# calmiLovesAI/ComputerVision.pytorch

Hardware: AMD Instinct MI355X
Metric: images/sec 640x640 YOLOv8-n train step (higher is better)
Workload: dtype f16; 1 GPU; YOLOv8-n train step (fwd + v8 loss + bwd + Adam), batch 32/GPU, 640x640, nc=80, random init; global_batch=32, parallelism=dp1, launch=eager, exchange=none (1 rank), gpu_max_hw_queues=4

## Files before the change

computervision.pytorch_amd/_lib.py:

```python
from __future__ import annotations

import ctypes as C
import os

import numpy as np

_HERE = os.path.dirname(os.path.abspath(__file__))
LIB_PATH = os.environ.get("CVX_LIB") or os.path.join(_HERE, "lib", "libcvx_engine.so")
ABI_VERSION = 6
SEG_OPTS_KEY_OFFSET = 4096


class CvxError(RuntimeError):
    pass


class BufDesc(C.Structure):
    _fields_ = [("h", C.c_int32), ("w", C.c_int32), ("c", C.c_int32), ("kind", C.c_int32)]


class View(C.Structure):
    _fields_ = [("buf", C.c_int32), ("coff", C.c_int32), ("c", C.c_int32), ("pix_off", C.c_int32)]


class OpDesc(C.Structure):
    _fields_ = [
        ("type", C.c_int32),
        ("in_", View), ("out", View), ("res", View),
        ("ih", C.c_int32), ("iw", C.c_int32), ("oh", C.c_int32), ("ow", C.c_int32),
        ("k", C.c_int32), ("stride", C.c_int32), ("pad", C.c_int32), ("dil", C.c_int32),
        ("act", C.c_int32), ("needs_dgrad", C.c_int32), ("w_cin", C.c_int32),
        ("w_off", C.c_int64), ("gamma_off", C.c_int64), ("beta_off", C.c_int64), ("bias_off", C.c_int64),
        ("rmean_off", C.c_int64), ("rvar_off", C.c_int64),
        ("lane", C.c_int32), ("flags", C.c_int32),
    ]


class SegDims(C.Structure):
    _fields_ = [(k, C.c_int32) for k in ("ld", "batch", "nc", "ih", "iw", "oh", "ow")]


class SegCriterion(C.Structure):
    _fields_ = [("base", C.c_int32), ("focal_alpha", C.c_float), ("focal_gamma", C.c_float), ("class_weight", C.c_void_p),
                ("label_smoothing", C.c_float), ("ignore_index", C.c_int64), ("ohem_theta", C.c_float), ("ohem_min_kept", C.c_int64),
                ("region", C.c_int32), ("base_weight", C.c_double), ("weight", C.c_double), ("alpha", C.c_double), ("beta", C.c_double),
                ("gamma", C.c_double), ("smooth", C.c_double), ("per_image", C.c_int32), ("skip_absent", C.c_int32),
                ("region_class_weight", C.c_void_p)]


BUF_ACT_F16, BUF_PRED_F32 = 0, 1
OP_CONV, OP_MAXPOOL5, OP_UPSAMPLE2, OP_MAXPOOL2, OP_DWCONVT, OP_COPY, OP_MAXPOOL3S2, OP_AVGPOOL, OP_RESIZE, OP_MAXPOOL3S1, OP_L2NORM = 1, 2, 3, 4, 5, 6, 7, 8, 9, 10, 11
OP_DROPOUT = 12
ACT_BN_SILU, ACT_BIAS, ACT_BN_RELU, ACT_BN_LINEAR, ACT_BIAS_RELU, ACT_BIAS_LINEAR = 1, 2, 3, 4, 5, 6
OPF_RES_PRE_ACT = 1
OPF_CONV_BIAS = 2
OPF_RAW_F16 = 4

_P, _I32, _I64, _F, _U64 = C.c_void_p, C.c_int32, C.c_int64, C.c_float, C.c_uint64

EXPERIMENTAL_PROTOTYPES = {
    "cvx_chain_pair_unit": (_I32, [_P, _I32, _I32, _I32, _I32, _P, _P, _P, _P, _P, _P, _I32, _P, _I32, _I32, _I32, C.POINTER(_F), _P]),
    "cvx_chain_conv_unit": (_I32, [_P, _I32, _I32, _I32, _I32, _P, _I32, _I32, _I32, _I32, _P, _P, _I32, _P, _I32, _I32, _I32, C.POINTER(_F), _P]),
    "cvx_chain_detect_unit": (_I32, [_P, _I32, _I32, _I32, _I32, _I32, _I32, _I32, _P, _P, _P, _P, _P, _P, _P, _P, _P, _P, _P, _I32, _I32, _I32,
                                     _I32, _I32, C.POINTER(_F), _P]),
    "cvx_wgrad_time_unit": (_I32, [_P, _P, _I32, _I32, _I32, _I32, _I32, _I32, _I32, _I32, _I32, _I32, _P, _I64, C.POINTER(_F), C.POINTER(_I32), _P]),
}

PROTOTYPES = {
    "cvx_last_error": (C.c_char_p, []),
    "cvx_abi_version": (_I32, []),
    "cvx_engine_create": (_I32, [C.POINTER(_P), C.POINTER(BufDesc), _I32, C.POINTER(OpDesc), _I32, _I32, _I32, _I32, _P]),
    "cvx_engine_destroy": (_I32, [_P]),
    "cvx_engine_bind": (_I32, [_P, _P, _P, _I64, _P, _I64]),
    "cvx_engine_set_bn": (_I32, [_P, _F, _F]),
    "cvx_engine_forward": (_I32, [_P, _P, _I32, _I32, _P]),
    "cvx_engine_backward": (_I32, [_P, _P, _F]),
    "cvx_engine_backward_begin": (_I32, [_P, _P, _F]),
    "cvx_engine_backward_range": (_I32, [_P, _I32, _I32]),
    "cvx_engine_grads_ready": (_I32, [_P, _I32, _I32, _P]),
    "cvx_engine_backward_end": (_I32, [_P]),
    "cvx_engine_workspace_bytes": (_I64, [_P]),
    "cvx_engine_plan_generation": (_I64, [_P]),
    "cvx_engine_debug_copy": (_I32, [_P, _I32, _I32, _P, _I64]),
    "cvx_engine_profile": (_I32, [_P, _I32]),
    "cvx_engine_profile_read": (_I32, [_P, _I32, C.POINTER(C.c_double), C.POINTER(C.c_double), C.POINTER(C.c_double),
                                       C.POINTER(_I64)]),
    "cvx_debug_clock_buffer": (_I32, [_P]),
    "cvx_debug_conv_tile_plan": (_I32, [_I32, _I32, _I32, _I32, _I32, _P]),
    "cvx_debug_conv_dma_plan": (_I32, [_I64, _I32, _I32, _I32, _P]),
    "cvx_debug_conv_halo_plan": (_I32, [_I32, _I32, _I32, _I32, _I32, _P]),
    "cvx_debug_conv_pw_plan": (_I32, [_I64, _I32, _I32, _P]),
    "cvx_debug_conv_grid_div": (_I32, [_I32]),
    "cvx_debug_conv_wgrad_plan": (_I32, [_I32] * 14 + [_P]),
    "cvx_debug_conv2d_wgrad_nhwc": (_I32, [_P, _P] + [_I32] * 13 + [_P, _P, _I64, _P]),
    "cvx_engine_profile_dump": (_I32, [_P, C.c_char_p]),
    "cvx_pred_level_to_nchw": (_I32, [_P, _I32, _I32, _I32, _I32, _I32, _I32, _P, _P]),
    "cvx_nchw_grad_to_dpred": (_I32, [_P, _I32, _I32, _I32, _I32, _I32, _I32, _F, _P, _P]),
    "cvx_loss_v8_workspace_bytes": (_I64, [_I32, _I32, _I32, _I32]),
    "cvx_loss_v8": (_I32, [_P, _I32, _I32, _I32, _P, _I32, _I32, C.POINTER(_I32), C.POINTER(_F), _I32, _F, _F, _F, _F, _P, _P, _P,
                           _I64, _P]),
    "cvx_loss_v8_strided": (_I32, [_P, _I32, _I32, _I32, _I32, _P, _I32, _I32, C.POINTER(_I32), C.POINTER(_F), _I32, _F, _F, _F, _F, _P, _P, _P,
                                   _I64, _P]),
    "cvx_loss_v8_assignment": (_I32, [_P, _I32, _I32, _I32, _P, _P, _P]),
    "cvx_pack_targets": (_I32, [_P, _P, _P, _I32, _P, _P]),
    "cvx_decode_strided": (_I32, [_P, _I32, _I32, _I32, _I32, C.POINTER(_I32), C.POINTER(_F), _I32, _P, _P]),
    "cvx_adam_step": (_I32, [_P, _P, _P, _P, _I64, _F, _F, _F, _F, _I32, _P, _I32, _P]),
    "cvx_check_finite": (_I32, [_P, _I64, _P, _P]),
    "cvx_adam_step_dev": (_I32, [_P, _P, _P, _P, _I64, _F, _F, _F, _P, _P, _I32, _F, _P]),
    "cvx_ema_update": (_I32, [_P, _P, _I64, _F, _F, _P]),
    "cvx_adam_ema_step_dev": (_I32, [_P, _P, _P, _P, _I64, _F, _F, _F, _P, _P, _I32, _F, _P, _F, _F, _P]),
    "cvx_optim_step": (_I32, [_I32, _P, _P, _P, _P, _I64, _P, _P, _I32, _P, _F, _F, _F, _P, _I32, _F, _P, _P, _F, _F, _P]),
    "cvx_grad_norm_workspace": (_I64, [_I64]),
    "cvx_grad_norm": (_I32, [_P, _I64, _P, _P, _I32, _F, _F, _P, _P, _P, _I64, _P]),
    "cvx_engine_set_stream": (_I32, [_P, _P]),
    "cvx_engine_exchange_stream": (_P, [_P]),
    "cvx_decode": (_I32, [_P, _I32, _I32, _I32, C.POINTER(_I32), C.POINTER(_F), _I32, _P, _P]),
    "cvx_yolo7_decode": (_I32, [_P, _I32, _I32, _I32, _P, _P, _I32, _I32, _I32, _P, _P, _P]),
    "cvx_ssd_decode": (_I32, [_P, _P, _P, _I32, _I32, _I32, _F, _F, _P, _P, _P]),
    "cvx_ssd_decode_max": (_I32, [_P, _P, _P, _I32, _I32, _I32, _F, _F, _P, _P, _P, _P]),
    "cvx_pred_cols_to_nchw": (_I32, [_P, _I32, _I32, _I32, _I32, _I32, _I32, _I32, _P, _I64, _I64, _P]),
    "cvx_nms_workspace_bytes": (_I64, [_I32, _I32]),
    "cvx_nms": (_I32, [_P, _I32, _I32, _I32, _F, _F, _I32, _P, _P, _P, _P, _I64, _P]),
    "cvx_nms_variant": (_I32, [_P, _I32, _I32, _I32, _F, _F, _I32, _I32, _P, _P, _P, _P, _I64, _P]),
    "cvx_centernet_decode_workspace_bytes": (_I64, [_I32, _I32, _I32, _I32]),
    "cvx_centernet_decode": (_I32, [_P, _I32, _I32, _I32, _I32, _I32, _I32, _I32, _I32, _F, _F, _I32, _P, _P, _P, _P, _P, _P, _P, _I64, _P]),
    "cvx_conv2d_nhwc": (_I32, [_P, _I32, _I32, _I32, _I32, _P, _I32, _I32, _I32, _I32, _I32, _I32, _P, _P, _P, _P]),
    "cvx_conv2d_dgrad_nhwc": (_I32, [_P, _I32, _I32, _I32, _I32, _P, _I32, _I32, _I32, _I32, _I32, _P, _P]),
    "cvx_conv2d_wgrad_workspace_bytes": (_I64, [_I32, _I32, _I32, _I32, _I32, _I32]),
    "cvx_conv2d_wgrad_nhwc": (_I32, [_P, _P, _I32, _I32, _I32, _I32, _I32, _I32, _I32, _I32, _I32, _P, _P, _I64, _P]),
    "cvx_bn_silu_train_nhwc": (_I32, [_P, _I32, _I32, _I32, _P, _P, _F, _F, _P, _P, _P, _P, _P, _P, _P, _P]),
    "cvx_bn_silu_bwd_nhwc": (_I32, [_P, _P, _I32, _I32, _I32, _P, _P, _P, _F, _P, _P, _P, _P, _I32, _P]),
    "cvx_letterbox_geometry": (_I32, [_I32, _I32, _I32, _I32, _P, _P, _P, _P, _P]),
    "cvx_letterbox_u8_to_nchw": (_I32, [_P, _I32, _I32, _I32, _I32, _P, _I32, _I32, _P]),
    "cvx_letterbox_batch_u8_to_nchw": (_I32, [_P, _I32, _I32, _I32, _P, _I32, _I32, _P]),
    "cvx_det_to_image": (_I32, [_P, _P, _I32, _I32, _I32, _P, _P, _P, _P, _P]),
    "cvx_draw_detections": (_I32, [_P, _I32, _I32, _I32, _P, _P, _I32, _P, _I32, _I32, _I32, _P]),
    "cvx_seg_overlay": (_I32, [_P, _I32, _I32, _I32, _P, _I32, _I32, _I32, _I32, _I32, _I32, _P, _I32, _P]),
    "cvx_tiles_u8_to_nchw": (_I32, [_P, _I32, _I32, _P, _I32, _I32, _P]),
    "cvx_det_merge_workspace_bytes": (_I64, [_I32]),
    "cvx_det_merge_tiles": (_I32, [_P, _P, _I32, _I32, _P, _P, _I32, _I32, _F, _I32, _I32, _P, _P, _P, _P, _P, _I64, _P]),
    "cvx_track_state_bytes": (_I64, [_I32]),
    "cvx_track_update": (_I32, [_P, _P, _I32, _I32, _P, _I32, _P, _P, _P, _P, _P]),
    "cvx_draw_tracks": (_I32, [_P, _I32, _I32, _I32, _P, _P, _I32, _P, _P, _I32, _I32, _I32, _P]),
    "cvx_seg_stitch": (_I32, [_P, _I32, _I32, _I32, _I32, _I32, _I32, _I32, _P, _P, _I32, _P, _I32, _I32, _I32, _P, _P, _P, _P, _I32, _I32, _I32, _P]),
    "cvx_seg_tta_inputs": (_I32, [_P, _I32, _I32, _I32, _I32, _I32, _I32, _I32, _P, _P]),
    "cvx_seg_fuse": (_I32, [_P, _I32, _I32, _I32, _I32, _I32, _I32, _I32, _P, _P, _P, _P, _P]),
    "cvx_det_tta_inputs": (_I32, [_P, _I32, _I32, _I32, _P, _I32, _F, _P, _P]),
    "cvx_det_fuse_views": (_I32, [_P, _P, _I32, _P, _P, _I32, _I32, _F, _I32, _I32, _I32, _I32, _P, _P, _P, _P, _P, _P, _I64, _P]),
    "cvx_det_wbf_workspace_bytes": (_I64, [_I32]),
    "cvx_det_fuse_wbf": (_I32, [_P, _P, _I32, _P, _P, _I32, _I32, _P, _F, _F, _I32, _I32, _I32, _I32, _P, _P, _P, _P, _P, _P, _I64, _P]),
    "cvx_aug_images": (_I32, [_P, _P, _P, _I32, _P, _I32, _I32, _P]),
    "cvx_aug_boxes": (_I32, [_P, _P, _I32, _P, _I32, _I32, _I32, _P, _P, _P]),
    "cvx_aug_images_plain": (_I32, [_P, _P, _I32, _P, _I32, _I32, _P]),
    "cvx_aug_boxes_padded": (_I32, [_P, _P, _P, _I32, _P, _I32, _I32, _I32, _I32, _P, _P, _P, _P]),
    "cvx_aug_warp_mix": (_I32, [_P, _P, _I32, _P, _I32, _I32, _P]),
    "cvx_aug_boxes_warp": (_I32, [_P, _P, _I32, _P, _I32, _I32, _I32, _F, _F, _F, _I32, _P, _I32, _P, _P, _P]),
    "cvx_engine_set_seed": (_I32, [_P, _U64]),
    "cvx_engine_keep_shadows": (_I32, [_P]),
    "cvx_engine_set_fusion": (_I32, [_P, _I32]),
    "cvx_engine_fused_groups": (_I32, [_P]),
    "cvx_centernet_loss_workspace_bytes": (_I64, [_I32, _I32]),
    "cvx_centernet_loss": (_I32, [_P, _I32, _I32, _I32, _I32, _I32, _I32, _P, _P, _P, _P, _P, _I32, _F, _F, _F, _F, _P, _P, _P, _P, _P]),
    "cvx_yolo7_loss_workspace_bytes": (_I64, [_I32, _I32, _I32, _I32]),
    "cvx_yolo7_loss": (_I32, [_P, _I32, _I32, _I32, _P, _P, _P, _P, _I32, _F, _F, _F, _F, _F, _F, _P, _P, _P, _P, _P]),
    "cvx_debug_yolo7_loss_layout": (_I32, [_I32, _I32, _I32, _I32, _P]),
    "cvx_centernet_draw_targets": (_I32, [_P, _P, _I32, _I32, _I32, _I32, _I32, _P, _P, _P, _P, _P, _P]),
    "cvx_ssd_encode_targets": (_I32, [_P, _P, _I32, _I32, _P, _I32, _I32, _F, _F, _F, _P, _P, _P]),
    "cvx_multibox_loss_workspace_bytes": (_I64, [_I32, _I32]),
    "cvx_multibox_loss": (_I32, [_P, _P, _P, _I32, _I32, _I32, _F, _F, _F, _P, _P, _P, _P, _P]),
    "cvx_seg_criterion_workspace_bytes": (_I64, [C.POINTER(SegDims), C.POINTER(SegCriterion), _I32]),
    "cvx_seg_criterion_loss": (_I32, [_P, C.POINTER(SegDims), _P, C.POINTER(SegCriterion), _F, _P, _P, _P, _P, _P, _P, _P]),
    "cvx_seg_criterion_eval": (_I32, [_P, C.POINTER(SegDims), _P, C.POINTER(SegCriterion), _P, _P, _P, _P, _P]),
    "cvx_seg_criterion_lovasz_view": (_I32, [C.POINTER(SegDims), C.POINTER(SegCriterion), C.POINTER(_I64)]),
    "cvx_det_match": (_I32, [_P, _P, _I32, _I32, _I32, _P, _P, _P, _I32, _I32, C.c_double, _I32, _P, _P, _P, _I64, _P, _P, _P]),
    "cvx_det_ap": (_I32, [_P, _P, _P, _P, _I32, C.c_double, _I32, _P, _P, _P, _P]),
    "cvx_coco_match": (_I32, [_P, _P, _I32, _I32, _I32, _P, _I32, _I32, _P, _P, _I32, _I32, _P, _P, _P, _P, _P, _P, _I64, _P, _P, _P]),
    "cvx_coco_accumulate": (_I32, [_P, _P, _P, _P, _P, _I32, _P, _P, _P, _P]),
    "cvx_coco_summarize": (_I32, [_P, _P, _I32, _P, _P]),
    "cvx_seg_pipeline": (_I32, [_P, _I32, _P, _I32, _I32, C.POINTER(_F), C.POINTER(_F), _P, _P, _I32, _I32, _P]),
    "cvx_seg_pipeline_aug": (_I32, [_P, _I32, _P, _I32, _I32, _I32, _I32, C.POINTER(_F), C.POINTER(_F), C.POINTER(_F), _P, _P, _I32, _I32, _P]),
    "cvx_resize_bilinear_nchw_grad_to_rows": (_I32, [_P, _I32, _I32, _I32, _I32, _I32, _I32, _F, _P, _I32, _P]),
    "cvx_maxpool3_train_nhwc": (_I32, [_P, _I32, _I32, _I32, _I32, _I32, _P, _P, _P]),
    "cvx_maxpool3_bwd_nhwc": (_I32, [_P, _P, _I32, _I32, _I32, _I32, _I32, _P, _I32, _P]),
    "cvx_l2norm_bwd_nhwc": (_I32, [_P, _P, _P, _I32, _I32, _I32, _F, _P, _P, _I32, _P]),
    "cvx_nchw_cols_grad_to_pred": (_I32, [_P, _I64, _I64, _I32, _I32, _I32, _I32, _I32, _F, _P, _I32, _I32, _P]),
    "cvx_dwconvt_nhwc": (_I32, [_P, _I32, _I32, _I32, _I32, _I32, _P, _P, _P]),
    "cvx_dwconvt_bwd_nhwc": (_I32, [_P, _P, _I32, _I32, _I32, _I32, _I32, _P, _P, _I32, _P, _F, _P]),
    "cvx_maxpool2_bwd_nhwc": (_I32, [_P, _P, _I32, _I32, _I32, _I32, _I32, _P, _I32, _P]),
    "cvx_avgpool_global_bwd_nhwc": (_I32, [_P, _I32, _I32, _I32, _P, _I32, _P]),
    "cvx_resize_bilinear_bwd_nhwc": (_I32, [_P, _I32, _I32, _I32, _I32, _I32, _I32, _P, _I32, _P]),
    "cvx_dropout_nhwc": (_I32, [_P, _I32, _I32, _I32, _F, _U64, _P, _I32, _P]),
    "cvx_bn_act_train_nhwc": (_I32, [_P, _I32, _I32, _I32, _P, _P, _F, _F, _P, _P, _P, _I32, _I32, _P, _P, _P, _P, _P]),
    "cvx_bn_act_bwd_nhwc": (_I32, [_P, _P, _P, _I32, _I32, _I32, _P, _P, _P, _I32, _I32, _F, _P, _P, _P, _P, _I32, _P]),
    "cvx_debug_bn_bwd_plan": (_I32, [_I64, _I32, _P]),
    "cvx_debug_bn_bwd_views": (_I32, [_P, _I32, _I32, _I32, _P, _P, _P, _P, _I32, _I32, _F, _P, _I64, _I32, _P, _I64, _I32, _P, _I64, _I32, _I32,
                                      _P, _P, _P, _P]),
    "cvx_maxpool5_nhwc": (_I32, [_P, _I32, _I32, _I32, _I32, _P, _P, _P]),
    "cvx_maxpool5_bwd_nhwc": (_I32, [_P, _P, _I32, _I32, _I32, _I32, _P, _I32, _P]),
    "cvx_resize_bilinear_rows_to_nchw": (_I32, [_P, _I32, _I32, _I32, _I32, _I32, _I32, _I32, _P, _P]),
    "cvx_maxpool_nhwc": (_I32, [_P, _I32, _I32, _I32, _I32, _I32, _I32, _I32, _P, _P]),
    "cvx_avgpool_global_nhwc": (_I32, [_P, _I32, _I32, _I32, _P, _P]),
    "cvx_resize_bilinear_nhwc": (_I32, [_P, _I32, _I32, _I32, _I32, _I32, _I32, _P, _P]),
    "cvx_l2norm_nhwc": (_I32, [_P, _P, _I32, _I32, _I32, _P, _P]),
    "cvx_upsample2_nhwc": (_I32, [_P, _I32, _I32, _I32, _I32, _P, _P]),
    "cvx_upsample2_bwd_nhwc": (_I32, [_P, _I32, _I32, _I32, _I32, _P, _I32, _P]),
    "cvx_stem_train_nchw": (_I32, [_P, _I32, _I32, _I32, _P, _I32, _P, _P, _F, _F, _P, _P, _P, _P, _P, _P, _P]),
    "cvx_stem_eval_nchw": (_I32, [_P, _I32, _I32, _I32, _P, _I32, _P, _P, _P, _P]),
    "cvx_stem_wgrad_nchw": (_I32, [_P, _I32, _I32, _I32, _P, _I32, _P, _P]),
    "cvx_comm_unique_id": (_I32, [_P]),
    "cvx_comm_create": (_I32, [C.POINTER(_P), _P, _I32, _I32, _I32]),
    "cvx_comm_destroy": (_I32, [_P]),
    "cvx_allreduce_f32": (_I32, [_P, _I64, _P, _P]),
    "cvx_allreduce_grads": (_I32, [_P, _P, _P]),
    "cvx_engine_backward_exchange": (_I32, [_P, _P, _F, _P, _P, _I32, _P]),
    "cvx_stem_backward_nchw": (_I32, [_P, _I32, _I32, _I32, _P, _P, _I32, _P, _P, _P, _F, _P, _P, _P, _P]),
    "cvx_stem_backward_recompute_nchw": (_I32, [_P, _I32, _I32, _I32, _P, _P, _I32, _P, _P, _P, _P, _F, _P, _P, _P, _P]),
}

SEG_VIEW_DTYPE = np.dtype([("rows", "<u8"), ("lh", "<i4"), ("lw", "<i4"), ("flip", "<i4"), ("reserved", "<i4")])
DET_VIEW_DTYPE = np.dtype([("h", "<i4"), ("w", "<i4"), ("top", "<i4"), ("left", "<i4"), ("flip", "<i4"), ("reserved", "<i4")])

_lib = None


def load():
    global _lib
    if _lib is not None:
        return _lib
    if not os.path.exists(LIB_PATH):
        raise CvxError(f"{LIB_PATH} not found: build it with `python -c 'import __graft_entry__ as g; g.build()'` "
                       "(hipcc --offload-arch=gfx950). There is no CPU fallback.")
    lib = C.CDLL(LIB_PATH)
    for name, (res, args) in PROTOTYPES.items():
        fn = getattr(lib, name)
        fn.restype = res
        fn.argtypes = args
    for name, (res, args) in EXPERIMENTAL_PROTOTYPES.items():
        fn = getattr(lib, name, None)
        if fn is not None:
            fn.restype = res
            fn.argtypes = args
    if lib.cvx_abi_version() != ABI_VERSION:
        raise CvxError(f"ABI mismatch: library {lib.cvx_abi_version()} != binding {ABI_VERSION}")
    _lib = lib
    return lib


def has_chain() -> bool:
    return hasattr(load(), "cvx_chain_pair_unit")


def check(rc: int, what: str = ""):
    if rc != 0:
        msg = load().cvx_last_error()
        raise CvxError(f"{what}: {msg.decode() if msg else 'unknown error'}")


def ptr(t):
    return C.c_void_p(0 if t is None else t.data_ptr())


def stream_ptr(device=None):
    import torch
    return C.c_void_p(torch.cuda.current_stream(device).cuda_stream)
```

computervision.pytorch_amd/arena.py:

```python
from __future__ import annotations

from collections import OrderedDict
from typing import Dict, List

import torch
import torch.nn as nn

from . import _lib as L
from .ema import clone_model
from .engine import Engine, check_finite
from .graph import TensorSlot


class ArenaLayout:

    def __init__(self):
        self.slots: "OrderedDict[str, TensorSlot]" = OrderedDict()
        self.nbt_keys: List[str] = []
        self.convs: Dict[str, dict] = {}
        self._p = self._s = 0

    def _take(self, arena, n):
        if arena == "param":
            off, self._p = self._p, (self._p + n + 3) & ~3
# ... 5 lines not shown
        ce = (cout + 7) & ~7
        spec = dict(cout=cout, cout_eng=ce, cin=cin, k=k, **spec_extra, w_off=self._take("param", ce * k * k * cin) if w_off is None else w_off)
        self.slots[key + ".weight"] = TensorSlot("param", spec["w_off"], (cout, cin, k, k), (k * k * cin, 1, k * cin, cin))
        if bias:
            spec["bias_off"] = self._take("param", ce) if b_off is None else b_off
            self.slots[key + ".bias"] = TensorSlot("param", spec["bias_off"], (cout,), (1,))
        self.convs[key] = spec
        return spec

    def bn(self, key, c, spec):
        spec.update(gamma_off=self._take("param", c), beta_off=self._take("param", c), rmean_off=self._take("stat", c),
                    rvar_off=self._take("stat", c))
        self.slots[key + ".weight"] = TensorSlot("param", spec["gamma_off"], (c,), (1,))
        self.slots[key + ".bias"] = TensorSlot("param", spec["beta_off"], (c,), (1,))
        self.slots[key + ".running_mean"] = TensorSlot("stat", spec["rmean_off"], (c,), (1,), False)
        self.slots[key + ".running_var"] = TensorSlot("stat", spec["rvar_off"], (c,), (1,), False)
        self.slots[key + ".num_batches_tracked"] = TensorSlot("nbt", len(self.nbt_keys), (), (), False)
        self.nbt_keys.append(key + ".num_batches_tracked")

    def conv_bn(self, ckey, bkey, cout, cin, k, **spec_extra):
        self.bn(bkey, cout, self.conv(ckey, cout, cin, k, **spec_extra))

    def _finish(self):
        self.n_params = (self._p + 3) & ~3
        self.n_stats = (self._s + 3) & ~3

    def views(self, arena, which="param"):
        return {k: torch.as_strided(arena, sl.shape, sl.strides, sl.offset) for k, sl in self.slots.items() if sl.arena == which}


class _Holder(nn.Module):

    def forward(self, *a, **k):
        raise L.CvxError(f"{type(self).__name__} has no standalone forward: the engine executes the whole graph (call the model that owns it)")


class ArenaModel(nn.Module):

    bn_eps_momentum = (1e-5, 0.1)
    _bind_grads_in_eval = False

    def __init__(self, layout, num_classes: int, loss_scale: float):
        super().__init__()
        self.layout = layout
        self.num_classes = num_classes
        self.loss_scale = float(loss_scale)
        n_bn = sum(1 for key in layout.slots if key.endswith(".running_mean"))
        self._flat = {"param": torch.zeros(layout.n_params), "stat": torch.zeros(layout.n_stats), "nbt": torch.zeros(n_bn, dtype=torch.long),
                      "grad": None}
        self._anchor = torch.zeros(1, requires_grad=True)
        self._grads_attached = False
        self._engines: Dict = {}
        self._build_tree()
        self._attach_views()
        self._init_like_reference()

    __deepcopy__ = clone_model

    def _build_graph(self, h: int, w: int):
        raise NotImplementedError

    def _init_like_reference(self):
        raise NotImplementedError

    def ctor_args(self) -> dict:
        return dict(num_classes=self.num_classes, loss_scale=self.loss_scale)

    def _engine_key(self, h, w, dev):
        return (h, w, dev)

    def _after_bind(self, eng):
        pass

    def _check_input(self, x, training):
        if x.dim() != 4 or x.shape[1] != 3:
            raise ValueError("expected images of shape (B, 3, H, W)")

    def _build_tree(self):
        for key in self.layout.slots:
            mod = self
            for name in key.split(".")[:-1]:
                if name not in mod._modules:
                    mod.add_module(name, _Holder())
                mod = mod._modules[name]

    def _attach_views(self):
        for key, sl in self.layout.slots.items():
            mod = self
            parts = key.split(".")
            for name in parts[:-1]:
                mod = mod._modules[name]
            if sl.arena == "nbt":
                mod._buffers[parts[-1]] = self._flat["nbt"][sl.offset]
                continue
            view = torch.as_strided(self._flat[sl.arena], sl.shape, sl.strides, sl.offset)
            if sl.trainable:
                old = mod._parameters.get(parts[-1])
                mod._parameters[parts[-1]] = nn.Parameter(view, requires_grad=True if old is None else old.requires_grad)
            else:
                mod._buffers[parts[-1]] = view
        self._grads_attached = False

    def _apply(self, fn, recurse=True):
        moved = {k: fn(self._flat[k]) for k in ("param", "stat", "nbt")}
        if moved["param"].dtype != torch.float32 or moved["stat"].dtype != torch.float32:
            raise L.CvxError("the engine keeps fp32 master parameters; half()/bfloat16() are not supported (compute is fp16 inside)")
        for k, t in moved.items():
            self._flat[k] = (t.long() if k == "nbt" else t).contiguous()
        self._flat["grad"] = None
        self._anchor = fn(self._anchor.detach()).requires_grad_(True)
        self._attach_views()
        self._engines.clear()
        return self

    @property
    def flat_params(self) -> torch.Tensor:
        return self._flat["param"]

    @property
    def flat_stats(self) -> torch.Tensor:
        return self._flat["stat"]

    @property
    def flat_grads(self) -> torch.Tensor:
        if self._flat["grad"] is None or self._flat["grad"].device != self._flat["param"].device:
            self._flat["grad"] = torch.zeros_like(self._flat["param"])
            self._grads_attached = False
        return self._flat["grad"]

    def attach_grads(self):
        g = self.flat_grads
        modules = dict(self.named_modules())
        for key, slot in self.layout.slots.items():
            if not slot.trainable:
                continue
            mod_name, attr = key.rsplit(".", 1)
            modules[mod_name]._parameters[attr].grad = torch.as_strided(g, slot.shape, slot.strides, slot.offset)
        self._grads_attached = True

    def engine_for(self, h: int, w: int) -> Engine:
        dev = self._flat["param"].device
        key = self._engine_key(h, w, dev)
        eng = self._engines.get(key)
        if eng is None:
            if dev.type != "cuda":
                raise L.CvxError(f"{type(self).__name__} runs on an MI355X only: move the model with .to('cuda') first (there is no CPU fallback)")
            eng = Engine(self._build_graph(h, w), dev)
            eng.set_bn(*self.bn_eps_momentum)
            self._engines[key] = eng
        eng.bind(self._flat["param"], self.flat_grads if self.training or self._bind_grads_in_eval else self._flat["grad"], self._flat["stat"])
        self._after_bind(eng)
        return eng

    def _run_forward(self, x: torch.Tensor, training: bool, pred=None) -> torch.Tensor:
        self._check_input(x, training)
        eng = self.engine_for(int(x.shape[2]), int(x.shape[3]))
        self._last_engine = eng
        rows = eng.forward(x, training, pred)
        if training:
            self._flat["nbt"] += 1
        return rows

    def _engine_backward(self, dpred: torch.Tensor, loss_scale: float, run_backward=None):
        first = next(p for p in self.parameters() if p.requires_grad)
        if first.grad is None:
            self.flat_grads.zero_()
            self._grads_attached = False
        if run_backward is not None:
            run_backward(self._last_engine, dpred, loss_scale)
        else:
            self._last_engine.backward(dpred, loss_scale)
        if not self._grads_attached or first.grad is None:
            self.attach_grads()


class EngineTrainStep:

    def __init__(self, model, criterion, optimizer, scaler=None, process_group=None, n_buckets: int = 4):
        self.model, self.criterion, self.optimizer, self.scaler = model, criterion, optimizer, scaler
        self.pg, self.n_buckets = process_group, n_buckets
        self.world, self.distributed = 1, False
        if process_group is not None or (torch.distributed.is_available() and torch.distributed.is_initialized()):
            self.world = torch.distributed.get_world_size(process_group)
            self.distributed = True
        self._side = None

    def _begin(self) -> float:
        if not self.model.training:
            raise L.CvxError(f"{type(self).__name__}: call model.train() first")
        self.optimizer.sync_lr()
        return self.scaler.begin_step() if self.scaler is not None else self.model.loss_scale

    def _backward(self, eng, dpred, scale):
        m = self.model
        if self.distributed and m.flat_params.device.type == "cuda":
            if self._side is None:
                from .train import OverlappedExchange
                self._side = OverlappedExchange(self.pg, self.n_buckets)
            self._side.backward(eng, m.flat_grads, dpred, scale)
        else:
            eng.backward(dpred, scale)

    def _update(self):
        if self.scaler is not None:
            if getattr(self.optimizer, "clip_grad_norm", None) is None:
                check_finite(self.model.flat_grads, self.scaler.found_inf)
            self.optimizer.found_inf = self.scaler.found_inf
        self.optimizer.step(zero_grad=True, grad_scale=1.0 / self.world)
        if self.scaler is not None:
            self.scaler.end_step()
```

computervision.pytorch_amd/csrc/loss_v8.hip:

```cpp
#include <cstring>
#include "cvx_common.h"
#include "../../include/cvx_engine.h"

namespace {

constexpr int REG = 16;
constexpr int TOPK = 10;
constexpr int MAXLV = 4;

struct Levels {
  int n;
  int a_off[MAXLV + 1];
  int w[MAXLV];
  float stride[MAXLV];
};

__device__ __forceinline__ void anchor_of(const Levels& L, int a, float* ax, float* ay, float* stride) {
  int lv = 0;
#pragma unroll
  for (int i = 1; i < MAXLV; ++i)
    if (i < L.n && a >= L.a_off[i]) lv = i;
  int r = a - L.a_off[lv];
  int y = r / L.w[lv], x = r - y * L.w[lv];
  *ax = x + 0.5f;
  *ay = y + 0.5f;
  *stride = L.stride[lv];
}

__device__ __forceinline__ float ciou_val(float ax1, float ay1, float ax2, float ay2, float bx1, float by1, float bx2, float by2) {
  const float eps = 1e-7f;
  float w1 = ax2 - ax1, h1 = ay2 - ay1 + eps, w2 = bx2 - bx1, h2 = by2 - by1 + eps;
  float iw = fmaxf(fminf(ax2, bx2) - fmaxf(ax1, bx1), 0.f), ih = fmaxf(fminf(ay2, by2) - fmaxf(ay1, by1), 0.f);
  float inter = iw * ih;
  float uni = w1 * h1 + w2 * h2 - inter + eps;
  float iou = inter / uni;
  float cw = fmaxf(ax2, bx2) - fminf(ax1, bx1), ch = fmaxf(ay2, by2) - fminf(ay1, by1);
  float c2 = cw * cw + ch * ch + eps;
  float sx = bx1 + bx2 - ax1 - ax2, sy = by1 + by2 - ay1 - ay2;
  float rho2 = (sx * sx + sy * sy) * 0.25f;
  float dat = atanf(w2 / h2) - atanf(w1 / h1);
  float v = 0.40528473456935108578f * dat * dat;
  float alpha = v / (v - iou + (1.f + eps));
  return iou - (rho2 / c2 + v * alpha);
}

__device__ __forceinline__ float ciou_grad(float ax1, float ay1, float ax2, float ay2, float bx1, float by1, float bx2, float by2, float g[4]) {
  const float eps = 1e-7f;
  float w1 = ax2 - ax1, h1 = ay2 - ay1 + eps, w2 = bx2 - bx1, h2 = by2 - by1 + eps;
  float iw_raw = fminf(ax2, bx2) - fmaxf(ax1, bx1), ih_raw = fminf(ay2, by2) - fmaxf(ay1, by1);
  float iw = fmaxf(iw_raw, 0.f), ih = fmaxf(ih_raw, 0.f);
  float inter = iw * ih;
  float uni = w1 * h1 + w2 * h2 - inter + eps;
  float iou = inter / uni;
  float cw = fmaxf(ax2, bx2) - fminf(ax1, bx1), ch = fmaxf(ay2, by2) - fminf(ay1, by1);
  float c2 = cw * cw + ch * ch + eps;
  float sx = bx1 + bx2 - ax1 - ax2, sy = by1 + by2 - ay1 - ay2;
  float rho2 = (sx * sx + sy * sy) * 0.25f;
  float dat = atanf(w2 / h2) - atanf(w1 / h1);
  const float k4pi2 = 0.40528473456935108578f;
  float v = k4pi2 * dat * dat;
  float alpha = v / (v - iou + (1.f + eps));
  float diw[4] = {(iw_raw > 0.f && ax1 > bx1) ? -1.f : 0.f, 0.f, (iw_raw > 0.f && ax2 < bx2) ? 1.f : 0.f, 0.f};
  float dih[4] = {0.f, (ih_raw > 0.f && ay1 > by1) ? -1.f : 0.f, 0.f, (ih_raw > 0.f && ay2 < by2) ? 1.f : 0.f};
  float dw1[4] = {-1.f, 0.f, 1.f, 0.f}, dh1[4] = {0.f, -1.f, 0.f, 1.f};
  float dcw[4] = {ax1 < bx1 ? -1.f : 0.f, 0.f, ax2 > bx2 ? 1.f : 0.f, 0.f};
  float dch[4] = {0.f, ay1 < by1 ? -1.f : 0.f, 0.f, ay2 > by2 ? 1.f : 0.f};
  float drho[4] = {-0.5f * sx, -0.5f * sy, -0.5f * sx, -0.5f * sy};
  float inv_u2 = 1.f / (uni * uni), inv_c22 = 1.f / (c2 * c2), inv_hw = 1.f / (h1 * h1 + w1 * w1);
#pragma unroll
  for (int i = 0; i < 4; ++i) {
    float dinter = diw[i] * ih + iw * dih[i];
    float duni = dw1[i] * h1 + w1 * dh1[i] - dinter;
    float diou = (dinter * uni - inter * duni) * inv_u2;
    float dc2 = 2.f * cw * dcw[i] + 2.f * ch * dch[i];
    float dpen = (drho[i] * c2 - rho2 * dc2) * inv_c22;
    float datan1 = (h1 * dw1[i] - w1 * dh1[i]) * inv_hw;
    float dv = 2.f * k4pi2 * dat * (-datan1);
    g[i] = diou - dpen - alpha * dv;
  }
  return iou - (rho2 / c2 + v * alpha);
}

__global__ void tgt_prep_kernel(const float* tg, int N, int B, float img_w, float img_h, float* gtbox, int* gtlabel, int* gtb, int* gtvalid,
                                int* img_start, int* img_end) {
  int n = blockIdx.x * blockDim.x + threadIdx.x;
  if (n >= N) return;
  const float* t = tg + (long long)n * 6;
  int b = (int)t[0];
  float cx = t[2] * img_w, cy = t[3] * img_h, w = t[4] * img_w, h = t[5] * img_h;
  float x1 = cx - w / 2, y1 = cy - h / 2, x2 = cx + w / 2, y2 = cy + h / 2;
  gtbox[n * 4 + 0] = x1;
  gtbox[n * 4 + 1] = y1;
  gtbox[n * 4 + 2] = x2;
  gtbox[n * 4 + 3] = y2;
  gtlabel[n] = (int)t[1];
  gtb[n] = b;
  gtvalid[n] = (x1 + y1 + x2 + y2) > 0.f;
  if (b >= 0 && b < B) {
    if (n == 0 || (int)tg[(long long)(n - 1) * 6] != b) img_start[b] = n;
    if (n == N - 1 || (int)tg[(long long)(n + 1) * 6] != b) img_end[b] = n + 1;
  }
}

__global__ void pred_prep_kernel(const float* pred, int B, int A, int no, Levels L, float* pbox) {
  long long i = (long long)blockIdx.x * blockDim.x + threadIdx.x;
  if (i >= (long long)B * A * 4) return;
  int side = (int)(i & 3);
  long long ba = i >> 2;
  int a = (int)(ba % A);
  const float* l = pred + ba * no + side * REG;
  float v[REG];
  float mx = -INFINITY;
#pragma unroll
  for (int k = 0; k < REG; k += 4) {
    f4 q = *reinterpret_cast<const f4*>(l + k);
    v[k] = q[0];
    v[k + 1] = q[1];
    v[k + 2] = q[2];
    v[k + 3] = q[3];
  }
#pragma unroll
  for (int k = 0; k < REG; ++k) mx = fmaxf(mx, v[k]);
  float s = 0.f, e = 0.f;
#pragma unroll
  for (int k = 0; k < REG; ++k) {
    float p = __expf(v[k] - mx);
    s += p;
    e += p * k;
  }
  float d = e / s;
  float ax, ay, st;
  anchor_of(L, a, &ax, &ay, &st);
  float c = (side & 1) ? ay : ax;
  pbox[i] = side < 2 ? c - d : c + d;
}

constexpr int TAL_TPB = 1024;
__global__ __launch_bounds__(TAL_TPB) void tal_metric_kernel(const float* pred, int A, int no, int nc, Levels L, const float* pbox, const float* gtbox,
                                                         const int* gtlabel, const int* gtb, const int* gtvalid, float* ov, float* metric,
                                                         uint8_t* mask) {
  extern __shared__ float smet[];
  __shared__ float rv[TAL_TPB / 64];
  __shared__ int ri[TAL_TPB / 64];
  const int n = blockIdx.x;
  const int b = gtb[n];
  const bool valid = gtvalid[n] != 0;
  const float gx1 = gtbox[n * 4], gy1 = gtbox[n * 4 + 1], gx2 = gtbox[n * 4 + 2], gy2 = gtbox[n * 4 + 3];
  int label = gtlabel[n];
  label = min(max(label, 0), nc - 1);
  for (int a = threadIdx.x; a < A; a += TAL_TPB) {
    float ax, ay, st;
    anchor_of(L, a, &ax, &ay, &st);
    float px = ax * st, py = ay * st;
    float dmin = fminf(fminf(px - gx1, py - gy1), fminf(gx2 - px, gy2 - py));
    float o = 0.f, m = 0.f;
    if (valid && dmin > 1e-9f) {
      const float* pb = pbox + ((long long)b * A + a) * 4;
      o = fmaxf(ciou_val(gx1, gy1, gx2, gy2, pb[0] * st, pb[1] * st, pb[2] * st, pb[3] * st), 0.f);
      float sc = cvx_sigmoid(pred[((long long)b * A + a) * no + 4 * REG + label]);
      float o2 = o * o;
      m = sqrtf(sc) * (o2 * o2 * o2);
    }
    ov[(long long)n * A + a] = o;
    metric[(long long)n * A + a] = m;
    mask[(long long)n * A + a] = 0;
    smet[a] = m;
  }
  __syncthreads();
  const int lane = threadIdx.x & 63, wave = threadIdx.x >> 6;
  for (int r = 0; r < TOPK; ++r) {
    float best = 0.f;
    int bi = 0x7fffffff;
    for (int a = threadIdx.x; a < A; a += TAL_TPB) {
      float m = smet[a];
      if (m > best) {
        best = m;
        bi = a;
      }
    }
    for (int o = 1; o < 64; o <<= 1) {
      float ob = __shfl_xor(best, o);
      int oi = __shfl_xor(bi, o);
      if (ob > best || (ob == best && oi < bi)) {
        best = ob;
        bi = oi;
      }
    }
    if (lane == 0) {
      rv[wave] = best;
      ri[wave] = bi;
    }
    __syncthreads();
    float fb = rv[0];
    int fi = ri[0];
#pragma unroll
    for (int w = 1; w < TAL_TPB / 64; ++w)
      if (rv[w] > fb || (rv[w] == fb && ri[w] < fi)) {
        fb = rv[w];
        fi = ri[w];
      }
    __syncthreads();
    if (!(fb > 0.f)) break;
    if (threadIdx.x == 0) {
      smet[fi] = -1.f;
      mask[(long long)n * A + fi] = 1;
    }
    __syncthreads();
  }
}

__global__ void tal_resolve_kernel(int B, int A, const int* img_start, const int* img_end, const float* ov, const uint8_t* mask, int* gt_idx) {
  long long i = (long long)blockIdx.x * blockDim.x + threadIdx.x;
  if (i >= (long long)B * A) return;
  int b = (int)(i / A), a = (int)(i - (long long)b * A);
  int s = img_start[b], e = img_end[b];
  int cnt = 0, first = -1, arg = s;
  float best = -1.f;
  for (int n = s; n < e; ++n) {
    if (mask[(long long)n * A + a]) {
      if (cnt == 0) first = n;
      ++cnt;
    }
    float o = ov[(long long)n * A + a];
    if (o > best) {
      best = o;
      arg = n;
    }
  }
  gt_idx[i] = cnt == 0 ? -1 : (cnt == 1 ? first : arg);
}

__global__ __launch_bounds__(TAL_TPB) void tal_posmax_kernel(int A, const int* gtb, const int* gt_idx, const float* ov, const float* metric,
                                                         float* pos_align, float* pos_ov) {
  __shared__ float sa[TAL_TPB / 64], so[TAL_TPB / 64];
  const int n = blockIdx.x;
  const int b = gtb[n];
  float ma = 0.f, mo = 0.f;
  for (int a = threadIdx.x; a < A; a += TAL_TPB) {
    if (gt_idx[(long long)b * A + a] == n) {
      ma = fmaxf(ma, metric[(long long)n * A + a]);
      mo = fmaxf(mo, ov[(long long)n * A + a]);
    }
  }
  ma = cvx_wave_max64(ma);
  mo = cvx_wave_max64(mo);
  if ((threadIdx.x & 63) == 0) {
    sa[threadIdx.x >> 6] = ma;
    so[threadIdx.x >> 6] = mo;
  }
  __syncthreads();
  if (threadIdx.x == 0) {
    float fa = sa[0], fo = so[0];
#pragma unroll
    for (int w = 1; w < TAL_TPB / 64; ++w) {
      fa = fmaxf(fa, sa[w]);
      fo = fmaxf(fo, so[w]);
    }
    pos_align[n] = fa;
    pos_ov[n] = fo;
  }
}

__global__ __launch_bounds__(256) void tal_norm_kernel(long long BA, int A, const int* gt_idx, const float* metric, const float* pos_align,
                                                       const float* pos_ov, float* norm, float* part) {
  __shared__ float sw[4];
  long long i = (long long)blockIdx.x * 256 + threadIdx.x;
  float v = 0.f;
  if (i < BA) {
    int g = gt_idx[i];
    if (g >= 0) {
      int a = (int)(i % A);
      v = metric[(long long)g * A + a] * pos_ov[g] / (pos_align[g] + 1e-9f);
    }
    norm[i] = v;
  }
  v = cvx_wave_sum64(v);
  if ((threadIdx.x & 63) == 0) sw[threadIdx.x >> 6] = v;
  __syncthreads();
  if (threadIdx.x == 0) part[blockIdx.x] = (sw[0] + sw[1]) + (sw[2] + sw[3]);
}

__device__ __forceinline__ float block_sum_partials(const float* part, int np) {
  __shared__ float sw[4];
  float v = 0.f;
  for (int i = threadIdx.x; i < np; i += 256) v += part[i];
  v = cvx_wave_sum64(v);
  if ((threadIdx.x & 63) == 0) sw[threadIdx.x >> 6] = v;
  __syncthreads();
  float t = (sw[0] + sw[1]) + (sw[2] + sw[3]);
  __syncthreads();
  return t;
}

__global__ __launch_bounds__(256) void loss_grad_kernel(const float* pred, int B, int A, int no, int nc, Levels L, const float* pbox,
                                                        const float* gtbox, const int* gtlabel, const int* gt_idx, const float* norm,
                                                        const float* tss_part, int n_tss_part, float gain_box, float gain_cls, float gain_dfl,
                                                        float loss_scale, half_t* dpred, float* loss_part) {
  __shared__ float sl[4][3];
  const float tss = fmaxf(block_sum_partials(tss_part, n_tss_part), 1.f);
  const int lane = threadIdx.x & 63, s = lane & 15;
  const long long BA = (long long)B * A;
  const long long i = (long long)blockIdx.x * 16 + (threadIdx.x >> 4);
  const bool live = i < BA;
  const long long ii = live ? i : 0;
  const int a = (int)(ii % A);
  const float* p = pred + ii * no;
  half_t* dp = dpred + ii * no;
  const int g = live ? gt_idx[ii] : -1;
  const bool fg = g >= 0;
  const float w = fg ? norm[ii] : 0.f;
  const float kscale = (float)B / tss * loss_scale;
  float l_cls = 0.f, l_box = 0.f, l_dfl = 0.f;

  int label = fg ? min(max(gtlabel[g], 0), nc - 1) : -1;
  const float kc = gain_cls * kscale;
  if ((nc & 3) == 0) {
    for (int c4 = s * 4; c4 < nc; c4 += 64) {
      if (live) {
        const f4 x4 = *reinterpret_cast<const f4*>(p + 4 * REG + c4);
        h4 o;
#pragma unroll
        for (int k = 0; k < 4; ++k) {
          const float x = x4[k];
          const float t = (c4 + k == label) ? w : 0.f;
          const float e = __expf(-fabsf(x));
          const float l1p = e < 1e-3f ? e * (1.f - e * (0.5f - e * (1.f / 3.f))) : __logf(1.f + e);
          l_cls += fmaxf(x, 0.f) - x * t + l1p;
          const float sg = (x >= 0.f ? 1.f : e) * __builtin_amdgcn_rcpf(1.f + e);
          o[k] = (half_t)((sg - t) * kc);
        }
        *reinterpret_cast<h4*>(dp + 4 * REG + c4) = o;
      }
    }
  } else {
    for (int c = s; c < nc; c += 16) {
      if (live) {
        float x = p[4 * REG + c];
        float t = (c == label) ? w : 0.f;
        l_cls += fmaxf(x, 0.f) - x * t + log1pf(__expf(-fabsf(x)));
        dp[4 * REG + c] = (half_t)((cvx_sigmoid(x) - t) * kc);
      }
    }
  }

  const int side = s >> 2, q = s & 3;
  f4 lg = live ? *reinterpret_cast<const f4*>(p + side * REG + q * 4) : f4{0.f, 0.f, 0.f, 0.f};
  float mx = fmaxf(fmaxf(lg[0], lg[1]), fmaxf(lg[2], lg[3]));
  mx = fmaxf(mx, __shfl_xor(mx, 1));
  mx = fmaxf(mx, __shfl_xor(mx, 2));
  float ex[4], se = 0.f, sb = 0.f;
#pragma unroll
  for (int k = 0; k < 4; ++k) {
    ex[k] = __expf(lg[k] - mx);
    se += ex[k];
    sb += ex[k] * (float)(q * 4 + k);
  }
  se += __shfl_xor(se, 1);
  se += __shfl_xor(se, 2);
  sb += __shfl_xor(sb, 1);
  sb += __shfl_xor(sb, 2);
  const float inv_se = 1.f / se;
  const float E = sb * inv_se;
  const int base = lane & ~15;
  const float dl = __shfl(E, base + 0), dt = __shfl(E, base + 4), dr = __shfl(E, base + 8), db = __shfl(E, base + 12);
  float gout[4] = {0.f, 0.f, 0.f, 0.f};
  if (fg) {
    float ax, ay, st;
    anchor_of(L, a, &ax, &ay, &st);
    const float inv_st = 1.f / st;
    const float tx1 = gtbox[g * 4] * inv_st, ty1 = gtbox[g * 4 + 1] * inv_st, tx2 = gtbox[g * 4 + 2] * inv_st, ty2 = gtbox[g * 4 + 3] * inv_st;
    float gb[4];
    float ci = ciou_grad(ax - dl, ay - dt, ax + dr, ay + db, tx1, ty1, tx2, ty2, gb);
    if (s == 0) l_box = (1.f - ci) * w;
    const float dE = side == 0 ? gb[0] : side == 1 ? gb[1] : side == 2 ? -gb[2] : -gb[3];
    const float kb = gain_box * kscale * w;
    float tdist = side == 0 ? ax - tx1 : side == 1 ? ay - ty1 : side == 2 ? tx2 - ax : ty2 - ay;
    tdist = fminf(fmaxf(tdist, 0.f), (float)(REG - 1) - 0.01f);
    const int tl = (int)tdist;
    const float wl = (float)(tl + 1) - tdist, wr = 1.f - wl;
    const float kd = gain_dfl * kscale * w * 0.25f;
    const float lse = mx + __logf(se);
    float ce = 0.f;
#pragma unroll
    for (int k = 0; k < 4; ++k) {
      const int bin = q * 4 + k;
      const float pk = ex[k] * inv_se;
      const float ind = (bin == tl ? wl : 0.f) + (bin == tl + 1 ? wr : 0.f);
      ce += ind * (lse - lg[k]);
      gout[k] = kb * dE * pk * ((float)bin - E) + kd * (pk - ind);
    }
    ce += __shfl_xor(ce, 1);
    ce += __shfl_xor(ce, 2);
    if (q == 0) l_dfl = ce * 0.25f * w;
  }
  if (live) {
    h4 o = {(half_t)gout[0], (half_t)gout[1], (half_t)gout[2], (half_t)gout[3]};
    *reinterpret_cast<h4*>(dp + side * REG + q * 4) = o;
  }

  l_box = cvx_wave_sum64(l_box);
  l_cls = cvx_wave_sum64(l_cls);
  l_dfl = cvx_wave_sum64(l_dfl);
  if (lane == 0) {
    sl[threadIdx.x >> 6][0] = l_box;
    sl[threadIdx.x >> 6][1] = l_cls;
    sl[threadIdx.x >> 6][2] = l_dfl;
  }
  __syncthreads();
  if (threadIdx.x < 3) loss_part[(long long)blockIdx.x * 3 + threadIdx.x] = (sl[0][threadIdx.x] + sl[1][threadIdx.x]) + (sl[2][threadIdx.x] + sl[3][threadIdx.x]);
}

__global__ __launch_bounds__(1024) void loss_finalize_kernel(const float* loss_part, int nblocks, const float* tss_part, int n_tss_part,
                                                             float gain_box, float gain_cls, float gain_dfl, float* items, float* aux) {
  __shared__ double sw[16][3];
  __shared__ float st[4];
  {
    float v = 0.f;
    if (threadIdx.x < 256) {
      for (int i = threadIdx.x; i < n_tss_part; i += 256) v += tss_part[i];
      v = cvx_wave_sum64(v);
      if ((threadIdx.x & 63) == 0) st[threadIdx.x >> 6] = v;
    }
  }
  double acc[3] = {0, 0, 0};
  for (int i = threadIdx.x; i < nblocks; i += 1024)
    for (int k = 0; k < 3; ++k) acc[k] += (double)loss_part[(long long)i * 3 + k];
  for (int k = 0; k < 3; ++k) {
    for (int o = 1; o < 64; o <<= 1) acc[k] += __shfl_xor(acc[k], o);
    if ((threadIdx.x & 63) == 0) sw[threadIdx.x >> 6][k] = acc[k];
  }
  __syncthreads();
  if (threadIdx.x == 0) {
    const float tss_raw = (st[0] + st[1]) + (st[2] + st[3]);
    const float tss = fmaxf(tss_raw, 1.f);
    const float gains[3] = {gain_box, gain_cls, gain_dfl};
    for (int k = 0; k < 3; ++k) {
      double t = 0;
      for (int w = 0; w < 16; ++w) t += sw[w][k];
      items[k] = (float)(t / (double)tss) * gains[k];
    }
    if (aux) aux[0] = tss_raw;
  }
}

struct Ws {
  float *gtbox, *pbox, *ov, *metric, *norm, *pos_align, *pos_ov, *tss_part, *loss_part, *aux;
  int *gtlabel, *gtb, *gtvalid, *img_start, *img_end, *gt_idx;
  uint8_t* mask;
};

long long align_up(long long x) { return (x + 255) & ~255LL; }

long long carve(char* base, int B, int A, int N, Ws* w) {
  long long off = 0;
  auto take = [&](long long bytes) {
    char* p = base ? base + off : nullptr;
    off += align_up(bytes);
    return p;
  };
  const long long BA = (long long)B * A;
  const int Nn = N > 0 ? N : 1;
  Ws t;
  t.gtbox = (float*)take(Nn * 16LL);
  t.gtlabel = (int*)take(Nn * 4LL);
  t.gtb = (int*)take(Nn * 4LL);
  t.gtvalid = (int*)take(Nn * 4LL);
  t.img_start = (int*)take(B * 4LL);
  t.img_end = (int*)take(B * 4LL);
  t.pbox = (float*)take(BA * 16);
  t.ov = (float*)take((long long)Nn * A * 4);
  t.metric = (float*)take((long long)Nn * A * 4);
  t.mask = (uint8_t*)take((long long)Nn * A);
  t.gt_idx = (int*)take(BA * 4);
  t.norm = (float*)take(BA * 4);
  t.pos_align = (float*)take(Nn * 4LL);
  t.pos_ov = (float*)take(Nn * 4LL);
  t.tss_part = (float*)take(((BA + 255) / 256) * 4);
  t.loss_part = (float*)take(((BA + 15) / 16) * 12);
  t.aux = (float*)take(64);
  if (w) *w = t;
  return off;
}

}

extern "C" int64_t cvx_loss_v8_workspace_bytes(int32_t batch, int32_t anchors, int32_t nc, int32_t max_targets) {
  (void)nc;
  return carve(nullptr, batch, anchors, max_targets, nullptr) + 256;
}

extern "C" int cvx_loss_v8(const float* pred, int32_t B, int32_t A, int32_t nc, const float* targets, int32_t N, int32_t max_targets,
                           const int32_t* level_hw, const float* strides, int32_t n_levels, float gain_box, float gain_cls, float gain_dfl,
                           float loss_scale, float* loss_items, void* dpred_f16, void* workspace, int64_t workspace_bytes, void* hip_stream) {
  return cvx_loss_v8_strided(pred, nc + 4 * REG, B, A, nc, targets, N, max_targets, level_hw, strides, n_levels, gain_box, gain_cls, gain_dfl,
                             loss_scale, loss_items, dpred_f16, workspace, workspace_bytes, hip_stream);
}

extern "C" int cvx_loss_v8_strided(const float* pred, int32_t pred_ld, int32_t B, int32_t A, int32_t nc, const float* targets, int32_t N,
                                   int32_t max_targets, const int32_t* level_hw, const float* strides, int32_t n_levels, float gain_box,
                                   float gain_cls, float gain_dfl, float loss_scale, float* loss_items, void* dpred_f16, void* workspace,
                                   int64_t workspace_bytes, void* hip_stream) {
  CVX_CHECK(pred && loss_items && dpred_f16 && workspace && level_hw && strides, "null arguments");
  CVX_CHECK(pred_ld >= nc + 4 * REG && pred_ld % 4 == 0, "pred_ld must cover 64 + nc values and be a multiple of 4");
  CVX_CHECK(n_levels >= 1 && n_levels <= MAXLV, "1..4 levels");
  CVX_CHECK(N >= 0 && N <= max_targets && (N == 0 || targets), "targets");
  CVX_CHECK(workspace_bytes >= cvx_loss_v8_workspace_bytes(B, A, nc, max_targets), "workspace too small");
  CVX_CHECK(((uintptr_t)pred % 16) == 0 && ((uintptr_t)dpred_f16 % 8) == 0, "alignment");
  hipStream_t st = (hipStream_t)hip_stream;
  const int no = pred_ld;
  Levels L;
  memset(&L, 0, sizeof(L));
  L.n = n_levels;
  int off = 0;
  for (int i = 0; i < n_levels; ++i) {
    L.a_off[i] = off;
    L.w[i] = level_hw[2 * i + 1];
    L.stride[i] = strides[i];
    off += level_hw[2 * i] * level_hw[2 * i + 1];
  }
  L.a_off[n_levels] = off;
  CVX_CHECK(off == A, "level sizes do not add up to the anchor count");
  const float img_h = level_hw[0] * strides[0], img_w = level_hw[1] * strides[0];
  char* base = (char*)(((uintptr_t)workspace + 255) & ~(uintptr_t)255);
  Ws w;
  carve(base, B, A, max_targets, &w);
  const long long BA = (long long)B * A;
  const int n_tss = (int)((BA + 255) / 256);
  const int n_lb = (int)((BA + 15) / 16);
  half_t* dpred = (half_t*)dpred_f16;

  {
    char *a = (char*)w.img_start, *b = (char*)w.img_end;
    if (b > a && b - a <= 4096) {
      CVX_HIP(hipMemsetAsync(a, 0, (size_t)(b - a) + (size_t)B * 4, st));
    } else {
      CVX_HIP(hipMemsetAsync(w.img_start, 0, B * 4, st));
      CVX_HIP(hipMemsetAsync(w.img_end, 0, B * 4, st));
    }
  }
  if (N > 0) {
    hipLaunchKernelGGL(tgt_prep_kernel, dim3(cvx_cdiv(N, 128)), dim3(128), 0, st, targets, N, B, img_w, img_h, w.gtbox, w.gtlabel, w.gtb,
                       w.gtvalid, w.img_start, w.img_end);
    hipLaunchKernelGGL(pred_prep_kernel, dim3(cvx_cdiv(BA * 4, 256)), dim3(256), 0, st, pred, B, A, no, L, w.pbox);
    hipLaunchKernelGGL(tal_metric_kernel, dim3(N), dim3(TAL_TPB), (size_t)A * 4, st, pred, A, no, nc, L, w.pbox, w.gtbox, w.gtlabel, w.gtb,
                       w.gtvalid, w.ov, w.metric, w.mask);
  }
  hipLaunchKernelGGL(tal_resolve_kernel, dim3(cvx_cdiv(BA, 256)), dim3(256), 0, st, B, A, w.img_start, w.img_end, w.ov, w.mask, w.gt_idx);
  if (N > 0)
    hipLaunchKernelGGL(tal_posmax_kernel, dim3(N), dim3(TAL_TPB), 0, st, A, w.gtb, w.gt_idx, w.ov, w.metric, w.pos_align, w.pos_ov);
  hipLaunchKernelGGL(tal_norm_kernel, dim3(n_tss), dim3(256), 0, st, BA, A, w.gt_idx, w.metric, w.pos_align, w.pos_ov, w.norm, w.tss_part);
  hipLaunchKernelGGL(loss_grad_kernel, dim3(n_lb), dim3(256), 0, st, pred, B, A, no, nc, L, w.pbox, w.gtbox, w.gtlabel, w.gt_idx, w.norm,
                     w.tss_part, n_tss, gain_box, gain_cls, gain_dfl, loss_scale, dpred, w.loss_part);
  hipLaunchKernelGGL(loss_finalize_kernel, dim3(1), dim3(1024), 0, st, w.loss_part, n_lb, w.tss_part, n_tss, gain_box, gain_cls, gain_dfl,
                     loss_items, w.aux);
  CVX_HIP(hipGetLastError());
  return 0;
}

extern "C" int cvx_loss_v8_assignment(const void* workspace, int32_t B, int32_t A, int32_t max_targets, int32_t* gt_index, float* norm_score,
                                      void* hip_stream) {
  CVX_CHECK(workspace && gt_index && norm_score && B > 0 && A > 0, "bad arguments");
  char* base = (char*)(((uintptr_t)workspace + 255) & ~(uintptr_t)255);
  Ws w;
  carve(base, B, A, max_targets, &w);
  hipStream_t st = (hipStream_t)hip_stream;
  CVX_HIP(hipMemcpyAsync(gt_index, w.gt_idx, (size_t)B * A * 4, hipMemcpyDeviceToDevice, st));
  CVX_HIP(hipMemcpyAsync(norm_score, w.norm, (size_t)B * A * 4, hipMemcpyDeviceToDevice, st));
  return 0;
}

namespace {
__global__ __launch_bounds__(256) void pack_targets_kernel(const float* bi, const float* cls, const float* box, int N, float* out) {
  const int i = blockIdx.x * 256 + threadIdx.x;
  if (i >= N) return;
  const float b = bi[i];
  int rank = 0;
  for (int j = 0; j < N; ++j) {
    const float bj = bi[j];
    rank += (bj < b || (bj == b && j < i)) ? 1 : 0;
  }
  float* o = out + (long long)rank * 6;
  o[0] = b;
  o[1] = cls[i];
  o[2] = box[i * 4 + 0];
  o[3] = box[i * 4 + 1];
  o[4] = box[i * 4 + 2];
  o[5] = box[i * 4 + 3];
}
}

extern "C" int cvx_pack_targets(const float* batch_idx, const float* cls, const float* bboxes, int32_t n, float* rows, void* hip_stream) {
  if (n <= 0) return 0;
  CVX_CHECK(batch_idx && cls && bboxes && rows, "null arguments");
  hipLaunchKernelGGL(pack_targets_kernel, dim3(cvx_cdiv(n, 256)), dim3(256), 0, (hipStream_t)hip_stream, batch_idx, cls, bboxes, n, rows);
  CVX_HIP(hipGetLastError());
  return 0;
}
```

computervision.pytorch_amd/csrc/misc_ops.hip:

```cpp
#include <algorithm>
#include "misc_ops.h"
#include "bilinear.h"
#include "bn_common.h"

namespace {

__device__ __forceinline__ long long voff(const ViewDesc& v, int b, long long pix) { return (long long)b * v.bstride + pix * v.ld; }

__global__ void image_to_nhwc8_kernel(const float* img, int B, int HW, half_t* out) {
  long long i = (long long)blockIdx.x * blockDim.x + threadIdx.x;
  long long n = (long long)B * HW;
  if (i >= n) return;
  long long b = i / HW, pix = i - b * HW;
  const float* src = img + b * 3 * HW + pix;
  h8 o = {(half_t)src[0], (half_t)src[HW], (half_t)src[2LL * HW], (half_t)0, (half_t)0, (half_t)0, (half_t)0, (half_t)0};
  *reinterpret_cast<h8*>(out + i * 8) = o;
}

__global__ void maxpool2_kernel(ViewDesc in, ViewDesc out, int B, int IH, int IW, int OH, int OW, int CG) {
  long long i = (long long)blockIdx.x * blockDim.x + threadIdx.x;
  long long n = (long long)B * OH * OW * CG;
  if (i >= n) return;
  int cg = (int)(i % CG);
  long long t = i / CG;
// ... 713 lines not shown
      h8 g = *reinterpret_cast<const h8*>(gout.p + voff(gout, (int)b, pix) + cg * 8);
      if (relu) {
        const h8 fo = *reinterpret_cast<const h8*>(fout.p + voff(fout, (int)b, pix) + cg * 8);
#pragma unroll
        for (int i = 0; i < 8; ++i)
          if (!((float)fo[i] > 0.f)) g[i] = (half_t)0.f;
      }
      *reinterpret_cast<h8*>(dy + m * C + cg * 8) = g;
#pragma unroll
      for (int i = 0; i < 8; ++i) acc[0][i] += (float)g[i];
    }
  }
  cvx_bn::block_channel_sums<1>(acc, C, CG, cg, active, sacc, part, blockIdx.x);
}

__global__ void copy_slice_kernel(ViewDesc in, ViewDesc out, int B, int HW, int CG) {
  long long i = (long long)blockIdx.x * blockDim.x + threadIdx.x;
  long long n = (long long)B * HW * CG;
  if (i >= n) return;
  int cg = (int)(i % CG);
  long long t = i / CG;
  int pix = (int)(t % HW);
  int b = (int)(t / HW);
  *reinterpret_cast<h8*>(out.p + voff(out, b, pix) + cg * 8) = *reinterpret_cast<const h8*>(in.p + voff(in, b, pix) + cg * 8);
}
__global__ void add_slice_kernel(ViewDesc in, ViewDesc out, int B, int HW, int CG) {
  long long i = (long long)blockIdx.x * blockDim.x + threadIdx.x;
  long long n = (long long)B * HW * CG;
  if (i >= n) return;
  int cg = (int)(i % CG);
  long long t = i / CG;
  int pix = (int)(t % HW);
  int b = (int)(t / HW);
  half_t* q = out.p + voff(out, b, pix) + cg * 8;
  const h8 a = *reinterpret_cast<const h8*>(in.p + voff(in, b, pix) + cg * 8), o = *reinterpret_cast<const h8*>(q);
  h8 r;
#pragma unroll
  for (int k = 0; k < 8; ++k) r[k] = (half_t)((float)a[k] + (float)o[k]);
  *reinterpret_cast<h8*>(q) = r;
}

__global__ void maxpool5_fwd_kernel(ViewDesc in, ViewDesc out, int B, int H, int W, int CG, uint8_t* idx) {
  long long i = (long long)blockIdx.x * blockDim.x + threadIdx.x;
  long long n = (long long)B * H * W * CG;
  if (i >= n) return;
  int cg = (int)(i % CG);
  long long t = i / CG;
  int w = (int)(t % W);
  t /= W;
  int h = (int)(t % H);
  int b = (int)(t / H);
  float best[8];
  int bi[8];
#pragma unroll
  for (int k = 0; k < 8; ++k) {
    best[k] = -INFINITY;
    bi[k] = 0;
  }
  bool first = true;
#pragma unroll
  for (int dy = 0; dy < 5; ++dy) {
    const int hh = h + dy - 2;
    const bool rok = hh >= 0 && hh < H;
    const int hc = min(max(hh, 0), H - 1);
    h8 v[5];
    bool ok[5];
#pragma unroll
    for (int dx = 0; dx < 5; ++dx) {
      const int ww = w + dx - 2;
      ok[dx] = rok && ww >= 0 && ww < W;
      const int wc = min(max(ww, 0), W - 1);
      v[dx] = *reinterpret_cast<const h8*>(in.p + voff(in, b, (long long)hc * W + wc) + cg * 8);
    }
#pragma unroll
    for (int dx = 0; dx < 5; ++dx) {
      if (!ok[dx]) continue;
#pragma unroll
      for (int k = 0; k < 8; ++k) {
        float f = (float)v[dx][k];
        if (first || f > best[k]) {
          best[k] = f;
          bi[k] = dy * 5 + dx;
        }
      }
      first = false;
    }
  }
  h8 o;
#pragma unroll
  for (int k = 0; k < 8; ++k) o[k] = (half_t)best[k];
  long long pix = (long long)h * W + w;
  *reinterpret_cast<h8*>(out.p + voff(out, b, pix) + cg * 8) = o;
  if (idx) {
    unsigned long long pk = 0;
#pragma unroll
    for (int k = 0; k < 8; ++k) pk |= (unsigned long long)(bi[k] & 0xff) << (8 * k);
    *reinterpret_cast<unsigned long long*>(idx + (((long long)b * H * W + pix) * CG + cg) * 8) = pk;
  }
}

__global__ void maxpool5_bwd_kernel(ViewDesc gout, ViewDesc gin, int B, int H, int W, int CG, const uint8_t* idx, int accumulate) {
  long long i = (long long)blockIdx.x * blockDim.x + threadIdx.x;
  long long n = (long long)B * H * W * CG;
  if (i >= n) return;
  int cg = (int)(i % CG);
  long long t = i / CG;
  int w = (int)(t % W);
  t /= W;
  int h = (int)(t % H);
  int b = (int)(t / H);
  float acc[8];
#pragma unroll
  for (int k = 0; k < 8; ++k) acc[k] = 0.f;
#pragma unroll
  for (int dy = 0; dy < 5; ++dy) {
    const int oh = h + dy - 2;
    const bool rok = oh >= 0 && oh < H;
    const int ohc = min(max(oh, 0), H - 1);
    unsigned long long pk[5];
    h8 g[5];
    bool ok[5];
#pragma unroll
    for (int dx = 0; dx < 5; ++dx) {
      const int ow = w + dx - 2;
      ok[dx] = rok && ow >= 0 && ow < W;
      const long long pix = (long long)ohc * W + min(max(ow, 0), W - 1);
      pk[dx] = *reinterpret_cast<const unsigned long long*>(idx + (((long long)b * H * W + pix) * CG + cg) * 8);
      g[dx] = *reinterpret_cast<const h8*>(gout.p + voff(gout, b, pix) + cg * 8);
    }
#pragma unroll
    for (int dx = 0; dx < 5; ++dx) {
      if (!ok[dx]) continue;
      const int tapcode = (4 - dy) * 5 + (4 - dx);
#pragma unroll
      for (int k = 0; k < 8; ++k)
        if ((int)((pk[dx] >> (8 * k)) & 0xff) == tapcode) acc[k] += (float)g[dx][k];
    }
  }
  half_t* q = gin.p + voff(gin, b, (long long)h * W + w) + cg * 8;
  if (accumulate) {
    h8 old = *reinterpret_cast<const h8*>(q);
#pragma unroll
    for (int k = 0; k < 8; ++k) acc[k] += (float)old[k];
  }
  h8 o;
#pragma unroll
  for (int k = 0; k < 8; ++k) o[k] = (half_t)acc[k];
  *reinterpret_cast<h8*>(q) = o;
}

__device__ __forceinline__ void pool5_row(const h8* src, int h, int w, int W, h8* rm, unsigned* ri) {
  float best[8];
  int bi[8];
  bool first = true;
#pragma unroll
  for (int dx = 0; dx < 5; ++dx) {
    const int ww = w + dx - 2;
    const bool ok = ww >= 0 && ww < W;
    const h8 v = src[h * W + min(max(ww, 0), W - 1)];
#pragma unroll
    for (int k = 0; k < 8; ++k) {
      const float f = (float)v[k];
      const bool take = ok && (first || f > best[k]);
      best[k] = take ? f : (first ? -INFINITY : best[k]);
      bi[k] = take ? dx : (first ? 0 : bi[k]);
    }
    first = first && !ok;
  }
  h8 o;
  unsigned pk = 0;
#pragma unroll
  for (int k = 0; k < 8; ++k) {
    o[k] = (half_t)best[k];
    pk |= (unsigned)bi[k] << (4 * k);
  }
  rm[h * W + w] = o;
  ri[h * W + w] = pk;
}
__device__ __forceinline__ h8 pool5_col(const h8* rm, const unsigned* ri, int h, int w, int H, int W, unsigned long long* pk_out) {
  float best[8];
  int bi[8];
  bool first = true;
#pragma unroll
  for (int dy = 0; dy < 5; ++dy) {
    const int hh = h + dy - 2;
    const bool ok = hh >= 0 && hh < H;
    const int q = min(max(hh, 0), H - 1) * W + w;
    const h8 v = rm[q];
    const unsigned di = ri[q];
#pragma unroll
    for (int k = 0; k < 8; ++k) {
      const float f = (float)v[k];
      const bool take = ok && (first || f > best[k]);
      best[k] = take ? f : (first ? -INFINITY : best[k]);
      bi[k] = take ? dy * 5 + (int)((di >> (4 * k)) & 7u) : (first ? 0 : bi[k]);
    }
    first = first && !ok;
  }
  h8 o;
  unsigned long long pk = 0;
#pragma unroll
  for (int k = 0; k < 8; ++k) {
    o[k] = (half_t)best[k];
    pk |= (unsigned long long)(bi[k] & 0xff) << (8 * k);
  }
  *pk_out = pk;
  return o;
}

constexpr int SPPF_FWD_BYTES_PER_PIXEL = 16 + 16 + 4;
constexpr int SPPF_BWD_BYTES_PER_PIXEL = 16 + 32;

__global__ __launch_bounds__(256) void sppf_pool3_fwd_kernel(ViewDesc in, ViewDesc o1, ViewDesc o2, ViewDesc o3, int H, int W, int CG, uint8_t* i1,
                                                             uint8_t* i2, uint8_t* i3) {
  extern __shared__ __attribute__((aligned(16))) unsigned char sppf_lds[];
  const int HW = H * W;
  h8* cur = reinterpret_cast<h8*>(sppf_lds);
  h8* rm = cur + HW;
  unsigned* ri = reinterpret_cast<unsigned*>(rm + HW);
  const int b = blockIdx.x / CG, cg = blockIdx.x - b * CG;
  for (int p = threadIdx.x; p < HW; p += 256) cur[p] = *reinterpret_cast<const h8*>(in.p + voff(in, b, p) + cg * 8);
  __syncthreads();
#pragma unroll
  for (int s = 0; s < 3; ++s) {
    const ViewDesc& out = s == 0 ? o1 : s == 1 ? o2 : o3;
    uint8_t* idx = s == 0 ? i1 : s == 1 ? i2 : i3;
    for (int p = threadIdx.x; p < HW; p += 256) {
      const int h = p / W;
      pool5_row(cur, h, p - h * W, W, rm, ri);
    }
    __syncthreads();
    for (int p = threadIdx.x; p < HW; p += 256) {
      const int h = p / W;
      unsigned long long pk;
      const h8 o = pool5_col(rm, ri, h, p - h * W, H, W, &pk);
      cur[p] = o;
      *reinterpret_cast<h8*>(out.p + voff(out, b, p) + cg * 8) = o;
      if (idx) *reinterpret_cast<unsigned long long*>(idx + (((long long)b * HW + p) * CG + cg) * 8) = pk;
    }
    __syncthreads();
  }
}

__global__ __launch_bounds__(256) void sppf_pool3_bwd_kernel(ViewDesc g3, ViewDesc g2, ViewDesc g1, ViewDesc g0, int H, int W, int CG, const uint8_t* i1,
                                                             const uint8_t* i2, const uint8_t* i3, int acc_mask) {
  extern __shared__ __attribute__((aligned(16))) unsigned char sppf_lds[];
  const int HW = H * W;
  h8* gcur = reinterpret_cast<h8*>(sppf_lds);
  h8* gnext = gcur + HW;
  unsigned long long* pks = reinterpret_cast<unsigned long long*>(gnext + HW);
  const int b = blockIdx.x / CG, cg = blockIdx.x - b * CG;
  for (int p = threadIdx.x; p < HW; p += 256) gcur[p] = *reinterpret_cast<const h8*>(g3.p + voff(g3, b, p) + cg * 8);
#pragma unroll
  for (int s = 2; s >= 0; --s) {
    const uint8_t* idx = s == 2 ? i3 : s == 1 ? i2 : i1;
    const ViewDesc& gin = s == 2 ? g2 : s == 1 ? g1 : g0;
    const bool accumulate = ((acc_mask >> s) & 1) != 0;
    for (int p = threadIdx.x; p < HW; p += 256) pks[p] = *reinterpret_cast<const unsigned long long*>(idx + (((long long)b * HW + p) * CG + cg) * 8);
    __syncthreads();
    for (int q = threadIdx.x; q < HW; q += 256) {
      const int hq = q / W, wq = q - hq * W;
      float a[8];
#pragma unroll
      for (int k = 0; k < 8; ++k) a[k] = 0.f;
      for (int dy = 0; dy < 5; ++dy) {
        const int h = hq - dy + 2;
        if (h < 0 || h >= H) continue;
        for (int dx = 0; dx < 5; ++dx) {
          const int w = wq - dx + 2;
          if (w < 0 || w >= W) continue;
          const int p = h * W + w;
          const unsigned long long pk = pks[p];
          const h8 g = gcur[p];
          const unsigned tap = (unsigned)(dy * 5 + dx);
#pragma unroll
          for (int k = 0; k < 8; ++k)
            if (((pk >> (8 * k)) & 0xff) == tap) a[k] += (float)g[k];
        }
      }
      half_t* dst = gin.p + voff(gin, b, q) + cg * 8;
      if (accumulate) {
        const h8 old = *reinterpret_cast<const h8*>(dst);
#pragma unroll
        for (int k = 0; k < 8; ++k) a[k] += (float)old[k];
      }
      h8 o;
#pragma unroll
      for (int k = 0; k < 8; ++k) o[k] = (half_t)a[k];
      gnext[q] = o;
      *reinterpret_cast<h8*>(dst) = o;
    }
    __syncthreads();
    h8* t = gcur;
    gcur = gnext;
    gnext = t;
  }
}

__global__ void upsample2_fwd_kernel(ViewDesc in, ViewDesc out, int B, int H, int W, int CG) {
  long long i = (long long)blockIdx.x * blockDim.x + threadIdx.x;
  int OH = 2 * H, OW = 2 * W;
  long long n = (long long)B * OH * OW * CG;
  if (i >= n) return;
  int cg = (int)(i % CG);
  long long t = i / CG;
  int ow = (int)(t % OW);
  t /= OW;
  int oh = (int)(t % OH);
  int b = (int)(t / OH);
  h8 v = *reinterpret_cast<const h8*>(in.p + voff(in, b, (long long)(oh >> 1) * W + (ow >> 1)) + cg * 8);
  *reinterpret_cast<h8*>(out.p + voff(out, b, (long long)oh * OW + ow) + cg * 8) = v;
}

__global__ void upsample2_bwd_kernel(ViewDesc gout, ViewDesc gin, int B, int H, int W, int CG, int accumulate) {
  long long i = (long long)blockIdx.x * blockDim.x + threadIdx.x;
  long long n = (long long)B * H * W * CG;
  if (i >= n) return;
  int cg = (int)(i % CG);
  long long t = i / CG;
  int w = (int)(t % W);
  t /= W;
  int h = (int)(t % H);
  int b = (int)(t / H);
  int OW = 2 * W;
  float acc[8];
#pragma unroll
  for (int k = 0; k < 8; ++k) acc[k] = 0.f;
#pragma unroll
  for (int dy = 0; dy < 2; ++dy)
#pragma unroll
    for (int dx = 0; dx < 2; ++dx) {
      h8 g = *reinterpret_cast<const h8*>(gout.p + voff(gout, b, (long long)(2 * h + dy) * OW + 2 * w + dx) + cg * 8);
#pragma unroll
      for (int k = 0; k < 8; ++k) acc[k] += (float)g[k];
    }
  half_t* q = gin.p + voff(gin, b, (long long)h * W + w) + cg * 8;
  if (accumulate) {
    h8 old = *reinterpret_cast<const h8*>(q);
#pragma unroll
    for (int k = 0; k < 8; ++k) acc[k] += (float)old[k];
  }
  h8 o;
#pragma unroll
  for (int k = 0; k < 8; ++k) o[k] = (half_t)acc[k];
  *reinterpret_cast<h8*>(q) = o;
}

__global__ void pred_to_nchw_kernel(const float* pred, int B, int A, int no, int a_off, int HW, float* out) {
  long long i = (long long)blockIdx.x * blockDim.x + threadIdx.x;
  long long n = (long long)B * no * HW;
  if (i >= n) return;
  int pix = (int)(i % HW);
  long long t = i / HW;
  int c = (int)(t % no);
  int b = (int)(t / no);
  out[i] = pred[((long long)b * A + a_off + pix) * no + c];
}
__global__ void nchw_to_pred_f16_kernel(const float* g, int B, int A, int no, int a_off, int HW, float scale, half_t* dpred) {
  long long i = (long long)blockIdx.x * blockDim.x + threadIdx.x;
  long long n = (long long)B * HW * no;
  if (i >= n) return;
  int c = (int)(i % no);
  long long t = i / no;
  int pix = (int)(t % HW);
  int b = (int)(t / HW);
  dpred[((long long)b * A + a_off + pix) * no + c] = (half_t)(g[((long long)b * no + c) * HW + pix] * scale);
}

__global__ __launch_bounds__(256) void pack_weights_kernel(const float* master, half_t* shadow, const PackDesc* descs, const BlockRef* blocks) {
  __shared__ float tile[32][33];
  const BlockRef br = blocks[blockIdx.x];
  const PackDesc d = descs[br.desc];
  if (br.start < 0) {
    const int lin = -(br.start + 1);
    const int tci = (d.Cin + 31) / 32, tco = (d.Cout + 31) / 32;
    const int t = lin / (tco * tci), rem = lin - t * (tco * tci);
    const int co0 = (rem / tci) * 32, ci0 = (rem % tci) * 32;
    const int c = threadIdx.x & 31, r0 = threadIdx.x >> 5;
#pragma unroll
    for (int k = 0; k < 4; ++k) {
      const int r = r0 + 8 * k;
      const int co = co0 + r, ci = ci0 + c;
      tile[r][c] = (co < d.Cout && ci < d.Cin) ? master[d.src_off + ((long long)co * d.T + t) * d.Cin + ci] : 0.f;
    }
    __syncthreads();
#pragma unroll
    for (int k = 0; k < 4; ++k) {
      const int r = r0 + 8 * k;
      const int ci = ci0 + r, co = co0 + c;
      if (ci < d.Cin && co < d.Cout) shadow[d.dg_off + ((long long)ci * d.T + t) * d.Cout + co] = (half_t)tile[c][r];
    }
    return;
  }
  const int total = d.Cout * d.T * d.Cin_pad;
  for (int k = 0; k < 4; ++k) {
    int e = br.start + k * 256 + threadIdx.x;
    if (e >= total) return;
    int ci = e % d.Cin_pad;
    int row = e / d.Cin_pad;
    float v = ci < d.Cin ? master[d.src_off + (long long)row * d.Cin + ci] : 0.f;
    shadow[d.fwd_off + e] = (half_t)v;
  }
}

__global__ __launch_bounds__(256) void ps_pack_kernel(const half_t* dg_base, half_t* ps_base, const PsPackDesc d) {
  const int k8 = (4 * d.C) / 8;
  const long long total = 4LL * d.cin_pad * k8;
  const long long idx = (long long)blockIdx.x * 256 + threadIdx.x;
  if (idx >= total) return;
  const int n = (int)(idx / k8), kk = (int)(idx - (long long)n * k8) * 8;
  const int phase = n / d.cin_pad, ci = n - phase * d.cin_pad;
  const int tau = kk / d.C, co = kk - tau * d.C;
  const int wt = d.wtap[phase * 4 + tau];
  h8 v = {0, 0, 0, 0, 0, 0, 0, 0};
  if (wt >= 0) v = *reinterpret_cast<const h8*>(dg_base + d.dg_off + ((long long)ci * d.T + wt) * d.C + co);
  *reinterpret_cast<h8*>(ps_base + d.ps_off + (long long)n * 4 * d.C + kk) = v;
}

__global__ __launch_bounds__(256) void reduce_slabs_kernel(const float* slabs, float* grads, float inv_scale, const SlabDesc* descs,
                                                           const BlockRef* blocks) {
  __shared__ float sred[256];
  const BlockRef br = blocks[blockIdx.x];
  const SlabDesc d = descs[br.desc];
  if (d.nsplit == 0) return;
  const long long total = (long long)d.rows * d.Cin;
  const long long slab_elems = (long long)d.rows * d.Cin_pad;
  const int LR = d.lanes, COLS = 256 / LR;
  const int col = threadIdx.x % COLS, rl = threadIdx.x / COLS;
  const long long e = (long long)br.start + col;
  float acc = 0.f;
// ... 242 lines not shown
```

computervision.pytorch_amd/csrc/unit_ops.hip:

```cpp
#include <vector>

#include "../../include/cvx_engine.h"
#include "misc_ops.h"
#include "stem.h"

namespace {

struct Scratch {
  void* p = nullptr;
  int alloc(size_t bytes) {
    CVX_HIP(hipMalloc(&p, bytes));
    CVX_HIP(hipMemset(p, 0, bytes));
    return 0;
  }
  ~Scratch() {
    if (p) (void)hipFree(p);
  }
};
size_t slab_bytes(int C) { return (size_t)cvx_stat_replicas(C) * C * CVX_STAT_WORDS * 8; }
ViewDesc dense(const void* p, int hw, int C) { return ViewDesc{(half_t*)p, (long long)hw * C, C}; }

}

extern "C" int cvx_bn_silu_train_nhwc(const float* y_f32, int32_t batch, int32_t hw, int32_t c, const float* gamma, const float* beta, float eps,
                                      float momentum, float* running_mean, float* running_var, const void* res_f16, void* out_f16,
                                      void* xhat_f16, float* mean, float* invstd, void* hip_stream) {
  return cvx_bn_act_train_nhwc(y_f32, batch, hw, c, gamma, beta, eps, momentum, running_mean, running_var, res_f16, 0, 0, out_f16, xhat_f16, mean,
                               invstd, hip_stream);
}
extern "C" int cvx_bn_act_train_nhwc(const float* y_f32, int32_t batch, int32_t hw, int32_t c, const float* gamma, const float* beta, float eps,
                                     float momentum, float* running_mean, float* running_var, const void* res_f16, int32_t act, int32_t res_pre,
                                     void* out_f16, void* xhat_f16, float* mean, float* invstd, void* hip_stream) {
  CVX_CHECK(y_f32 && gamma && beta && running_mean && running_var && out_f16 && xhat_f16 && mean && invstd && batch > 0 && hw > 0, "bad arguments");
  hipStream_t st = (hipStream_t)hip_stream;
  const long long M = (long long)batch * hw;
  Scratch slab;
  CVX_TRY(slab.alloc(slab_bytes(c)));
  CVX_TRY(cvx_bn_stats_f32(y_f32, M, c, (long long*)slab.p, st));
  BnTrainArgs ta{(const long long*)slab.p, gamma, beta, mean, invstd, running_mean, running_var, eps, momentum};
  CVX_TRY(cvx_bn_act_apply(y_f32, M, c, hw, ta, dense(out_f16, hw, c), res_f16 ? dense(res_f16, hw, c) : ViewDesc{nullptr, 0, 0}, act, res_pre,
                           (half_t*)xhat_f16, st));
  CVX_HIP(hipStreamSynchronize(st));
  return 0;
}

extern "C" int cvx_bn_silu_bwd_nhwc(const void* xhat_f16, const void* gout_f16, int32_t batch, int32_t hw, int32_t c, const float* gamma,
                                    const float* beta, const float* invstd, float inv_scale, float* dgamma, float* dbeta, void* dy_f16,
                                    void* gres_f16, int32_t res_accumulate, void* hip_stream) {
  return cvx_bn_act_bwd_nhwc(xhat_f16, gout_f16, nullptr, batch, hw, c, gamma, beta, invstd, 0, 0, inv_scale, dgamma, dbeta, dy_f16, gres_f16,
                             res_accumulate, hip_stream);
}
extern "C" int cvx_bn_act_bwd_nhwc(const void* xhat_f16, const void* gout_f16, const void* out_f16, int32_t batch, int32_t hw, int32_t c,
                                   const float* gamma, const float* beta, const float* invstd, int32_t act, int32_t res_pre, float inv_scale,
                                   float* dgamma, float* dbeta, void* dy_f16, void* gres_f16, int32_t res_accumulate, void* hip_stream) {
  CVX_CHECK(xhat_f16 && gout_f16 && gamma && beta && invstd && dgamma && dbeta && dy_f16 && batch > 0 && hw > 0, "bad arguments");
  CVX_CHECK(!(act == 0 && res_pre) || out_f16, "SiLU with a pre-activation residual: the residual's forward value is needed (pass it as out_f16)");
  const BnActKind ak{act, res_pre, out_f16 ? dense(out_f16, hw, c) : ViewDesc{nullptr, 0, 0}};
  hipStream_t st = (hipStream_t)hip_stream;
  const long long M = (long long)batch * hw;
  Scratch slab;
  CVX_TRY(slab.alloc(slab_bytes(c) + CVX_STAT_GATE_WORDS * 8));
  BnCoef k{invstd, gamma, beta};
  const ViewDesc g = dense(gout_f16, hw, c);
  const int one = cvx_bn_bwd_fused((const half_t*)xhat_f16, M, c, hw, k, (long long*)slab.p, (unsigned long long*)((char*)slab.p + slab_bytes(c)), inv_scale,
                                   dgamma, dbeta, g, ak, (half_t*)dy_f16, gres_f16 ? dense(gres_f16, hw, c) : ViewDesc{nullptr, 0, 0}, res_accumulate, st);
  if (one < 0) return one;
  if (one == 0) {
    CVX_HIP(hipStreamSynchronize(st));
    return 0;
  }
  CVX_TRY(cvx_bn_bwd_reduce((const half_t*)xhat_f16, M, c, hw, k, g, ak, (long long*)slab.p, st));
  CVX_TRY(cvx_bn_bwd_apply((const half_t*)xhat_f16, M, c, hw, k, (const long long*)slab.p, inv_scale, dgamma, dbeta, g, ak, (half_t*)dy_f16,
                           gres_f16 ? dense(gres_f16, hw, c) : ViewDesc{nullptr, 0, 0}, res_accumulate, st));
  CVX_HIP(hipStreamSynchronize(st));
  return 0;
}

extern "C" int cvx_debug_bn_bwd_plan(int64_t rows, int32_t c, int32_t* out4) {
  int o[4] = {0, 0, 0, 0};
  CVX_CHECK(out4, "bad arguments");
  CVX_TRY(cvx_bn_bwd_plan(rows, c, o));
  for (int i = 0; i < 4; ++i) out4[i] = o[i];
  return 0;
}
extern "C" int cvx_debug_bn_bwd_views(const void* kept_f16, int32_t batch, int32_t hw, int32_t c, const float* gamma, const float* beta,
                                      const float* invstd, const float* mean, int32_t act, int32_t res_pre, float inv_scale, const void* gout_f16,
                                      int64_t gout_bstride, int32_t gout_ld, const void* fwd_f16, int64_t fwd_bstride, int32_t fwd_ld,
                                      void* gres_f16, int64_t gres_bstride, int32_t gres_ld, int32_t res_accumulate, float* dgamma, float* dbeta,
                                      void* dy_f16, void* hip_stream) {
  CVX_CHECK(kept_f16 && gout_f16 && gamma && beta && invstd && dgamma && dbeta && dy_f16 && batch > 0 && hw > 0, "bad arguments");
  CVX_CHECK(gout_ld >= c && gout_bstride >= (int64_t)hw * gout_ld && (!fwd_f16 || (fwd_ld >= c && fwd_bstride >= (int64_t)hw * fwd_ld)) &&
                (!gres_f16 || (gres_ld >= c && gres_bstride >= (int64_t)hw * gres_ld)),
            "a view's pixel pitch is below its channels, or its image pitch below its pixels");
  CVX_CHECK(gout_ld % 8 == 0 && gout_bstride % 8 == 0 && (!fwd_f16 || (fwd_ld % 8 == 0 && fwd_bstride % 8 == 0)) &&
                (!gres_f16 || (gres_ld % 8 == 0 && gres_bstride % 8 == 0)),
            "view pitches in multiples of 8 elements (16-byte rows)");
  hipStream_t st = (hipStream_t)hip_stream;
  const long long M = (long long)batch * hw;
  const ViewDesc none{nullptr, 0, 0};
  const BnActKind ak{act, res_pre, fwd_f16 ? ViewDesc{(half_t*)fwd_f16, fwd_bstride, fwd_ld} : none};
  const ViewDesc g{(half_t*)gout_f16, gout_bstride, gout_ld};
  const ViewDesc gres = gres_f16 ? ViewDesc{(half_t*)gres_f16, gres_bstride, gres_ld} : none;
  Scratch slab;
  CVX_TRY(slab.alloc(slab_bytes(c)));
  BnCoef k{invstd, gamma, beta, mean};
  CVX_TRY(cvx_bn_bwd_reduce((const half_t*)kept_f16, M, c, hw, k, g, ak, (long long*)slab.p, st));
  CVX_TRY(cvx_bn_bwd_apply((const half_t*)kept_f16, M, c, hw, k, (const long long*)slab.p, inv_scale, dgamma, dbeta, g, ak, (half_t*)dy_f16, gres,
                           res_accumulate, st));
  CVX_HIP(hipStreamSynchronize(st));
  return 0;
}

extern "C" int cvx_maxpool5_nhwc(const void* x_f16, int32_t batch, int32_t h, int32_t w, int32_t c, void* out_f16, uint8_t* argmax,
                                 void* hip_stream) {
  CVX_CHECK(x_f16 && out_f16 && batch > 0 && c % 8 == 0, "bad arguments (channels in multiples of 8)");
  CVX_TRY(cvx_maxpool5_fwd(dense(x_f16, h * w, c), dense(out_f16, h * w, c), batch, h, w, c, argmax, (hipStream_t)hip_stream));
  CVX_HIP(hipStreamSynchronize((hipStream_t)hip_stream));
  return 0;
}
extern "C" int cvx_maxpool5_bwd_nhwc(const void* gout_f16, const uint8_t* argmax, int32_t batch, int32_t h, int32_t w, int32_t c,
                                     void* gin_f16, int32_t accumulate, void* hip_stream) {
  CVX_CHECK(gout_f16 && argmax && gin_f16 && batch > 0 && c % 8 == 0, "bad arguments (channels in multiples of 8)");
  CVX_TRY(cvx_maxpool5_bwd(dense(gout_f16, h * w, c), dense(gin_f16, h * w, c), batch, h, w, c, argmax, accumulate, (hipStream_t)hip_stream));
  CVX_HIP(hipStreamSynchronize((hipStream_t)hip_stream));
  return 0;
}
extern "C" int cvx_resize_bilinear_rows_to_nchw(const float* rows_f32, int32_t ld, int32_t batch, int32_t c, int32_t ih, int32_t iw, int32_t oh,
                                                int32_t ow, float* out_nchw, void* hip_stream) {
  CVX_CHECK(rows_f32 && out_nchw && batch > 0, "bad arguments");
  CVX_TRY(cvx_resize_bilinear_f32_nchw(rows_f32, ld, batch, c, ih, iw, oh, ow, out_nchw, (hipStream_t)hip_stream));
  return 0;
}
extern "C" int cvx_pred_cols_to_nchw(const float* rows, int32_t ld, int32_t col0, int32_t c, int32_t batch, int32_t anchors, int32_t a_off,
                                     int32_t hw, float* out, int64_t out_bstride, int64_t out_off, void* hip_stream) {
  CVX_CHECK(rows && out && batch > 0 && c > 0 && col0 >= 0 && col0 + c <= ld && a_off >= 0 && a_off + hw <= anchors, "bad arguments");
  return cvx_pred_cols_to_nchw_launch(rows, ld, col0, c, batch, anchors, a_off, hw, out, out_bstride, out_off, (hipStream_t)hip_stream);
}
extern "C" int cvx_nchw_cols_grad_to_pred(const float* grad, int64_t grad_bstride, int64_t grad_off, int32_t c, int32_t batch, int32_t anchors,
                                          int32_t a_off, int32_t hw, float scale, void* dpred_f16, int32_t ld, int32_t col0, void* hip_stream) {
  CVX_CHECK(grad && dpred_f16 && batch > 0 && c > 0 && col0 >= 0 && col0 + c <= ld && a_off >= 0 && a_off + hw <= anchors, "bad arguments");
  return cvx_nchw_cols_grad_to_pred_launch(grad, grad_bstride, grad_off, c, batch, anchors, a_off, hw, scale, (half_t*)dpred_f16, ld, col0,
                                           (hipStream_t)hip_stream);
}
extern "C" int cvx_l2norm_bwd_nhwc(const void* x_f16, const void* gout_f16, const float* weight, int32_t batch, int32_t hw, int32_t c, float inv_scale,
                                   void* gin_f16, float* dweight, int32_t accumulate, void* hip_stream) {
  CVX_CHECK(x_f16 && gout_f16 && weight && gin_f16 && dweight && batch > 0, "bad arguments");
  Scratch part;
  CVX_TRY(part.alloc((size_t)cvx_l2norm_bwd_blocks((long long)batch * hw) * c * 4));
  CVX_TRY(cvx_l2norm_bwd(dense(x_f16, hw, c), dense(gout_f16, hw, c), dense(gin_f16, hw, c), weight, dweight, inv_scale, batch, hw, c, accumulate,
                         (float*)part.p, (hipStream_t)hip_stream));
  CVX_HIP(hipStreamSynchronize((hipStream_t)hip_stream));
  return 0;
}
extern "C" int cvx_maxpool_nhwc(const void* x_f16, int32_t batch, int32_t h, int32_t w, int32_t c, int32_t kernel, int32_t stride,
                                int32_t ceil_mode, void* out_f16, void* hip_stream) {
  CVX_CHECK(x_f16 && out_f16 && batch > 0 && c % 8 == 0, "bad arguments (channels in multiples of 8)");
  hipStream_t st = (hipStream_t)hip_stream;
  if (kernel == 2 && stride == 2) {
    const int oh = ceil_mode ? (h + 1) / 2 : h / 2, ow = ceil_mode ? (w + 1) / 2 : w / 2;
    CVX_TRY(cvx_maxpool2(dense(x_f16, h * w, c), dense(out_f16, oh * ow, c), batch, h, w, oh, ow, c, st));
  } else if (kernel == 3 && (stride == 1 || stride == 2) && !ceil_mode) {
    const int oh = (h - 1) / stride + 1, ow = (w - 1) / stride + 1;
    CVX_TRY(cvx_maxpool3(dense(x_f16, h * w, c), dense(out_f16, oh * ow, c), batch, h, w, c, stride, nullptr, st));
  } else {
    CVX_CHECK(false, "max pools built: 2x2 / stride 2 (floor or ceil mode), 3x3 / pad 1 / stride 1 or 2");
  }
  CVX_HIP(hipStreamSynchronize(st));
  return 0;
}
extern "C" int cvx_avgpool_global_nhwc(const void* x_f16, int32_t batch, int32_t hw, int32_t c, void* out_f16, void* hip_stream) {
  CVX_CHECK(x_f16 && out_f16 && batch > 0 && c % 8 == 0, "bad arguments (channels in multiples of 8)");
  CVX_TRY(cvx_avgpool_global(dense(x_f16, hw, c), dense(out_f16, 1, c), batch, hw, c, (hipStream_t)hip_stream));
  CVX_HIP(hipStreamSynchronize((hipStream_t)hip_stream));
  return 0;
}
extern "C" int cvx_resize_bilinear_nhwc(const void* x_f16, int32_t batch, int32_t ih, int32_t iw, int32_t c, int32_t oh, int32_t ow,
                                        void* out_f16, void* hip_stream) {
  CVX_CHECK(x_f16 && out_f16 && batch > 0 && c % 8 == 0, "bad arguments (channels in multiples of 8)");
  CVX_TRY(cvx_resize_bilinear(dense(x_f16, ih * iw, c), dense(out_f16, oh * ow, c), batch, ih, iw, oh, ow, c, (hipStream_t)hip_stream));
  CVX_HIP(hipStreamSynchronize((hipStream_t)hip_stream));
  return 0;
}
extern "C" int cvx_l2norm_nhwc(const void* x_f16, const float* weight, int32_t batch, int32_t hw, int32_t c, void* out_f16, void* hip_stream) {
  CVX_CHECK(x_f16 && weight && out_f16 && batch > 0 && c % 8 == 0, "bad arguments (channels in multiples of 8)");
  CVX_TRY(cvx_l2norm(dense(x_f16, hw, c), dense(out_f16, hw, c), weight, batch, hw, c, (hipStream_t)hip_stream));
  CVX_HIP(hipStreamSynchronize((hipStream_t)hip_stream));
  return 0;
}
extern "C" int cvx_maxpool3_train_nhwc(const void* x_f16, int32_t batch, int32_t h, int32_t w, int32_t c, int32_t stride, void* out_f16,
                                       uint8_t* argmax, void* hip_stream) {
  CVX_CHECK(x_f16 && out_f16 && argmax && batch > 0 && c % 8 == 0, "bad arguments (channels in multiples of 8)");
  const int oh = (h - 1) / stride + 1, ow = (w - 1) / stride + 1;
  CVX_TRY(cvx_maxpool3(dense(x_f16, h * w, c), dense(out_f16, oh * ow, c), batch, h, w, c, stride, argmax, (hipStream_t)hip_stream));
  CVX_HIP(hipStreamSynchronize((hipStream_t)hip_stream));
  return 0;
}
extern "C" int cvx_maxpool3_bwd_nhwc(const void* gout_f16, const uint8_t* argmax, int32_t batch, int32_t h, int32_t w, int32_t c, int32_t stride,
                                     void* gin_f16, int32_t accumulate, void* hip_stream) {
  CVX_CHECK(gout_f16 && argmax && gin_f16 && batch > 0 && c % 8 == 0, "bad arguments (channels in multiples of 8)");
  const int oh = (h - 1) / stride + 1, ow = (w - 1) / stride + 1;
  CVX_TRY(cvx_maxpool3_bwd(dense(gout_f16, oh * ow, c), dense(gin_f16, h * w, c), batch, h, w, c, stride, argmax, accumulate, (hipStream_t)hip_stream));
  CVX_HIP(hipStreamSynchronize((hipStream_t)hip_stream));
  return 0;
}
extern "C" int cvx_maxpool2_bwd_nhwc(const void* x_f16, const void* gout_f16, int32_t batch, int32_t h, int32_t w, int32_t c, int32_t ceil_mode,
                                     void* gin_f16, int32_t accumulate, void* hip_stream) {
  CVX_CHECK(x_f16 && gout_f16 && gin_f16 && batch > 0 && c % 8 == 0, "bad arguments (channels in multiples of 8)");
  const int oh = ceil_mode ? (h + 1) / 2 : h / 2, ow = ceil_mode ? (w + 1) / 2 : w / 2;
  CVX_TRY(cvx_maxpool2_bwd(dense(x_f16, h * w, c), dense(gout_f16, oh * ow, c), dense(gin_f16, h * w, c), batch, h, w, oh, ow, c, accumulate,
                           (hipStream_t)hip_stream));
  CVX_HIP(hipStreamSynchronize((hipStream_t)hip_stream));
  return 0;
}
extern "C" int cvx_dwconvt_nhwc(const void* x_f16, int32_t batch, int32_t ih, int32_t iw, int32_t c, int32_t f, const float* weight, void* out_f16,
                                void* hip_stream) {
  CVX_CHECK(x_f16 && weight && out_f16 && batch > 0 && c % 8 == 0 && f >= 2 && f % 2 == 0, "bad arguments (channels in multiples of 8, even stride)");
  CVX_TRY(cvx_dwconvt(dense(x_f16, ih * iw, c), dense(out_f16, ih * f * iw * f, c), weight, batch, ih, iw, c, f, (hipStream_t)hip_stream));
  CVX_HIP(hipStreamSynchronize((hipStream_t)hip_stream));
  return 0;
}
extern "C" int cvx_dwconvt_bwd_nhwc(const void* x_f16, const void* gout_f16, int32_t batch, int32_t ih, int32_t iw, int32_t c, int32_t f,
                                    const float* weight, void* gin_f16, int32_t accumulate, float* dweight, float inv_scale, void* hip_stream) {
  CVX_CHECK(x_f16 && gout_f16 && weight && gin_f16 && dweight && batch > 0 && c % 8 == 0 && f >= 2 && f % 2 == 0,
            "bad arguments (channels in multiples of 8, even stride)");
  float* part = nullptr;
  CVX_HIP(hipMalloc((void**)&part, (size_t)cvx_dwconvt_bwd_scratch_floats((long long)batch * ih * iw, c, f) * 4));
  int rc = cvx_dwconvt_bwd(dense(x_f16, ih * iw, c), dense(gout_f16, ih * f * iw * f, c), dense(gin_f16, ih * iw, c), weight, dweight, inv_scale, batch,
                           ih, iw, c, f, accumulate, part, (hipStream_t)hip_stream);
  (void)hipStreamSynchronize((hipStream_t)hip_stream);
  (void)hipFree(part);
  return rc;
}
extern "C" int cvx_avgpool_global_bwd_nhwc(const void* gout_f16, int32_t batch, int32_t hw, int32_t c, void* gin_f16, int32_t accumulate,
                                           void* hip_stream) {
  CVX_CHECK(gout_f16 && gin_f16 && batch > 0 && c % 8 == 0, "bad arguments (channels in multiples of 8)");
  CVX_TRY(cvx_avgpool_global_bwd(dense(gout_f16, 1, c), dense(gin_f16, hw, c), batch, hw, c, accumulate, (hipStream_t)hip_stream));
  CVX_HIP(hipStreamSynchronize((hipStream_t)hip_stream));
  return 0;
}
extern "C" int cvx_resize_bilinear_bwd_nhwc(const void* gout_f16, int32_t batch, int32_t ih, int32_t iw, int32_t c, int32_t oh, int32_t ow,
                                            void* gin_f16, int32_t accumulate, void* hip_stream) {
  CVX_CHECK(gout_f16 && gin_f16 && batch > 0 && c % 8 == 0, "bad arguments (channels in multiples of 8)");
  CVX_TRY(cvx_resize_bilinear_bwd(dense(gout_f16, oh * ow, c), dense(gin_f16, ih * iw, c), batch, ih, iw, oh, ow, c, accumulate,
                                  (hipStream_t)hip_stream));
  CVX_HIP(hipStreamSynchronize((hipStream_t)hip_stream));
  return 0;
}
extern "C" int cvx_dropout_nhwc(const void* x_f16, int32_t batch, int32_t hw, int32_t c, float p, uint64_t seed, void* out_f16, int32_t accumulate,
                                void* hip_stream) {
  CVX_CHECK(x_f16 && out_f16 && batch > 0 && c % 8 == 0, "bad arguments (channels in multiples of 8)");
  CVX_TRY(cvx_dropout(dense(x_f16, hw, c), dense(out_f16, hw, c), batch, hw, c, p, seed, accumulate, (hipStream_t)hip_stream));
  CVX_HIP(hipStreamSynchronize((hipStream_t)hip_stream));
  return 0;
}
extern "C" int cvx_upsample2_nhwc(const void* x_f16, int32_t batch, int32_t h, int32_t w, int32_t c, void* out_f16, void* hip_stream) {
  CVX_CHECK(x_f16 && out_f16 && batch > 0 && c % 8 == 0, "bad arguments (channels in multiples of 8)");
  CVX_TRY(cvx_upsample2_fwd(dense(x_f16, h * w, c), dense(out_f16, 4 * h * w, c), batch, h, w, c, (hipStream_t)hip_stream));
  CVX_HIP(hipStreamSynchronize((hipStream_t)hip_stream));
  return 0;
}
extern "C" int cvx_upsample2_bwd_nhwc(const void* gout_f16, int32_t batch, int32_t h, int32_t w, int32_t c, void* gin_f16, int32_t accumulate,
                                      void* hip_stream) {
  CVX_CHECK(gout_f16 && gin_f16 && batch > 0 && c % 8 == 0, "bad arguments (channels in multiples of 8)");
  CVX_TRY(cvx_upsample2_bwd(dense(gout_f16, 4 * h * w, c), dense(gin_f16, h * w, c), batch, h, w, c, accumulate, (hipStream_t)hip_stream));
  CVX_HIP(hipStreamSynchronize((hipStream_t)hip_stream));
  return 0;
}

extern "C" int cvx_stem_train_nchw(const float* images, int32_t batch, int32_t h, int32_t w, const float* weight, int32_t cout,
                                   const float* gamma, const float* beta, float eps, float momentum, float* running_mean,
                                   float* running_var, void* out_f16, void* xhat_f16, float* mean, float* invstd, void* hip_stream) {
  CVX_CHECK(images && weight && gamma && beta && running_mean && running_var && out_f16 && xhat_f16 && mean && invstd, "null arguments");
  hipStream_t st = (hipStream_t)hip_stream;
  const StemParams sp{images, batch, h, w, h / 2, w / 2, weight, cout};
  Scratch slab;
  CVX_TRY(slab.alloc(slab_bytes(cout)));
// ... 80 lines not shown
```

computervision.pytorch_amd/engine.py:

```python
from __future__ import annotations

import ctypes as C
from typing import Optional, Sequence

import warnings

import torch

from . import _lib as L
from .graph import Graph, ParamLayout, build_yolov8_graph, grad_buckets


def _need_gpu(t: torch.Tensor, what: str):
    if not t.is_cuda:
        raise L.CvxError(f"{what} must live on an MI355X device (got {t.device}); the engine has no CPU path")


class Engine:
    _warned_stream = False
    keep_weight_images = True

    def __init__(self, graph: Graph, device: torch.device):
        self.lib = L.load()
        self.graph = graph
        self.device = torch.device(device)
        if self.device.type != "cuda":
            raise L.CvxError("the engine needs a HIP device (torch device type 'cuda'); there is no CPU path")
        bufs, ops = graph.c_arrays()
        h = C.c_void_p()
        with torch.cuda.device(self.device):
            L.check(self.lib.cvx_engine_create(C.byref(h), bufs, len(graph.bufs), ops, len(graph.ops), graph.image_buf, graph.pred_buf,
                                               self.device.index or 0, L.stream_ptr(self.device)), "cvx_engine_create")
        self.handle = h
        self._bound = None

    def bind(self, params: torch.Tensor, grads: Optional[torch.Tensor], stats: torch.Tensor):
        for t, n in ((params, "params"), (stats, "stats")):
            _need_gpu(t, n)
            assert t.dtype == torch.float32 and t.is_contiguous()
        key = (params.data_ptr(), 0 if grads is None else grads.data_ptr(), stats.data_ptr())
        if key == self._bound:
            return
        L.check(self.lib.cvx_engine_bind(self.handle, L.ptr(params), L.ptr(grads), params.numel(), L.ptr(stats), stats.numel()),
                "cvx_engine_bind")
        self._bound = key
        self._keep = (params, grads, stats)

    def set_bn(self, eps: float, momentum: float):
        L.check(self.lib.cvx_engine_set_bn(self.handle, eps, momentum), "cvx_engine_set_bn")

    def set_fusion(self, enable: bool):
        L.check(self.lib.cvx_engine_set_fusion(self.handle, int(bool(enable))), "cvx_engine_set_fusion")

    def fused_groups(self) -> int:
        return int(self.lib.cvx_engine_fused_groups(self.handle))

    def set_seed(self, seed: int):
        if seed != getattr(self, "_seed", None):
            L.check(self.lib.cvx_engine_set_seed(self.handle, int(seed) & (2 ** 64 - 1)), "cvx_engine_set_seed")
            self._seed = seed

    def forward(self, images: torch.Tensor, training: bool, pred: Optional[torch.Tensor] = None) -> torch.Tensor:
        _need_gpu(images, "images")
        images = images.contiguous().float()
        b = images.shape[0]
        no = self.graph.bufs[self.graph.pred_buf][2]
        if pred is None:
            pred = torch.empty(b, self.graph.anchors, no, device=images.device, dtype=torch.float32)
        self._use_current_stream()
        params = self._keep[0] if getattr(self, "_keep", None) else None
        wkey = None if params is None else (params.data_ptr(), params._version, PARAM_WRITES.get(params.data_ptr(), 0))
        if Engine.keep_weight_images and wkey is not None and wkey == getattr(self, "_weights_key", None) and not torch.cuda.is_current_stream_capturing():
            L.check(self.lib.cvx_engine_keep_shadows(self.handle), "cvx_engine_keep_shadows")
        self._weights_key = wkey
        L.check(self.lib.cvx_engine_forward(self.handle, L.ptr(images), b, 1 if training else 0, L.ptr(pred)), "cvx_engine_forward")
        self._images = images if training else None
        return pred

    def exchange_stream(self) -> torch.cuda.Stream:
        if getattr(self, "_xstream", None) is None:
            ptr = self.lib.cvx_engine_exchange_stream(self.handle)
            if not ptr:
                raise L.CvxError("cvx_engine_exchange_stream failed")
            self._xstream = torch.cuda.ExternalStream(int(ptr), device=self.device)
        return self._xstream

    def plan_generation(self) -> int:
        return int(self.lib.cvx_engine_plan_generation(self.handle))

    def _use_current_stream(self):
        s = torch.cuda.current_stream(self.device).cuda_stream
        if s != 0 and not Engine._warned_stream and not torch.cuda.is_current_stream_capturing():
            Engine._warned_stream = True
            warnings.warn("the engine is being launched on a non-default HIP stream: fine by itself (the engine leaves one hardware queue "
                          "to the caller), but a process that works more than four queues -- this stream, the default stream, the engine's two, "
                          "a data-parallel exchange stream, further torch streams -- pays 2.2-2.5x per train step on the ROCm 7 runtime "
                          "(tools/stream_probe.py, DESIGN.md section 6)", RuntimeWarning, stacklevel=3)
        if s != getattr(self, "_stream", None):
            L.check(self.lib.cvx_engine_set_stream(self.handle, C.c_void_p(s)), "cvx_engine_set_stream")
            self._stream = s

    def backward(self, dpred_f16: torch.Tensor, loss_scale: float):
        assert dpred_f16.dtype == torch.float16 and dpred_f16.is_contiguous()
        self._use_current_stream()
        L.check(self.lib.cvx_engine_backward(self.handle, L.ptr(dpred_f16), float(loss_scale)), "cvx_engine_backward")

    def backward_begin(self, dpred_f16: torch.Tensor, loss_scale: float):
        assert dpred_f16.dtype == torch.float16 and dpred_f16.is_contiguous()
        self._use_current_stream()
        L.check(self.lib.cvx_engine_backward_begin(self.handle, L.ptr(dpred_f16), float(loss_scale)), "cvx_engine_backward_begin")

    def backward_range(self, op_hi: int, op_lo: int):
        L.check(self.lib.cvx_engine_backward_range(self.handle, op_hi, op_lo), "cvx_engine_backward_range")

    def grads_ready(self, op_hi: int, op_lo: int, stream: torch.cuda.Stream):
        if stream is None:
            stream = torch.cuda.current_stream(self.device)
        L.check(self.lib.cvx_engine_grads_ready(self.handle, op_hi, op_lo, C.c_void_p(stream.cuda_stream)), "cvx_engine_grads_ready")

    def backward_end(self):
        L.check(self.lib.cvx_engine_backward_end(self.handle), "cvx_engine_backward_end")

    def grad_buckets(self, layout: ParamLayout, n_buckets: int):
        return grad_buckets(self.graph, layout, n_buckets)

    def read_buffer(self, buf: int, batch: int, grad: bool = False) -> torch.Tensor:
        h, w, c, _ = self.graph.bufs[buf]
        out = torch.empty(batch, h, w, c, dtype=torch.float16, device=self.device)
        L.check(self.lib.cvx_engine_debug_copy(self.handle, buf, 1 if grad else 0, L.ptr(out), out.numel() * 2), "cvx_engine_debug_copy")
        return out

    def read_layer(self, op: int, batch: int, what: str = "xhat") -> torch.Tensor:
        o = self.graph.ops[op]
        wide = what == "xhat32"
        out = torch.empty(batch, o["oh"], o["ow"], o["out"][2], dtype=torch.float32 if wide else torch.float16, device=self.device)
        which = {"xhat": 2, "dy": 3, "xhat32": 4}[what]
        L.check(self.lib.cvx_engine_debug_copy(self.handle, op, which, L.ptr(out), out.numel() * (4 if wide else 2)), "cvx_engine_debug_copy")
        return out

    PROFILE_CLASSES = ("conv_fwd", "conv_dgrad", "conv_wgrad", "bn_silu_fwd", "bn_silu_bwd", "misc", "slab_reduce")

    def profile(self, enable: bool):
        L.check(self.lib.cvx_engine_profile(self.handle, 1 if enable else 0), "cvx_engine_profile")

    def profile_read(self):
        n = len(self.PROFILE_CLASSES)
        ms, fl, by, la = (C.c_double * n)(), (C.c_double * n)(), (C.c_double * n)(), (C.c_int64 * n)()
        L.check(self.lib.cvx_engine_profile_read(self.handle, n, ms, fl, by, la), "cvx_engine_profile_read")
        return {name: dict(ms=ms[i], flops=fl[i], bytes=by[i], launches=int(la[i])) for i, name in enumerate(self.PROFILE_CLASSES)}

    def profile_dump(self, path: str):
        L.check(self.lib.cvx_engine_profile_dump(self.handle, str(path).encode()), "cvx_engine_profile_dump")

    def workspace_bytes(self) -> int:
        return int(self.lib.cvx_engine_workspace_bytes(self.handle))

    def __del__(self):
        try:
            if getattr(self, "handle", None):
                self.lib.cvx_engine_destroy(self.handle)
                self.handle = None
        except Exception:
            pass


def _levels(level_hw: Sequence[Sequence[int]], strides: Sequence[float]):
    flat = [int(v) for hw in level_hw for v in hw]
    return (C.c_int32 * len(flat))(*flat), (C.c_float * len(strides))(*[float(s) for s in strides]), len(strides)


class V8LossOp:

    def __init__(self, nc: int, gains=(7.5, 0.5, 1.5)):
        self.lib = L.load()
        self.nc = nc
        self.gains = tuple(float(g) for g in gains)
        self._ws = None

    def __call__(self, pred: torch.Tensor, targets: torch.Tensor, level_hw, strides, loss_scale: float,
                 dpred: Optional[torch.Tensor] = None):
        _need_gpu(pred, "pred")
        B, A, no = pred.shape
        assert pred.dtype == torch.float32 and no == self.nc + 64
        if not (pred.stride(2) == 1 and pred.stride(0) == A * pred.stride(1) and pred.stride(1) % 4 == 0):
            padded = torch.zeros(B, A, (no + 3) & ~3, dtype=torch.float32, device=pred.device)
            padded[..., :no] = pred
            pred = padded[..., :no]
        ld = pred.stride(1)
        n = int(targets.shape[0])
        if n:
            _need_gpu(targets, "targets")
            targets = targets.contiguous().float()
        cap = max(n, 1)
        need = int(self.lib.cvx_loss_v8_workspace_bytes(B, A, self.nc, cap))
        if self._ws is None or self._ws.numel() < need or self._ws.device != pred.device:
            self._ws = torch.empty(need, dtype=torch.uint8, device=pred.device)
        if dpred is None:
            dpred = torch.zeros(B, A, ld, dtype=torch.float16, device=pred.device)
        assert dpred.is_contiguous() and dpred.shape[2] == ld
        items = torch.empty(3, dtype=torch.float32, device=pred.device)
        lv, st, nl = _levels(level_hw, strides)
        L.check(self.lib.cvx_loss_v8_strided(L.ptr(pred), ld, B, A, self.nc, L.ptr(targets) if n else C.c_void_p(0), n, cap, lv, st, nl,
                                             self.gains[0], self.gains[1], self.gains[2], float(loss_scale), L.ptr(items), L.ptr(dpred),
                                             L.ptr(self._ws), self._ws.numel(), L.stream_ptr(pred.device)), "cvx_loss_v8")
        self._last_shape = (B, A, cap)
        return items, dpred

    def assignment(self, B: int, A: int, n_targets: int):
        assert self._ws is not None and self._last_shape == (B, A, max(n_targets, 1)), "call the loss first (same shapes)"
        dev = self._ws.device
        idx = torch.empty(B, A, dtype=torch.int32, device=dev)
        norm = torch.empty(B, A, dtype=torch.float32, device=dev)
        L.check(self.lib.cvx_loss_v8_assignment(L.ptr(self._ws), B, A, max(n_targets, 1), L.ptr(idx), L.ptr(norm), L.stream_ptr(dev)),
                "cvx_loss_v8_assignment")
        return idx.long(), norm


PARAM_WRITES: dict = {}


def _note_param_write(params: torch.Tensor):
    PARAM_WRITES[params.data_ptr()] = PARAM_WRITES.get(params.data_ptr(), 0) + 1


def adam_step(params, grads, exp_avg, exp_avg_sq, lr, betas, eps, step, found_inf=None, zero_grad=True):
    lib = L.load()
    _need_gpu(params, "params")
    _note_param_write(params)
    L.check(lib.cvx_adam_step(L.ptr(params), L.ptr(grads), L.ptr(exp_avg), L.ptr(exp_avg_sq), params.numel(), lr, betas[0], betas[1], eps,
                              step, L.ptr(found_inf), 1 if zero_grad else 0, L.stream_ptr(params.device)), "cvx_adam_step")


def adam_step_dev(params, grads, exp_avg, exp_avg_sq, betas, eps, state, found_inf=None, zero_grad=True, grad_scale=1.0):
    lib = L.load()
    _need_gpu(params, "params")
    _note_param_write(params)
    L.check(lib.cvx_adam_step_dev(L.ptr(params), L.ptr(grads), L.ptr(exp_avg), L.ptr(exp_avg_sq), params.numel(), betas[0], betas[1], eps,
                                  L.ptr(state), L.ptr(found_inf), 1 if zero_grad else 0, float(grad_scale), L.stream_ptr(params.device)),
            "cvx_adam_step_dev")


def ema_update(ema_arena: torch.Tensor, src: torch.Tensor, d: float, one_minus_d: float):
    lib = L.load()
    _need_gpu(ema_arena, "ema")
    _need_gpu(src, "src")
    if ema_arena.numel() != src.numel():
        raise L.CvxError(f"the average holds {ema_arena.numel()} values, the arena it follows {src.numel()}")
    if ema_arena.numel() == 0:
        return
    _note_param_write(ema_arena)
    L.check(lib.cvx_ema_update(L.ptr(ema_arena), L.ptr(src), ema_arena.numel(), float(d), float(one_minus_d), L.stream_ptr(src.device)),
            "cvx_ema_update")


def adam_ema_step_dev(params, grads, exp_avg, exp_avg_sq, betas, eps, state, ema_arena, d, one_minus_d, found_inf=None, zero_grad=True,
                      grad_scale=1.0):
    lib = L.load()
    _need_gpu(params, "params")
    _need_gpu(ema_arena, "ema")
    if ema_arena.numel() != params.numel():
        raise L.CvxError(f"the average holds {ema_arena.numel()} values, the parameter arena {params.numel()}")
    _note_param_write(params)
    _note_param_write(ema_arena)
    L.check(lib.cvx_adam_ema_step_dev(L.ptr(params), L.ptr(grads), L.ptr(exp_avg), L.ptr(exp_avg_sq), params.numel(), betas[0], betas[1], eps,
                                      L.ptr(state), L.ptr(found_inf), 1 if zero_grad else 0, float(grad_scale), L.ptr(ema_arena), float(d),
                                      float(one_minus_d), L.stream_ptr(params.device)), "cvx_adam_ema_step_dev")


def check_finite(grads: torch.Tensor, found_inf: torch.Tensor):
    lib = L.load()
    L.check(lib.cvx_check_finite(L.ptr(grads), grads.numel(), L.ptr(found_inf), L.stream_ptr(grads.device)), "cvx_check_finite")


OPTIM_SGD, OPTIM_ADAM = 0, 1
OPTIM_MAX_GROUPS, OPTIM_GROUP_FLOATS, OPTIM_UNMAPPED = 16, 8, 255


def _check_group_tables(n, group_map, group_state):
    if group_map.dtype != torch.uint8 or group_map.numel() != (n + 3) // 4:
        raise L.CvxError(f"the group map is one uint8 per 16-byte chunk: {(n + 3) // 4} bytes for {n} values, got {group_map.numel()} of {group_map.dtype}")
    if group_state.dtype != torch.float32 or group_state.dim() != 2 or group_state.shape[1] != OPTIM_GROUP_FLOATS or not group_state.is_contiguous():
        raise L.CvxError(f"the group table is a contiguous float32 (n_groups, {OPTIM_GROUP_FLOATS}) tensor")
    return int(group_state.shape[0])


def optim_step(kind, params, grads, buf1, buf2, group_map, group_state, state, betas=(0.9, 0.999), eps=1e-8, found_inf=None, zero_grad=True,
               grad_scale=1.0, clip_state=None, ema_arena=None, d=0.0, one_minus_d=1.0):
    lib = L.load()
    _need_gpu(params, "params")
    n = params.numel()
    G = _check_group_tables(n, group_map, group_state)
    if ema_arena is not None:
        _need_gpu(ema_arena, "ema")
        if ema_arena.numel() != n:
            raise L.CvxError(f"the average holds {ema_arena.numel()} values, the parameter arena {n}")
        _note_param_write(ema_arena)
    _note_param_write(params)
    L.check(lib.cvx_optim_step(int(kind), L.ptr(params), L.ptr(grads), L.ptr(buf1), L.ptr(buf2), n, L.ptr(group_map), L.ptr(group_state), G,
                               L.ptr(state), betas[0], betas[1], eps, L.ptr(found_inf), 1 if zero_grad else 0, float(grad_scale), L.ptr(clip_state),
                               L.ptr(ema_arena), float(d), float(one_minus_d), L.stream_ptr(params.device)), "cvx_optim_step")


def grad_norm_workspace(n: int) -> int:
    return int(L.load().cvx_grad_norm_workspace(int(n)))


def grad_norm(grads, group_map, group_state, max_norm, clip_state, workspace, grad_scale=1.0, found_inf=None):
    lib = L.load()
    _need_gpu(grads, "grads")
    G = _check_group_tables(grads.numel(), group_map, group_state)
    L.check(lib.cvx_grad_norm(L.ptr(grads), grads.numel(), L.ptr(group_map), L.ptr(group_state), G, float(grad_scale), float(max_norm),
                              L.ptr(clip_state), L.ptr(found_inf), L.ptr(workspace), workspace.numel(), L.stream_ptr(grads.device)), "cvx_grad_norm")


def decode(pred: torch.Tensor, nc: int, level_hw, strides) -> torch.Tensor:
    lib = L.load()
    _need_gpu(pred, "pred")
    B, A, no = pred.shape
    if not (pred.stride(2) == 1 and pred.stride(0) == A * pred.stride(1)):
        pred = pred.contiguous()
    y = torch.empty(B, 4 + nc, A, dtype=torch.float32, device=pred.device)
    lv, st, nl = _levels(level_hw, strides)
    L.check(lib.cvx_decode_strided(L.ptr(pred), pred.stride(1), B, A, nc, lv, st, nl, L.ptr(y), L.stream_ptr(pred.device)), "cvx_decode")
    return y


_nms_ws = {}


NMS_VARIANTS = {"tv0141_cuda": 0, "tv0141_cpu": 1, "offset": 2, "vanilla": 3}


def nms(y: torch.Tensor, conf_thres: float, iou_thres: float, max_det: int = 300, variant: str = "tv0141_cuda", boxes_xyxy: bool = False):
    lib = L.load()
    _need_gpu(y, "y")
    if not (0 <= conf_thres <= 1 and 0 <= iou_thres <= 1):
        raise AssertionError("thresholds must lie in [0, 1]")
    y = y.contiguous().float()
    B, ch, A = y.shape
    nc = ch - 4
    need = int(lib.cvx_nms_workspace_bytes(B, A))
    ws = _nms_ws.get(y.device)
    if ws is None or ws.numel() < need:
        ws = _nms_ws[y.device] = torch.empty(need, dtype=torch.uint8, device=y.device)
    rows = torch.zeros(B, max_det, 6, dtype=torch.float32, device=y.device)
    index = torch.zeros(B, max_det, dtype=torch.int32, device=y.device)
    counts = torch.zeros(B, dtype=torch.int32, device=y.device)
    L.check(lib.cvx_nms_variant(L.ptr(y), B, A, nc, conf_thres, iou_thres, max_det, NMS_VARIANTS[variant] | (0x100 if boxes_xyxy else 0), L.ptr(rows), L.ptr(index),
                                L.ptr(counts), L.ptr(ws), ws.numel(), L.stream_ptr(y.device)), "cvx_nms")
    return rows, index, counts


def yolo7_decode(rows: torch.Tensor, nc: int, level_hw, anchors_wh, input_hw, want_nms_input: bool = True):
    lib = L.load()
    _need_gpu(rows, "rows")
    rows = rows.contiguous().float()
    B, R, ld = rows.shape
    assert R == sum(h * w for h, w in level_hw)
# ... 102 lines not shown
```

computervision.pytorch_amd/model.py:

```python
from __future__ import annotations

import math
from typing import Optional

import torch
import torch.nn as nn

from .arena import ArenaModel, _Holder
from .engine import decode
from .graph import REG_MAX, STRIDES, ParamLayout, build_yolov8_graph

BN_EPS, BN_MOMENTUM = 1e-3, 0.03


class Conv2dParams(_Holder):
    def __init__(self, c1, c2, k, bias):
        super().__init__()
        self.in_channels, self.out_channels, self.kernel_size = c1, c2, (k, k)
        self.weight = nn.Parameter(torch.empty(0))
        if bias:
            self.bias = nn.Parameter(torch.empty(0))
        else:
            self.register_parameter("bias", None)

# ... 16 lines not shown
        self.bn = BatchNormParams(c2)
        self.stride = s


class Bottleneck(_Holder):
    def __init__(self, c, shortcut):
        super().__init__()
        self.cv1 = Conv(c, c, 3)
        self.cv2 = Conv(c, c, 3)
        self.add = shortcut


class C2f(_Holder):
    def __init__(self, c1, c2, n, shortcut):
        super().__init__()
        self.c = c2 // 2
        self.cv1 = Conv(c1, 2 * self.c, 1)
        self.cv2 = Conv((2 + n) * self.c, c2, 1)
        self.m = nn.ModuleList(Bottleneck(self.c, shortcut) for _ in range(n))


class SPPF(_Holder):
    def __init__(self, c1, c2):
        super().__init__()
        self.cv1 = Conv(c1, c1 // 2, 1)
        self.cv2 = Conv((c1 // 2) * 4, c2, 1)


class Upsample(_Holder):
    pass


class Concat(_Holder):
    pass


class DFL(_Holder):
    def __init__(self, c1=REG_MAX):
        super().__init__()
        self.conv = Conv2dParams(c1, 1, 1, bias=False)
        self.conv.weight.requires_grad_(False)
        self.c1 = c1


class Detect(_Holder):
    def __init__(self, nc, ch, c_box, c_cls):
        super().__init__()
        self.nc, self.nl, self.reg_max = nc, len(ch), REG_MAX
        self.no = nc + 4 * REG_MAX
        self.stride = torch.tensor([float(s) for s in STRIDES])
        self.cv2 = nn.ModuleList(nn.Sequential(Conv(x, c_box, 3), Conv(c_box, c_box, 3), Conv2dParams(c_box, 4 * REG_MAX, 1, True)) for x in ch)
        self.cv3 = nn.ModuleList(nn.Sequential(Conv(x, c_cls, 3), Conv(c_cls, c_cls, 3), Conv2dParams(c_cls, nc, 1, True)) for x in ch)
        self.dfl = DFL(REG_MAX)


class PredList(list):
    pred: Optional[torch.Tensor] = None
    level_hw = None


class _EngineFn(torch.autograd.Function):
    @staticmethod
    def forward(ctx, images, anchor, model):
        ctx.model = model
        pred = model._run_forward(images, training=True)
        return pred

    @staticmethod
    def backward(ctx, gpred):
        model = ctx.model
        model._run_backward(gpred)
        return None, None, None


class Yolo8(ArenaModel):
    bn_eps_momentum = (BN_EPS, BN_MOMENTUM)
    _bind_grads_in_eval = True

    def __init__(self, scale_name: str = "n", num_classes: int = 80, ch: int = 3, loss_scale: float = 1024.0):
        if ch != 3:
            raise ValueError("the MI355X engine is built for 3-channel images")
        super().__init__(ParamLayout(scale_name, num_classes), num_classes, loss_scale)
        self.scale_name = scale_name

    def ctor_args(self):
        return dict(super().ctor_args(), scale_name=self.scale_name)

    def _build_graph(self, h, w):
        return build_yolov8_graph(self.layout, h, w)

    def _build_tree(self):
        lay = self.layout
        c64, c128, c256, c512, c1024 = lay.c64, lay.c128, lay.c256, lay.c512, lay.c1024
        layers = [
            Conv(3, c64, 3, 2), Conv(c64, c128, 3, 2), C2f(c128, c128, lay.n3, True), Conv(c128, c256, 3, 2),
            C2f(c256, c256, lay.n6, True), Conv(c256, c512, 3, 2), C2f(c512, c512, lay.n6, True), Conv(c512, c1024, 3, 2),
            C2f(c1024, c1024, lay.n3, True), SPPF(c1024, c1024),
            Upsample(), Concat(), C2f(c1024 + c512, c512, lay.n3, False),
            Upsample(), Concat(), C2f(c512 + c256, c256, lay.n3, False),
            Conv(c256, c256, 3, 2), Concat(), C2f(c256 + c512, c512, lay.n3, False),
            Conv(c512, c512, 3, 2), Concat(), C2f(c512 + c1024, c1024, lay.n3, False),
            Detect(self.num_classes, lay.head_in, lay.c_box, lay.c_cls),
        ]
        self.model = nn.Sequential(*layers)
        self.stride = self.model[-1].stride

    def _attach_views(self):
        super()._attach_views()
        i_bn = 0
        for mod in self.modules():
            if isinstance(mod, BatchNormParams):
                mod._buffers["num_batches_tracked"] = self._flat["nbt"][i_bn]
                i_bn += 1
        dfl = self.model[-1].dfl.conv
        if dfl.weight.numel() == 0:
            dfl._parameters["weight"] = nn.Parameter(torch.arange(REG_MAX, dtype=torch.float32).view(1, REG_MAX, 1, 1), requires_grad=False)

    def _apply(self, fn, recurse=True):
        grad = self._flat["grad"]
        super()._apply(fn)
        if grad is not None:
            self._flat["grad"] = fn(grad).contiguous()
        dfl = self.model[-1].dfl.conv
        dfl._parameters["weight"] = nn.Parameter(fn(dfl.weight.data), requires_grad=False)
        self.model[-1].stride = fn(self.model[-1].stride)
        self.stride = self.model[-1].stride
        return self

    def _init_like_reference(self):
        det = self.model[-1]
        with torch.no_grad():
            for mod in self.modules():
                if isinstance(mod, Conv2dParams):
                    k = mod.kernel_size[0]
                    w = torch.empty(mod.out_channels, mod.in_channels, k, k)
                    nn.init.kaiming_uniform_(w, a=math.sqrt(5))
                    if mod.weight.requires_grad:
                        mod.weight.copy_(w)
                    if mod.bias is not None:
                        bound = 1.0 / math.sqrt(mod.in_channels * k * k)
                        b = torch.empty(mod.out_channels)
                        nn.init.uniform_(b, -bound, bound)
                        mod.bias.copy_(b)
                elif isinstance(mod, BatchNormParams):
                    mod.weight.fill_(1.0)
                    mod.bias.zero_()
                    mod.running_mean.zero_()
                    mod.running_var.fill_(0.9)
            self._flat["nbt"].fill_(1)
            for a, b, s in zip(det.cv2, det.cv3, STRIDES):
                a[-1].bias.fill_(1.0)
                b[-1].bias[:det.nc] = math.log(5 / det.nc / (640 / s) ** 2)

    def _run_forward(self, images: torch.Tensor, training: bool, pred: Optional[torch.Tensor] = None) -> torch.Tensor:
        out = super()._run_forward(images, training, pred)
        no = self.layout.no
        return out if out.shape[2] == no else out[..., :no]

    def _run_backward(self, gpred: torch.Tensor):
        dpred = (gpred * self.loss_scale).to(torch.float16)
        if self.layout.no_pad != self.layout.no:
            padded = torch.zeros(*dpred.shape[:2], self.layout.no_pad, dtype=torch.float16, device=dpred.device)
            padded[..., :self.layout.no] = dpred
            dpred = padded
        self._engine_backward(dpred.contiguous(), self.loss_scale)

    def level_shapes(self, h: int, w: int):
        return [(h // s, w // s) for s in STRIDES]

    def forward(self, x: torch.Tensor):
        B, _, H, W = x.shape
        det = self.model[-1]
        if self.training and torch.is_grad_enabled():
            pred = _EngineFn.apply(x, self._anchor, self)
        else:
            pred = self._run_forward(x, training=self.training)
        outs = PredList()
        off = 0
        for (h, w) in self.level_shapes(H, W):
            outs.append(pred[:, off:off + h * w, :].permute(0, 2, 1).reshape(B, det.no, h, w))
            off += h * w
        outs.pred = pred
        outs.level_hw = self.level_shapes(H, W)
        if self.training:
            return outs
        y = decode(pred.detach(), det.nc, outs.level_hw, STRIDES)
        return y, outs


def get_yolo8(model_type: str, nc: int = 80, **kw) -> Yolo8:
    return Yolo8(model_type, nc, **kw)
```

computervision.pytorch_amd/train.py:

```python
from __future__ import annotations

from typing import Dict, List, Optional

import torch

import ctypes as C
import os

from . import _lib as L
from .arena import EngineTrainStep
from .engine import V8LossOp, _note_param_write, adam_ema_step_dev, adam_step, adam_step_dev
from .graph import STRIDES
from .model import PredList, Yolo8
from .optim import FlatStep


def flatten_targets(batch: Dict[str, torch.Tensor], device) -> torch.Tensor:
    n = int(batch["batch_idx"].numel())
    device = torch.device(device)
    if n == 0:
        return torch.zeros(0, 6, device=device)
    bi, cls, box = batch["batch_idx"].reshape(-1), batch["cls"].reshape(-1), batch["bboxes"].reshape(-1, 4)
    if bi.is_cuda and device.type == "cuda":
        bi, cls, box = (t if t.dtype == torch.float32 and t.is_contiguous() else t.float().contiguous() for t in (bi, cls, box))
# ... 112 lines not shown
        self._ensure_state()
        if "state" in sd:
            params = self._all_params()
            self._m.zero_()
            self._v.zero_()
            step = 0
            skipped = []
            for i, st in sd["state"].items():
                i = int(i)
                if i >= len(params):
                    raise L.CvxError(f"optimizer checkpoint has state for parameter {i}, the model has {len(params)} parameters")
                mv = self._moment_views(params[i])
                if mv is None:
                    skipped.append(i)
                    continue
                for key in ("exp_avg", "exp_avg_sq"):
                    if tuple(st[key].shape) != tuple(params[i].shape):
                        raise L.CvxError(f"optimizer checkpoint: {key} of parameter {i} has shape {tuple(st[key].shape)}, the model's is {tuple(params[i].shape)}")
                mv[0].copy_(st["exp_avg"])
                mv[1].copy_(st["exp_avg_sq"])
                step = max(step, int(float(st["step"])))
            self._step = step
            if skipped:
                import warnings
                warnings.warn(f"FlatAdam.load_state_dict: state of {len(skipped)} parameter(s) (indices {skipped[:8]}...) was NOT restored: they are "
                              "not views of the flat parameter arena (their moments start from zero)", stacklevel=2)
        else:
            self._step = int(sd["step"])
            if sd.get("exp_avg") is not None:
                self._m.copy_(sd["exp_avg"])
                self._v.copy_(sd["exp_avg_sq"])
            else:
                self._m.zero_()
                self._v.zero_()
        self._state.copy_(torch.tensor([self.param_groups[0]["lr"], float(self._step), 0.0, 0.0]))
        self._lr_on_device = self.param_groups[0]["lr"]


class DynamicLossScale:

    def __init__(self, device, init_scale=65536.0, growth_factor=2.0, backoff_factor=0.5, growth_interval=2000,
                 min_scale=1.0, max_scale=2.0 ** 24):
        self.scale = float(init_scale)
        self.growth_factor, self.backoff_factor, self.growth_interval = growth_factor, backoff_factor, int(growth_interval)
        self.min_scale, self.max_scale = float(min_scale), float(max_scale)
        self.device = torch.device(device)
        self.found_inf = torch.zeros(1, dtype=torch.int32, device=device)
        self._host = torch.zeros(1, dtype=torch.int32).pin_memory() if torch.device(device).type == "cuda" else torch.zeros(1, dtype=torch.int32)
        self._event = None
        self._good = 0
        self.skipped = 0

    def poll(self):
        if self._event is None or not self._event.query():
            return
        self._event = None
        if int(self._host[0]) != 0:
            self.scale = max(self.scale * self.backoff_factor, self.min_scale)
            self._good = 0
            self.skipped += 1
        else:
            self._good += 1
            if self._good >= self.growth_interval:
                self.scale = min(self.scale * self.growth_factor, self.max_scale)
                self._good = 0

    def begin_step(self) -> float:
        self.poll()
        self.found_inf.zero_()
        return self.scale

    def end_step(self):
        if self._event is None:
            with torch.cuda.device(self.device):
                self._host.copy_(self.found_inf, non_blocking=True)
                self._event = torch.cuda.Event()
                self._event.record(torch.cuda.current_stream(self.device))

    def state_dict(self):
        return {"scale": self.scale, "good_steps": self._good}

    def load_state_dict(self, sd):
        self.scale, self._good = float(sd["scale"]), int(sd.get("good_steps", 0))


class CvxComm:

    def __init__(self, device: torch.device, process_group=None, rank: Optional[int] = None, world: Optional[int] = None, unique_id: Optional[bytes] = None):
        import torch.distributed as dist
        lib = L.load()
        have_pg = dist.is_available() and dist.is_initialized()
        self.rank = rank if rank is not None else (dist.get_rank(process_group) if have_pg else 0)
        self.world = world if world is not None else (dist.get_world_size(process_group) if have_pg else 1)
        if unique_id is None:
            buf = C.create_string_buffer(128)
            if self.rank == 0:
                L.check(lib.cvx_comm_unique_id(buf), "cvx_comm_unique_id")
            box = [bytes(buf.raw)]
            if self.world > 1:
                dist.broadcast_object_list(box, src=0, group=process_group)
            unique_id = box[0]
        self.handle = C.c_void_p()
        dev_index = device.index if device.index is not None else torch.cuda.current_device()
        L.check(lib.cvx_comm_create(C.byref(self.handle), C.c_char_p(unique_id), self.rank, self.world, dev_index), "cvx_comm_create")
        self.stream = None
        self._lib = lib

    def all_reduce_(self, t: torch.Tensor, stream: Optional[torch.cuda.Stream] = None):
        st = stream or torch.cuda.current_stream(t.device)
        L.check(self._lib.cvx_allreduce_f32(L.ptr(t), t.numel(), self.handle, C.c_void_p(st.cuda_stream)), "cvx_allreduce_f32")
        _note_param_write(t)
        return t

    def backward_exchange(self, eng, buckets, dpred: torch.Tensor, loss_scale: float):
        flat = (C.c_int64 * (4 * len(buckets)))(*[int(v) for b in buckets for v in b])
        eng._use_current_stream()
        self.stream = eng.exchange_stream()
        L.check(self._lib.cvx_engine_backward_exchange(eng.handle, L.ptr(dpred), float(loss_scale), self.handle, flat, len(buckets),
                                                       C.c_void_p(self.stream.cuda_stream)), "cvx_engine_backward_exchange")

    def __del__(self):
        try:
            if getattr(self, "handle", None):
                self._lib.cvx_comm_destroy(self.handle)
        except Exception:
            pass


class FusedTrainStep(EngineTrainStep):

    def __init__(self, model: Yolo8, criterion: V8DetectionLoss, optimizer: FlatAdam, process_group=None, n_buckets: int = 4,
                 scaler: Optional[DynamicLossScale] = None, comm: Optional["CvxComm"] = None):
        super().__init__(model, criterion, optimizer, scaler, process_group, n_buckets)
        self.comm = comm
        if comm is not None:
            self.world, self.distributed = comm.world, True
        self._pred = None
        self._dpred = None
        self._buckets, self._buckets_key = None, None

    def __call__(self, images: torch.Tensor, batch: Dict[str, torch.Tensor]) -> torch.Tensor:
        self.optimizer.sync_lr()
        return self._eager(images, batch)

    def _eager(self, images: torch.Tensor, batch: Dict[str, torch.Tensor]) -> torch.Tensor:
        m, crit = self.model, self.criterion
        dev = m.flat_params.device
        B, _, H, W = images.shape
        eng = m.engine_for(H, W)
        A, no = eng.graph.anchors, m.layout.no_pad
        if self._pred is None or self._pred.shape[0] != B or self._pred.shape[1] != A:
            self._pred = torch.empty(B, A, no, device=dev)
            self._dpred = torch.zeros(B, A, no, device=dev, dtype=torch.float16)
        targets = flatten_targets(batch, dev)
        scale = self.scaler.begin_step() if self.scaler is not None else crit.loss_scale
        pred = m._run_forward(images, training=True, pred=self._pred)
        items, dpred = crit.op(pred, targets, m.level_shapes(H, W), STRIDES, scale, self._dpred)
        if self.distributed and dev.type == "cuda":
            self._backward_overlapped(eng, dpred, scale)
        else:
            eng.backward(dpred, scale)
        self._update()
        return items

    def _backward_overlapped(self, eng, dpred, loss_scale):
        m = self.model
        g = m.flat_grads
        self._side = eng.exchange_stream()
        key = id(eng)
        if self._buckets_key != key:
            self._buckets = eng.grad_buckets(m.layout, self.n_buckets)
            self._buckets_key = key
        if self.comm is not None:
            self.comm.backward_exchange(eng, self._buckets, dpred, loss_scale)
            return
        cur = torch.cuda.current_stream(g.device)
        backward_with_overlapped_exchange(eng, self._buckets, g, dpred, loss_scale, self.pg, self._side)
        cur.wait_stream(self._side)


def backward_with_overlapped_exchange(eng, buckets, g: torch.Tensor, dpred, loss_scale: float, group=None, side_stream=None):
    import torch.distributed as dist
    eng.backward_begin(dpred, loss_scale)
    for op_hi, op_lo, p0, p1 in buckets:
        eng.backward_range(op_hi, op_lo)
        eng.grads_ready(op_hi, op_lo, side_stream)
        if side_stream is not None:
            with torch.cuda.stream(side_stream):
                dist.all_reduce(g[p0:p1], group=group)
        else:
            dist.all_reduce(g[p0:p1], group=group)
    eng.backward_end()


class OverlappedExchange:

    def __init__(self, process_group=None, n_buckets: int = 4):
        self.pg, self.n_buckets = process_group, n_buckets
        self._side = None
        self._buckets, self._key = None, None

    def backward(self, eng, flat_grads: torch.Tensor, dpred: torch.Tensor, loss_scale: float):
        from .graph import generic_grad_buckets
        self._side = eng.exchange_stream()
        if self._key != id(eng):
            self._buckets, self._key = generic_grad_buckets(eng.graph, self.n_buckets), id(eng)
        cur = torch.cuda.current_stream(flat_grads.device)
        backward_with_overlapped_exchange(eng, self._buckets, flat_grads, dpred, loss_scale, self.pg, self._side)
        cur.wait_stream(self._side)


def broadcast_bn_statistics(model: Yolo8, group=None, src: int = 0):
    import torch.distributed as dist
    if dist.is_available() and dist.is_initialized() and dist.get_world_size(group) > 1:
        dist.broadcast(model.flat_stats, src=src, group=group)
        dist.broadcast(model._flat["nbt"], src=src, group=group)


def bucket_bounds(n: int, n_buckets: int):
    per = (n + n_buckets - 1) // max(n_buckets, 1)
    per = max((per + 3) & ~3, 4)
    return [(s, min(n, s + per)) for s in range(0, n, per)]


def allreduce_mean_flat(g: torch.Tensor, world: int, group=None, n_buckets: int = 4, side_stream=None, average: bool = True):
    import torch.distributed as dist
    if not (dist.is_available() and dist.is_initialized()):
        return
    bounds = bucket_bounds(g.numel(), n_buckets)
    if not g.is_cuda or side_stream is None:
        for s, e in bounds:
            dist.all_reduce(g[s:e], group=group)
            if average:
                g[s:e].div_(world)
        return
    cur = torch.cuda.current_stream(g.device)
    side_stream.wait_stream(cur)
    with torch.cuda.stream(side_stream):
        for s, e in bounds:
            chunk = g[s:e]
            dist.all_reduce(chunk, group=group)
            if average:
                chunk.div_(world)
    cur.wait_stream(side_stream)
```

include/cvx_engine.h:

```cpp
#ifndef CVX_ENGINE_H
#define CVX_ENGINE_H
#include <stdint.h>
#ifdef __cplusplus
extern "C" {
#endif

#define CVX_ABI_VERSION 6

const char* cvx_last_error(void);
int cvx_abi_version(void);

enum { CVX_BUF_ACT_F16 = 0, CVX_BUF_PRED_F32 = 1 };
typedef struct {
  int32_t h, w, c;
  int32_t kind;
} cvx_buf_desc;

typedef struct {
  int32_t buf;
  int32_t coff;
  int32_t c;
  int32_t pix_off;
} cvx_view;

enum { CVX_OP_CONV = 1, CVX_OP_MAXPOOL5 = 2, CVX_OP_UPSAMPLE2 = 3,
       CVX_OP_MAXPOOL2 = 4,
       CVX_OP_DWCONVT = 5,
       CVX_OP_COPY = 6,
       CVX_OP_MAXPOOL3S2 = 7,
       CVX_OP_AVGPOOL = 8,
       CVX_OP_RESIZE = 9,
       CVX_OP_MAXPOOL3S1 = 10,
       CVX_OP_L2NORM = 11,
       CVX_OP_DROPOUT = 12 };
enum { CVX_ACT_BN_SILU = 1, CVX_ACT_BIAS = 2,
       CVX_ACT_BN_RELU = 3,
       CVX_ACT_BN_LINEAR = 4,
       CVX_ACT_BIAS_RELU = 5,
       CVX_ACT_BIAS_LINEAR = 6 };
#define CVX_OPF_RES_PRE_ACT 1
#define CVX_OPF_CONV_BIAS 2
#define CVX_OPF_RAW_F16 4

typedef struct {
  int32_t type;
  cvx_view in, out, res;
  int32_t ih, iw, oh, ow;
  int32_t k, stride, pad, dil;
  int32_t act;
  int32_t needs_dgrad;
  int32_t w_cin;
  int64_t w_off;
  int64_t gamma_off, beta_off;
  int64_t bias_off;
  int64_t rmean_off, rvar_off;
  int32_t lane;
  int32_t flags;
} cvx_op_desc;

typedef struct cvx_engine cvx_engine;

int cvx_engine_create(cvx_engine** out, const cvx_buf_desc* bufs, int32_t nbufs, const cvx_op_desc* ops, int32_t nops,
                      int32_t image_buf, int32_t pred_buf, int32_t device, void* hip_stream);
int cvx_engine_destroy(cvx_engine* e);

int cvx_engine_bind(cvx_engine* e, float* params, float* grads, int64_t n_params, float* stats, int64_t n_stats);

int cvx_engine_set_stream(cvx_engine* e, void* hip_stream);
void* cvx_engine_exchange_stream(cvx_engine* e);

int cvx_engine_set_bn(cvx_engine* e, float eps, float momentum);
int cvx_engine_keep_shadows(cvx_engine* e);
int cvx_engine_set_fusion(cvx_engine* e, int32_t enable);
int32_t cvx_engine_fused_groups(const cvx_engine* e);

int cvx_engine_set_seed(cvx_engine* e, uint64_t seed);

int cvx_engine_forward(cvx_engine* e, const float* images, int32_t batch, int32_t training, float* pred);

int cvx_engine_backward(cvx_engine* e, const void* dpred_f16, float loss_scale);

int cvx_engine_debug_copy(cvx_engine* e, int32_t buf, int32_t which, void* dst, int64_t bytes);

int cvx_engine_backward_begin(cvx_engine* e, const void* dpred_f16, float loss_scale);
int cvx_engine_backward_range(cvx_engine* e, int32_t op_hi, int32_t op_lo);
int cvx_engine_grads_ready(cvx_engine* e, int32_t op_hi, int32_t op_lo, void* hip_stream);
int cvx_engine_backward_end(cvx_engine* e);

int cvx_engine_profile(cvx_engine* e, int32_t enable);
int cvx_engine_profile_read(cvx_engine* e, int32_t n_classes, double* ms, double* flops, double* bytes, int64_t* launches);
int cvx_engine_profile_dump(cvx_engine* e, const char* path);

int cvx_debug_clock_buffer(void* buf);

int cvx_debug_conv_tile_plan(int32_t batch, int32_t h, int32_t w, int32_t cin, int32_t cout, int32_t* out8);
int cvx_debug_conv_dma_plan(int64_t pixels, int32_t cin, int32_t cout, int32_t ntaps, int32_t* out4);
int cvx_debug_conv_halo_plan(int32_t batch, int32_t h, int32_t w, int32_t cin, int32_t cout, int32_t* out4);
int cvx_debug_conv_pw_plan(int64_t pixels, int32_t cin, int32_t cout, int32_t* out4);
int cvx_debug_conv_grid_div(int32_t div);
int cvx_debug_conv_wgrad_plan(int32_t batch, int32_t ih, int32_t iw, int32_t cin, int32_t cout, int32_t k, int32_t stride, int32_t pad, int32_t dil,
                              int32_t x_ld, int32_t dy_ld, int32_t kernel, int32_t nsplit, int32_t wide, int32_t* out16);
int cvx_debug_conv2d_wgrad_nhwc(const void* x_f16, const void* dy_f16, int32_t batch, int32_t ih, int32_t iw, int32_t cin, int32_t cout, int32_t k,
                                int32_t stride, int32_t pad, int32_t dil, int32_t x_ld, int32_t dy_ld, int32_t kernel, int32_t nsplit, float* dw,
                                void* workspace, int64_t workspace_bytes, void* hip_stream);

int64_t cvx_engine_workspace_bytes(const cvx_engine* e);
int64_t cvx_engine_plan_generation(const cvx_engine* e);

int cvx_pred_level_to_nchw(const float* pred, int32_t batch, int32_t anchors, int32_t no, int32_t a_off, int32_t h, int32_t w,
                           float* out_nchw, void* hip_stream);
int cvx_nchw_grad_to_dpred(const float* grad_nchw, int32_t batch, int32_t anchors, int32_t no, int32_t a_off, int32_t h, int32_t w,
                           float scale, void* dpred_f16, void* hip_stream);

int64_t cvx_loss_v8_workspace_bytes(int32_t batch, int32_t anchors, int32_t nc, int32_t max_targets_per_image);
int cvx_loss_v8(const float* pred, int32_t batch, int32_t anchors, int32_t nc, const float* targets, int32_t n_targets,
                int32_t max_targets_per_image, const int32_t* level_hw, const float* strides, int32_t n_levels, float gain_box,
                float gain_cls, float gain_dfl, float loss_scale, float* loss_items, void* dpred_f16, void* workspace,
                int64_t workspace_bytes, void* hip_stream);
int cvx_loss_v8_strided(const float* pred, int32_t pred_ld, int32_t batch, int32_t anchors, int32_t nc, const float* targets,
                        int32_t n_targets, int32_t max_targets_per_image, const int32_t* level_hw, const float* strides, int32_t n_levels,
                        float gain_box, float gain_cls, float gain_dfl, float loss_scale, float* loss_items, void* dpred_f16,
                        void* workspace, int64_t workspace_bytes, void* hip_stream);

int cvx_loss_v8_assignment(const void* workspace, int32_t batch, int32_t anchors, int32_t max_targets_per_image, int32_t* gt_index,
                           float* norm_score, void* hip_stream);
int cvx_pack_targets(const float* batch_idx, const float* cls, const float* bboxes, int32_t n, float* rows, void* hip_stream);

int cvx_letterbox_geometry(int32_t h, int32_t w, int32_t H, int32_t W, int32_t* new_h, int32_t* new_w, int32_t* top, int32_t* left, double* scale);
int cvx_letterbox_u8_to_nchw(const uint8_t* image_hwc, int32_t h, int32_t w, int32_t letterbox, int32_t swap_rb, float* out_chw, int32_t H,
                             int32_t W, void* hip_stream);
typedef struct cvx_letterbox_job {
  const uint8_t* src;
  int32_t h, w, out, reserved;
} cvx_letterbox_job;
int cvx_letterbox_batch_u8_to_nchw(const cvx_letterbox_job* jobs, int32_t n_jobs, int32_t letterbox, int32_t swap_rb, float* out_nchw, int32_t H,
                                   int32_t W, void* hip_stream);

int cvx_adam_step(float* params, float* grads, float* exp_avg, float* exp_avg_sq, int64_t n, float lr, float beta1, float beta2,
                  float eps, int32_t step, const int32_t* found_inf, int32_t zero_grad, void* hip_stream);
int cvx_check_finite(const float* grads, int64_t n, int32_t* found_inf, void* hip_stream);
int cvx_adam_step_dev(float* params, float* grads, float* exp_avg, float* exp_avg_sq, int64_t n, float beta1, float beta2, float eps,
                      float* state, const int32_t* found_inf, int32_t zero_grad, float grad_scale, void* hip_stream);

int cvx_ema_update(float* ema, const float* src, int64_t n, float d, float one_minus_d, void* hip_stream);
int cvx_adam_ema_step_dev(float* params, float* grads, float* exp_avg, float* exp_avg_sq, int64_t n, float beta1, float beta2, float eps,
                          float* state, const int32_t* found_inf, int32_t zero_grad, float grad_scale, float* ema, float d, float one_minus_d,
                          void* hip_stream);

enum { CVX_OPTIM_SGD = 0, CVX_OPTIM_ADAM = 1 };
#define CVX_OPTIM_MAX_GROUPS 16
#define CVX_OPTIM_GROUP_FLOATS 8
#define CVX_OPTIM_UNMAPPED 255
int cvx_optim_step(int32_t kind, float* params, float* grads, float* buf1, float* buf2, int64_t n, const uint8_t* group_map, float* group_state,
                   int32_t n_groups, float* state, float beta1, float beta2, float eps, const int32_t* found_inf, int32_t zero_grad,
                   float grad_scale, const float* clip_state, float* ema, float d, float one_minus_d, void* hip_stream);
int64_t cvx_grad_norm_workspace(int64_t n);
int cvx_grad_norm(const float* grads, int64_t n, const uint8_t* group_map, const float* group_state, int32_t n_groups, float grad_scale,
                  float max_norm, float* clip_state, int32_t* found_inf, float* workspace, int64_t workspace_floats, void* hip_stream);

int cvx_decode(const float* pred, int32_t batch, int32_t anchors, int32_t nc, const int32_t* level_hw, const float* strides,
               int32_t n_levels, float* y, void* hip_stream);
int cvx_decode_strided(const float* pred, int32_t pred_ld, int32_t batch, int32_t anchors, int32_t nc, const int32_t* level_hw,
                       const float* strides, int32_t n_levels, float* y, void* hip_stream);
int cvx_ssd_decode(const float* loc, const float* conf, const float* priors, int32_t batch, int32_t anchors, int32_t num_classes_plus_bg,
                   float variance_xy, float variance_wh, float* boxes, float* prob, void* hip_stream);
int cvx_ssd_decode_max(const float* loc, const float* conf, const float* priors, int32_t B, int32_t A, int32_t num_classes_plus_bg,
                       float variance_xy, float variance_wh, float* boxes, float* prob, float* class_max, void* hip_stream);
int cvx_pred_cols_to_nchw(const float* rows, int32_t ld, int32_t col0, int32_t c, int32_t batch, int32_t anchors, int32_t a_off, int32_t hw,
                          float* out, int64_t out_bstride, int64_t out_off, void* hip_stream);
int cvx_yolo7_decode(const float* pred, int32_t pred_ld, int32_t batch, int32_t nc, const int32_t* level_hw, const float* anchors_wh,
                     int32_t n_levels, int32_t input_h, int32_t input_w, float* dec, float* y, void* hip_stream);
enum { CVX_NMS_TV0141_CUDA = 0,
       CVX_NMS_TV0141_CPU = 1,
       CVX_NMS_OFFSET = 2,
       CVX_NMS_VANILLA = 3 };
#define CVX_NMS_BOXES_XYXY 0x100
int64_t cvx_nms_workspace_bytes(int32_t batch, int32_t anchors);
int cvx_nms(const float* y, int32_t batch, int32_t anchors, int32_t nc, float conf_thres, float iou_thres, int32_t max_det,
            float* out_rows, int32_t* out_index, int32_t* counts, void* workspace, int64_t workspace_bytes, void* hip_stream);
int cvx_nms_variant(const float* y, int32_t batch, int32_t anchors, int32_t nc, float conf_thres, float iou_thres, int32_t max_det,
                    int32_t variant, float* out_rows, int32_t* out_index, int32_t* counts, void* workspace, int64_t workspace_bytes,
                    void* hip_stream);

int64_t cvx_centernet_decode_workspace_bytes(int32_t batch, int32_t h, int32_t w, int32_t nc);
int cvx_centernet_decode(const float* pred, int32_t pred_ld, int32_t batch, int32_t h, int32_t w, int32_t nc, int32_t reg_col, int32_t wh_col,
                         int32_t k, float conf, float nms_thr, int32_t use_nms, float* boxes, float* scores, int32_t* classes,
                         int32_t* topk_index, int32_t* keep, int32_t* counts, void* workspace, int64_t workspace_bytes, void* hip_stream);

int cvx_conv2d_nhwc(const void* x_f16, int32_t batch, int32_t ih, int32_t iw, int32_t cin, const void* w_f16, int32_t cout, int32_t k,
                    int32_t stride, int32_t pad, int32_t dil, int32_t mode, const float* scale_or_bias, const float* shift, void* out,
                    void* hip_stream);
int cvx_conv2d_dgrad_nhwc(const void* dy_f16, int32_t batch, int32_t ih, int32_t iw, int32_t cin, const void* wt_f16, int32_t cout,
                          int32_t k, int32_t stride, int32_t pad, int32_t dil, void* dx_f16, void* hip_stream);
int64_t cvx_conv2d_wgrad_workspace_bytes(int32_t batch, int32_t oh, int32_t ow, int32_t cin, int32_t cout, int32_t k);
int cvx_conv2d_wgrad_nhwc(const void* x_f16, const void* dy_f16, int32_t batch, int32_t ih, int32_t iw, int32_t cin, int32_t cout,
                          int32_t k, int32_t stride, int32_t pad, int32_t dil, float* dw, void* workspace, int64_t workspace_bytes,
                          void* hip_stream);


int cvx_bn_silu_train_nhwc(const float* y_f32, int32_t batch, int32_t hw, int32_t c, const float* gamma, const float* beta, float eps,
                           float momentum, float* running_mean, float* running_var, const void* res_f16, void* out_f16, void* xhat_f16,
                           float* mean, float* invstd, void* hip_stream);
int cvx_bn_silu_bwd_nhwc(const void* xhat_f16, const void* gout_f16, int32_t batch, int32_t hw, int32_t c, const float* gamma,
                         const float* beta, const float* invstd, float inv_scale, float* dgamma, float* dbeta, void* dy_f16, void* gres_f16,
                         int32_t res_accumulate, void* hip_stream);
int cvx_bn_act_train_nhwc(const float* y_f32, int32_t batch, int32_t hw, int32_t c, const float* gamma, const float* beta, float eps,
                          float momentum, float* running_mean, float* running_var, const void* res_f16, int32_t act, int32_t res_pre,
                          void* out_f16, void* xhat_f16, float* mean, float* invstd, void* hip_stream);
int cvx_bn_act_bwd_nhwc(const void* xhat_f16, const void* gout_f16, const void* out_f16, int32_t batch, int32_t hw, int32_t c,
                        const float* gamma, const float* beta, const float* invstd, int32_t act, int32_t res_pre, float inv_scale,
                        float* dgamma, float* dbeta, void* dy_f16, void* gres_f16, int32_t res_accumulate, void* hip_stream);
int cvx_debug_bn_bwd_plan(int64_t rows, int32_t c, int32_t* out4);
int cvx_debug_bn_bwd_views(const void* kept_f16, int32_t batch, int32_t hw, int32_t c, const float* gamma, const float* beta,
                           const float* invstd, const float* mean, int32_t act, int32_t res_pre, float inv_scale, const void* gout_f16,
                           int64_t gout_bstride, int32_t gout_ld, const void* fwd_f16, int64_t fwd_bstride, int32_t fwd_ld, void* gres_f16,
                           int64_t gres_bstride, int32_t gres_ld, int32_t res_accumulate, float* dgamma, float* dbeta, void* dy_f16,
                           void* hip_stream);
int cvx_maxpool5_nhwc(const void* x_f16, int32_t batch, int32_t h, int32_t w, int32_t c, void* out_f16, uint8_t* argmax, void* hip_stream);
int cvx_maxpool5_bwd_nhwc(const void* gout_f16, const uint8_t* argmax, int32_t batch, int32_t h, int32_t w, int32_t c, void* gin_f16,
                          int32_t accumulate, void* hip_stream);
int cvx_maxpool_nhwc(const void* x_f16, int32_t batch, int32_t h, int32_t w, int32_t c, int32_t kernel, int32_t stride, int32_t ceil_mode,
                     void* out_f16, void* hip_stream);
int cvx_avgpool_global_nhwc(const void* x_f16, int32_t batch, int32_t hw, int32_t c, void* out_f16, void* hip_stream);
int cvx_resize_bilinear_nhwc(const void* x_f16, int32_t batch, int32_t ih, int32_t iw, int32_t c, int32_t oh, int32_t ow, void* out_f16,
                             void* hip_stream);
int cvx_l2norm_nhwc(const void* x_f16, const float* weight, int32_t batch, int32_t hw, int32_t c, void* out_f16, void* hip_stream);
int cvx_resize_bilinear_rows_to_nchw(const float* rows_f32, int32_t ld, int32_t batch, int32_t c, int32_t ih, int32_t iw, int32_t oh, int32_t ow,
                                     float* out_nchw, void* hip_stream);
#define CVX_SEG_OPTS_KEY_OFFSET 4096
#define CVX_SEG_DIMS_BYTES 28
#define CVX_SEG_CRITERION_BYTES 128
typedef struct cvx_seg_dims {
  int32_t ld, batch, nc, ih, iw, oh, ow;
} cvx_seg_dims;
typedef struct cvx_seg_criterion {
  int32_t base;
  float focal_alpha, focal_gamma;
  const float* class_weight;
  float label_smoothing;
  int64_t ignore_index;
  float ohem_theta;
  int64_t ohem_min_kept;
  int32_t region;
  double base_weight, weight, alpha, beta, gamma, smooth;
  int32_t per_image, skip_absent;
  const float* region_class_weight;
} cvx_seg_criterion;
int64_t cvx_seg_criterion_workspace_bytes(const cvx_seg_dims* dims, const cvx_seg_criterion* crit, int32_t for_eval);
int cvx_seg_criterion_loss(const float* rows_f32, const cvx_seg_dims* dims, const int64_t* target, const cvx_seg_criterion* crit, float loss_scale,
                           float* loss_out, void* dpred_f16, int32_t* bad_target, double* stats_out, double* region_stats_out, void* workspace,
                           void* hip_stream);
int cvx_seg_criterion_eval(const float* rows_f32, const cvx_seg_dims* dims, const int64_t* target, const cvx_seg_criterion* crit, int64_t* confusion,
                           float* loss_out, double* region_stats_out, void* workspace, void* hip_stream);
int cvx_seg_criterion_lovasz_view(const cvx_seg_dims* dims, const cvx_seg_criterion* crit, int64_t offsets_out[3]);
int cvx_det_match(const float* rows, const int32_t* counts, int32_t batch, int32_t max_det, int32_t box_mode, const float* box_map,
                  const int32_t* gt, const int32_t* gt_counts, int32_t max_gt, int32_t nc, double min_overlap, int32_t quantize,
                  float* rec_score, int32_t* rec_class, int32_t* rec_flag, int64_t capacity, int64_t* state, int64_t* gt_per_class,
                  void* hip_stream);
int cvx_det_ap(const float* score, const int32_t* flag, const int64_t* seg_off, const int64_t* gt_per_class, int32_t nc,
               double score_threshold, int32_t quantize, double* prec, double* rec, double* stats, void* hip_stream);
int cvx_coco_match(const float* rows, const int32_t* counts, int32_t batch, int32_t max_det, int32_t box_mode, const float* box_map,
                   int32_t truncate, int32_t quantize, const double* gt, const int32_t* gt_counts, int32_t max_gt, int32_t nc,
                   const double* iou_thrs, float* rec_score, int32_t* rec_class, int32_t* rec_rank, int64_t* rec_matched, int64_t* rec_ignored,
                   int64_t capacity, int64_t* state, int64_t* npig, void* hip_stream);
int cvx_coco_accumulate(const int32_t* rank, const int64_t* matched, const int64_t* ignored, const int64_t* seg_off, const int64_t* npig,
                        int32_t nc, const double* rec_thrs, double* precision, double* recall, void* hip_stream);
int cvx_coco_summarize(const double* precision, const double* recall, int32_t nc, double* stats, void* hip_stream);
int64_t cvx_centernet_loss_workspace_bytes(int32_t batch, int32_t anchors);
int cvx_centernet_loss(const float* rows_f32, int32_t ld, int32_t batch, int32_t anchors, int32_t nc, int32_t col_a, int32_t col_b,
                       const float* heat_true, const float* true_a, const float* true_b, const float* mask, const int64_t* indices,
                       int32_t max_objects, float hm_weight, float a_weight, float b_weight, float loss_scale, float* loss_items, void* dpred_f16,
                       int32_t* bad_index, void* workspace, void* hip_stream);
int64_t cvx_multibox_loss_workspace_bytes(int32_t batch, int32_t anchors);
int cvx_multibox_loss(const float* loc, const float* conf, const float* y_true, int32_t batch, int32_t anchors, int32_t nc1, float neg_pos_ratio,
                      float alpha, float grad_scale, float* loss_items, float* dloc, float* dconf, void* workspace, void* hip_stream);
int64_t cvx_yolo7_loss_workspace_bytes(int32_t batch, int32_t anchors, int32_t ld, int32_t n_targets);
int cvx_yolo7_loss(const float* rows_f32, int32_t ld, int32_t batch, int32_t nc, const int32_t* level_hw, const float* anchors_px, const float* strides,
                   const float* targets, int32_t n_targets, float img_size, float box_ratio, float obj_ratio, float cls_ratio, float label_smoothing,
                   float loss_scale, float* loss_items, void* dpred_f16, int32_t* bad, void* workspace, void* hip_stream);
int cvx_debug_yolo7_loss_layout(int32_t batch, int32_t anchors, int32_t ld, int32_t n_targets, int64_t* offsets);
int cvx_centernet_draw_targets(const float* labels, const int32_t* counts, int32_t batch, int32_t max_boxes, int32_t fh, int32_t fw, int32_t nc,
                               float* heatmap, float* reg, float* wh, float* reg_mask, float* indices, void* hip_stream);
int cvx_ssd_encode_targets(const float* labels, const int32_t* counts, int32_t batch, int32_t max_boxes, const float* priors, int32_t anchors, int32_t nc1,
                           float overlap_threshold, float variance_xy, float variance_wh, float* y_true, int32_t* workspace, void* hip_stream);
int cvx_resize_bilinear_nchw_grad_to_rows(const float* grad_nchw, int32_t batch, int32_t nc, int32_t ih, int32_t iw, int32_t oh, int32_t ow,
                                          float scale, void* dpred_f16, int32_t ld, void* hip_stream);
int cvx_maxpool3_train_nhwc(const void* x_f16, int32_t batch, int32_t h, int32_t w, int32_t c, int32_t stride, void* out_f16, uint8_t* argmax,
                            void* hip_stream);
int cvx_maxpool3_bwd_nhwc(const void* gout_f16, const uint8_t* argmax, int32_t batch, int32_t h, int32_t w, int32_t c, int32_t stride,
                          void* gin_f16, int32_t accumulate, void* hip_stream);
int cvx_avgpool_global_bwd_nhwc(const void* gout_f16, int32_t batch, int32_t hw, int32_t c, void* gin_f16, int32_t accumulate, void* hip_stream);
int cvx_l2norm_bwd_nhwc(const void* x_f16, const void* gout_f16, const float* weight, int32_t batch, int32_t hw, int32_t c, float inv_scale,
                        void* gin_f16, float* dweight, int32_t accumulate, void* hip_stream);
int cvx_nchw_cols_grad_to_pred(const float* grad, int64_t grad_bstride, int64_t grad_off, int32_t c, int32_t batch, int32_t anchors, int32_t a_off,
                               int32_t hw, float scale, void* dpred_f16, int32_t ld, int32_t col0, void* hip_stream);
int cvx_maxpool2_bwd_nhwc(const void* x_f16, const void* gout_f16, int32_t batch, int32_t h, int32_t w, int32_t c, int32_t ceil_mode,
                          void* gin_f16, int32_t accumulate, void* hip_stream);
int cvx_dwconvt_nhwc(const void* x_f16, int32_t batch, int32_t ih, int32_t iw, int32_t c, int32_t f, const float* weight, void* out_f16,
                     void* hip_stream);
int cvx_dwconvt_bwd_nhwc(const void* x_f16, const void* gout_f16, int32_t batch, int32_t ih, int32_t iw, int32_t c, int32_t f, const float* weight,
                         void* gin_f16, int32_t accumulate, float* dweight, float inv_scale, void* hip_stream);
int cvx_resize_bilinear_bwd_nhwc(const void* gout_f16, int32_t batch, int32_t ih, int32_t iw, int32_t c, int32_t oh, int32_t ow, void* gin_f16,
                                 int32_t accumulate, void* hip_stream);
int cvx_dropout_nhwc(const void* x_f16, int32_t batch, int32_t hw, int32_t c, float p, uint64_t seed, void* out_f16, int32_t accumulate,
                     void* hip_stream);

int cvx_upsample2_nhwc(const void* x_f16, int32_t batch, int32_t h, int32_t w, int32_t c, void* out_f16, void* hip_stream);
int cvx_upsample2_bwd_nhwc(const void* gout_f16, int32_t batch, int32_t h, int32_t w, int32_t c, void* gin_f16, int32_t accumulate,
                           void* hip_stream);
int cvx_stem_train_nchw(const float* images, int32_t batch, int32_t h, int32_t w, const float* weight, int32_t cout, const float* gamma,
                        const float* beta, float eps, float momentum, float* running_mean, float* running_var, void* out_f16,
                        void* xhat_f16, float* mean, float* invstd, void* hip_stream);
int cvx_stem_eval_nchw(const float* images, int32_t batch, int32_t h, int32_t w, const float* weight, int32_t cout, const float* scale,
                       const float* shift, void* out_f16, void* hip_stream);
int cvx_stem_wgrad_nchw(const float* images, int32_t batch, int32_t h, int32_t w, const void* dy_f16, int32_t cout, float* dw,
                        void* hip_stream);
int cvx_stem_backward_nchw(const float* images, int32_t batch, int32_t h, int32_t w, const void* xhat_f16, const void* gout_f16, int32_t cout,
                           const float* gamma, const float* beta, const float* invstd, float inv_scale, float* dgamma, float* dbeta, float* dw,
                           void* hip_stream);
int cvx_stem_backward_recompute_nchw(const float* images, int32_t batch, int32_t h, int32_t w, const float* weight, const void* gout_f16, int32_t cout,
                                     const float* gamma, const float* beta, const float* mean, const float* invstd, float inv_scale,
                                     float* dgamma, float* dbeta, float* dw, void* hip_stream);

typedef struct cvx_aug_job {
  const uint8_t* src;
  int32_t ih, iw, nh, nw, dx, dy, flip, out, x0, y0, x1, y1, quad, reserved;
} cvx_aug_job;
int cvx_aug_images(const cvx_aug_job* jobs, const int32_t* job_start, const uint8_t* luts, int32_t batch, float* out_nchw, int32_t H, int32_t W,
                   void* hip_stream);
int cvx_aug_boxes(const cvx_aug_job* jobs, const int32_t* job_box_start, int32_t n_jobs, const float* boxes, int32_t n_boxes, int32_t H, int32_t W,
                  float* targets, int32_t* count, void* hip_stream);
int cvx_aug_images_plain(const cvx_aug_job* jobs, const int32_t* job_start, int32_t batch, float* out_nchw, int32_t H, int32_t W, void* hip_stream);
int cvx_aug_boxes_padded(const cvx_aug_job* jobs, const int32_t* job_start, const int32_t* job_box_start, int32_t batch, const float* boxes,
                         int32_t n_boxes, int32_t H, int32_t W, int32_t max_boxes, float* labels, int32_t* counts, int32_t* overflow, void* hip_stream);
typedef struct cvx_aug_view {
  float m[9], inv[9], s;
  int32_t partner;
  float r, r1;
  int32_t reserved[2];
} cvx_aug_view;
int cvx_aug_warp_mix(const float* canvases, const cvx_aug_view* views, int32_t batch, float* out_nchw, int32_t H, int32_t W, void* hip_stream);
int cvx_aug_boxes_warp(const float* labels_in, const int32_t* counts_in, int32_t cap_in, const cvx_aug_view* views, int32_t batch, int32_t H,
                       int32_t W, float min_wh, float min_area_ratio, float max_aspect, int32_t compact, float* out, int32_t cap_out,
                       int32_t* counts, int32_t* overflow, void* hip_stream);

typedef struct cvx_seg_job {
  const uint8_t* image;
  const uint8_t* mask;
  int32_t ih, iw, rh, rw, i, j, flip, mask_channels, reserved[4];
} cvx_seg_job;
int cvx_seg_pipeline(const cvx_seg_job* jobs, int32_t batch, const uint8_t* colours, int32_t n_colours, int32_t label_mode, const float* mean3,
                     const float* std3, float* out_nchw, int64_t* targets, int32_t H, int32_t W, void* hip_stream);

#define CVX_SEG_AUG_BRIGHTNESS 1
#define CVX_SEG_AUG_CONTRAST 2
#define CVX_SEG_AUG_CONTRAST_LAST 4
#define CVX_SEG_AUG_SATURATION 8
#define CVX_SEG_AUG_HUE 16
#define CVX_SEG_AUG_BLUR 32
typedef struct cvx_seg_aug_job {
  const uint8_t* image;
  const uint8_t* mask;
  int32_t ih, iw, rh, rw, i, j, flip, mask_channels;
  float cos, sin;
  int32_t flags;
  float beta, alpha, sat, hue;
  int32_t blur_k;
  float taps[9];
  int32_t reserved[3];
} cvx_seg_aug_job;
int cvx_seg_pipeline_aug(const cvx_seg_aug_job* jobs, int32_t batch, const uint8_t* colours, int32_t n_colours, int32_t label_mode,
                         int32_t unlisted_mode, int32_t ignore_index, const float* fill3, const float* mean3, const float* std3,
                         float* out_nchw, int64_t* targets, int32_t H, int32_t W, void* hip_stream);
// ... 93 lines not shown
```

Baseline: 5785 images/sec.

## Split v8 loss into prepare/prepared/finalize and parallelize TAL top-k across anchor chunks

Target packing and preparation move into one early kernel that runs before the forward pass. That kernel also clears the per-target tickets and bumps the batch counter, which removes the host-side flatten and several memsets. The TAL metric kernel is split across anchor chunks with per-chunk top-k candidates, merged by the last block through an atomic ticket. This replaces the per-anchor byte mask with a compact per-target selection list. Loss-item finalization runs on a separate exchange stream so it can overlap backward. The cost is more code complexity and an O(N^2) rank pack in a single block.

```diff
diff --git a/computervision.pytorch_amd/_lib.py b/computervision.pytorch_amd/_lib.py
--- a/computervision.pytorch_amd/_lib.py
+++ b/computervision.pytorch_amd/_lib.py
@@ -101,6 +101,10 @@
                            _I64, _P]),
     "cvx_loss_v8_strided": (_I32, [_P, _I32, _I32, _I32, _I32, _P, _I32, _I32, C.POINTER(_I32), C.POINTER(_F), _I32, _F, _F, _F, _F, _P, _P, _P,
                                    _I64, _P]),
+    "cvx_loss_v8_prepare_targets": (_I32, [_P, _P, _P, _I32, _I32, _I32, _I32, _I32, C.POINTER(_I32), C.POINTER(_F), _I32, _P, _I32, _P, _I64, _P]),
+    "cvx_loss_v8_prepared": (_I32, [_P, _I32, _I32, _I32, _I32, _I32, _I32, C.POINTER(_I32), C.POINTER(_F), _I32, _F, _F, _F, _F, _P, _P, _I64,
+                                    _P]),
+    "cvx_loss_v8_finalize": (_I32, [_P, _I64, _I32, _I32, _I32, _I32, _F, _F, _F, _P, _P]),
     "cvx_loss_v8_assignment": (_I32, [_P, _I32, _I32, _I32, _P, _P, _P]),
     "cvx_pack_targets": (_I32, [_P, _P, _P, _I32, _P, _P]),
     "cvx_decode_strided": (_I32, [_P, _I32, _I32, _I32, _I32, C.POINTER(_I32), C.POINTER(_F), _I32, _P, _P]),
@@ -197,6 +201,8 @@
                                       _P, _P, _P, _P]),
     "cvx_maxpool5_nhwc": (_I32, [_P, _I32, _I32, _I32, _I32, _P, _P, _P]),
     "cvx_maxpool5_bwd_nhwc": (_I32, [_P, _P, _I32, _I32, _I32, _I32, _P, _I32, _P]),
+    "cvx_sppf_pool3_nhwc": (_I32, [_P, _I32, _I32, _I32, _I32, _I32, _P, _P]),
+    "cvx_sppf_pool3_bwd_nhwc": (_I32, [_P, _P, _I32, _I32, _I32, _I32, _I32, _I32, _P]),
     "cvx_resize_bilinear_rows_to_nchw": (_I32, [_P, _I32, _I32, _I32, _I32, _I32, _I32, _I32, _P, _P]),
     "cvx_maxpool_nhwc": (_I32, [_P, _I32, _I32, _I32, _I32, _I32, _I32, _I32, _P, _P]),
     "cvx_avgpool_global_nhwc": (_I32, [_P, _I32, _I32, _I32, _P, _P]),
diff --git a/computervision.pytorch_amd/arena.py b/computervision.pytorch_amd/arena.py
--- a/computervision.pytorch_amd/arena.py
+++ b/computervision.pytorch_amd/arena.py
@@ -181,12 +181,12 @@
         self._after_bind(eng)
         return eng
 
-    def _run_forward(self, x: torch.Tensor, training: bool, pred=None) -> torch.Tensor:
+    def _run_forward(self, x: torch.Tensor, training: bool, pred=None, count_batch: bool = True) -> torch.Tensor:
         self._check_input(x, training)
         eng = self.engine_for(int(x.shape[2]), int(x.shape[3]))
         self._last_engine = eng
         rows = eng.forward(x, training, pred)
-        if training:
+        if training and count_batch:
             self._flat["nbt"] += 1
         return rows
 
diff --git a/computervision.pytorch_amd/csrc/loss_v8.hip b/computervision.pytorch_amd/csrc/loss_v8.hip
--- a/computervision.pytorch_amd/csrc/loss_v8.hip
+++ b/computervision.pytorch_amd/csrc/loss_v8.hip
@@ -81,10 +81,8 @@
   return iou - (rho2 / c2 + v * alpha);
 }
 
-__global__ void tgt_prep_kernel(const float* tg, int N, int B, float img_w, float img_h, float* gtbox, int* gtlabel, int* gtb, int* gtvalid,
-                                int* img_start, int* img_end) {
-  int n = blockIdx.x * blockDim.x + threadIdx.x;
-  if (n >= N) return;
+__device__ __forceinline__ void tgt_prep_row(const float* tg, int n, int N, int B, float img_w, float img_h, float* gtbox, int* gtlabel, int* gtb,
+                                             int* gtvalid, int* img_start, int* img_end) {
   const float* t = tg + (long long)n * 6;
   int b = (int)t[0];
   float cx = t[2] * img_w, cy = t[3] * img_h, w = t[4] * img_w, h = t[5] * img_h;
@@ -102,6 +100,45 @@
   }
 }
 
+__global__ void tgt_prep_kernel(const float* tg, int N, int B, float img_w, float img_h, float* gtbox, int* gtlabel, int* gtb, int* gtvalid,
+                                int* img_start, int* img_end) {
+  int n = blockIdx.x * blockDim.x + threadIdx.x;
+  if (n >= N) return;
+  tgt_prep_row(tg, n, N, B, img_w, img_h, gtbox, gtlabel, gtb, gtvalid, img_start, img_end);
+}
+
+__device__ __forceinline__ void pack_row(const float* bi, const float* cls, const float* box, int N, int i, float* out) {
+  const float b = bi[i];
+  int rank = 0;
+  for (int j = 0; j < N; ++j) {
+    const float bj = bi[j];
+    rank += (bj < b || (bj == b && j < i)) ? 1 : 0;
+  }
+  float* o = out + (long long)rank * 6;
+  o[0] = b;
+  o[1] = cls[i];
+  o[2] = box[i * 4 + 0];
+  o[3] = box[i * 4 + 1];
+  o[4] = box[i * 4 + 2];
+  o[5] = box[i * 4 + 3];
+}
+
+constexpr int TGT_EARLY_TPB = 1024;
+__global__ __launch_bounds__(TGT_EARLY_TPB) void tgt_early_kernel(const float* bi, const float* cls, const float* box, int N, int B, float img_w,
+                                                                  float img_h, float* rows, float* gtbox, int* gtlabel, int* gtb, int* gtvalid,
+                                                                  int* img_start, int* img_end, unsigned* ticket, long long* counters,
+                                                                  int n_counters) {
+  for (int i = threadIdx.x; i < B; i += TGT_EARLY_TPB) {
+    img_start[i] = 0;
+    img_end[i] = 0;
+  }
+  for (int i = threadIdx.x; i < N; i += TGT_EARLY_TPB) ticket[i] = 0u;
+  for (int i = threadIdx.x; i < n_counters; i += TGT_EARLY_TPB) counters[i] += 1;
+  for (int i = threadIdx.x; i < N; i += TGT_EARLY_TPB) pack_row(bi, cls, box, N, i, rows);
+  __syncthreads();
+  for (int n = threadIdx.x; n < N; n += TGT_EARLY_TPB) tgt_prep_row(rows, n, N, B, img_w, img_h, gtbox, gtlabel, gtb, gtvalid, img_start, img_end);
+}
+
 __global__ void pred_prep_kernel(const float* pred, int B, int A, int no, Levels L, float* pbox) {
   long long i = (long long)blockIdx.x * blockDim.x + threadIdx.x;
   if (i >= (long long)B * A * 4) return;
@@ -136,19 +173,26 @@
 }
 
 constexpr int TAL_TPB = 1024;
-__global__ __launch_bounds__(TAL_TPB) void tal_metric_kernel(const float* pred, int A, int no, int nc, Levels L, const float* pbox, const float* gtbox,
-                                                         const int* gtlabel, const int* gtb, const int* gtvalid, float* ov, float* metric,
-                                                         uint8_t* mask) {
+constexpr int TALM_TPB = 256;
+constexpr int TAL_MAX_SPLIT = 16;
+constexpr int TAL_MIN_CHUNK = 64;
+__global__ __launch_bounds__(TALM_TPB) void tal_metric_kernel(const float* pred, int A, int no, int nc, Levels L, const float* pbox, const float* gtbox,
+                                                          const int* gtlabel, const int* gtb, const int* gtvalid, float* ov, float* metric,
+                                                          int* sel, int chunk, float* cand_v, int* cand_i, unsigned* ticket) {
   extern __shared__ float smet[];
-  __shared__ float rv[TAL_TPB / 64];
-  __shared__ int ri[TAL_TPB / 64];
-  const int n = blockIdx.x;
+  __shared__ float rv[TALM_TPB / 64];
+  __shared__ int ri[TALM_TPB / 64];
+  __shared__ float cv[TAL_MAX_SPLIT * TOPK];
+  __shared__ int ci[TAL_MAX_SPLIT * TOPK];
+  __shared__ bool last;
+  const int n = blockIdx.y, part = blockIdx.x, S = gridDim.x;
+  const int a0 = part * chunk, a1 = min(A, a0 + chunk);
   const int b = gtb[n];
   const bool valid = gtvalid[n] != 0;
   const float gx1 = gtbox[n * 4], gy1 = gtbox[n * 4 + 1], gx2 = gtbox[n * 4 + 2], gy2 = gtbox[n * 4 + 3];
   int label = gtlabel[n];
   label = min(max(label, 0), nc - 1);
-  for (int a = threadIdx.x; a < A; a += TAL_TPB) {
+  for (int a = a0 + threadIdx.x; a < a1; a += TALM_TPB) {
     float ax, ay, st;
     anchor_of(L, a, &ax, &ay, &st);
     float px = ax * st, py = ay * st;
@@ -163,16 +207,17 @@
     }
     ov[(long long)n * A + a] = o;
     metric[(long long)n * A + a] = m;
-    mask[(long long)n * A + a] = 0;
-    smet[a] = m;
+    smet[a - a0] = m;
   }
   __syncthreads();
   const int lane = threadIdx.x & 63, wave = threadIdx.x >> 6;
+  float* my_v = cand_v + ((long long)n * S + part) * TOPK;
+  int* my_i = cand_i + ((long long)n * S + part) * TOPK;
   for (int r = 0; r < TOPK; ++r) {
     float best = 0.f;
     int bi = 0x7fffffff;
-    for (int a = threadIdx.x; a < A; a += TAL_TPB) {
-      float m = smet[a];
+    for (int a = a0 + threadIdx.x; a < a1; a += TALM_TPB) {
+      float m = smet[a - a0];
       if (m > best) {
         best = m;
         bi = a;
@@ -194,22 +239,53 @@
     float fb = rv[0];
     int fi = ri[0];
 #pragma unroll
-    for (int w = 1; w < TAL_TPB / 64; ++w)
+    for (int w = 1; w < TALM_TPB / 64; ++w)
       if (rv[w] > fb || (rv[w] == fb && ri[w] < fi)) {
         fb = rv[w];
         fi = ri[w];
       }
     __syncthreads();
-    if (!(fb > 0.f)) break;
+    if (!(fb > 0.f)) {
+      if (threadIdx.x == 0)
+        for (int q = r; q < TOPK; ++q) {
+          __hip_atomic_store(my_v + q, 0.f, __ATOMIC_RELAXED, __HIP_MEMORY_SCOPE_AGENT);
+          __hip_atomic_store(my_i + q, 0x7fffffff, __ATOMIC_RELAXED, __HIP_MEMORY_SCOPE_AGENT);
+        }
+      break;
+    }
     if (threadIdx.x == 0) {
-      smet[fi] = -1.f;
-      mask[(long long)n * A + fi] = 1;
+      smet[fi - a0] = -1.f;
+      __hip_atomic_store(my_v + r, fb, __ATOMIC_RELAXED, __HIP_MEMORY_SCOPE_AGENT);
+      __hip_atomic_store(my_i + r, fi, __ATOMIC_RELAXED, __HIP_MEMORY_SCOPE_AGENT);
     }
     __syncthreads();
   }
-}
-
-__global__ void tal_resolve_kernel(int B, int A, const int* img_start, const int* img_end, const float* ov, const uint8_t* mask, int* gt_idx) {
+  if (threadIdx.x == 0) {
+    __builtin_amdgcn_s_waitcnt(0);
+    last = __hip_atomic_fetch_add(ticket + n, 1u, __ATOMIC_RELAXED, __HIP_MEMORY_SCOPE_AGENT) == (unsigned)(S - 1);
+    if (last) __hip_atomic_store(ticket + n, 0u, __ATOMIC_RELAXED, __HIP_MEMORY_SCOPE_AGENT);
+  }
+  __syncthreads();
+  if (!last) return;
+  if (threadIdx.x < TOPK) sel[n * TOPK + threadIdx.x] = -1;
+  const int ncand = S * TOPK;
+  if ((int)threadIdx.x < ncand) {
+    cv[threadIdx.x] = __hip_atomic_load(cand_v + (long long)n * ncand + threadIdx.x, __ATOMIC_RELAXED, __HIP_MEMORY_SCOPE_AGENT);
+    ci[threadIdx.x] = __hip_atomic_load(cand_i + (long long)n * ncand + threadIdx.x, __ATOMIC_RELAXED, __HIP_MEMORY_SCOPE_AGENT);
+  }
+  __syncthreads();
+  if ((int)threadIdx.x < ncand) {
+    const float v = cv[threadIdx.x];
+    const int i = ci[threadIdx.x];
+    if (v > 0.f) {
+      int rank = 0;
+      for (int j = 0; j < ncand; ++j) rank += (cv[j] > v || (cv[j] == v && ci[j] < i)) ? 1 : 0;
+      if (rank < TOPK) sel[n * TOPK + rank] = i;
+    }
+  }
+}
+
+__global__ void tal_resolve_kernel(int B, int A, const int* img_start, const int* img_end, const float* ov, const int* sel, int* gt_idx) {
   long long i = (long long)blockIdx.x * blockDim.x + threadIdx.x;
   if (i >= (long long)B * A) return;
   int b = (int)(i / A), a = (int)(i - (long long)b * A);
@@ -217,7 +293,10 @@
   int cnt = 0, first = -1, arg = s;
   float best = -1.f;
   for (int n = s; n < e; ++n) {
-    if (mask[(long long)n * A + a]) {
+    bool mine = false;
+#pragma unroll
+    for (int r = 0; r < TOPK; ++r) mine = mine || sel[n * TOPK + r] == a;
+    if (mine) {
       if (cnt == 0) first = n;
       ++cnt;
     }
@@ -446,7 +525,10 @@
 struct Ws {
   float *gtbox, *pbox, *ov, *metric, *norm, *pos_align, *pos_ov, *tss_part, *loss_part, *aux;
   int *gtlabel, *gtb, *gtvalid, *img_start, *img_end, *gt_idx;
-  uint8_t* mask;
+  int* sel;
+  unsigned* ticket;
+  float *rows, *cand_v;
+  int* cand_i;
 };
 
 long long align_up(long long x) { return (x + 255) & ~255LL; }
@@ -467,10 +549,11 @@
   t.gtvalid = (int*)take(Nn * 4LL);
   t.img_start = (int*)take(B * 4LL);
   t.img_end = (int*)take(B * 4LL);
+  t.ticket = (unsigned*)take(Nn * 4LL);
   t.pbox = (float*)take(BA * 16);
   t.ov = (float*)take((long long)Nn * A * 4);
   t.metric = (float*)take((long long)Nn * A * 4);
-  t.mask = (uint8_t*)take((long long)Nn * A);
+  t.sel = (int*)take((long long)Nn * TOPK * 4);
   t.gt_idx = (int*)take(BA * 4);
   t.norm = (float*)take(BA * 4);
   t.pos_align = (float*)take(Nn * 4LL);
@@ -478,6 +561,9 @@
   t.tss_part = (float*)take(((BA + 255) / 256) * 4);
   t.loss_part = (float*)take(((BA + 15) / 16) * 12);
   t.aux = (float*)take(64);
+  t.rows = (float*)take(Nn * 24LL);
+  t.cand_v = (float*)take((long long)Nn * TAL_MAX_SPLIT * TOPK * 4);
+  t.cand_i = (int*)take((long long)Nn * TAL_MAX_SPLIT * TOPK * 4);
   if (w) *w = t;
   return off;
 }
@@ -496,18 +582,11 @@
                              loss_scale, loss_items, dpred_f16, workspace, workspace_bytes, hip_stream);
 }
 
-extern "C" int cvx_loss_v8_strided(const float* pred, int32_t pred_ld, int32_t B, int32_t A, int32_t nc, const float* targets, int32_t N,
-                                   int32_t max_targets, const int32_t* level_hw, const float* strides, int32_t n_levels, float gain_box,
-                                   float gain_cls, float gain_dfl, float loss_scale, float* loss_items, void* dpred_f16, void* workspace,
-                                   int64_t workspace_bytes, void* hip_stream) {
-  CVX_CHECK(pred && loss_items && dpred_f16 && workspace && level_hw && strides, "null arguments");
-  CVX_CHECK(pred_ld >= nc + 4 * REG && pred_ld % 4 == 0, "pred_ld must cover 64 + nc values and be a multiple of 4");
+namespace {
+
+int make_levels(const int32_t* level_hw, const float* strides, int32_t n_levels, int32_t A, Levels* out) {
+  CVX_CHECK(level_hw && strides, "null arguments");
   CVX_CHECK(n_levels >= 1 && n_levels <= MAXLV, "1..4 levels");
-  CVX_CHECK(N >= 0 && N <= max_targets && (N == 0 || targets), "targets");
-  CVX_CHECK(workspace_bytes >= cvx_loss_v8_workspace_bytes(B, A, nc, max_targets), "workspace too small");
-  CVX_CHECK(((uintptr_t)pred % 16) == 0 && ((uintptr_t)dpred_f16 % 8) == 0, "alignment");
-  hipStream_t st = (hipStream_t)hip_stream;
-  const int no = pred_ld;
   Levels L;
   memset(&L, 0, sizeof(L));
   L.n = n_levels;
@@ -520,6 +599,28 @@
   }
   L.a_off[n_levels] = off;
   CVX_CHECK(off == A, "level sizes do not add up to the anchor count");
+  *out = L;
+  return 0;
+}
+
+int tal_split(int N, int A) {
+  int s = cvx_cdiv(512, N > 0 ? N : 1);
+  s = s < A / TAL_MIN_CHUNK ? s : A / TAL_MIN_CHUNK;
+  s = s < TAL_MAX_SPLIT ? s : TAL_MAX_SPLIT;
+  return s < 1 ? 1 : s;
+}
+
+int run_chain(const float* pred, int32_t pred_ld, int32_t B, int32_t A, int32_t nc, const float* targets, bool prepared, int32_t N,
+              int32_t max_targets, const int32_t* level_hw, const float* strides, int32_t n_levels, float gain_box, float gain_cls, float gain_dfl,
+              float loss_scale, void* dpred_f16, void* workspace, int64_t workspace_bytes, hipStream_t st) {
+  CVX_CHECK(pred && dpred_f16 && workspace && level_hw && strides, "null arguments");
+  CVX_CHECK(pred_ld >= nc + 4 * REG && pred_ld % 4 == 0, "pred_ld must cover 64 + nc values and be a multiple of 4");
+  CVX_CHECK(N >= 0 && N <= max_targets && (N == 0 || targets || prepared), "targets");
+  CVX_CHECK(workspace_bytes >= cvx_loss_v8_workspace_bytes(B, A, nc, max_targets), "workspace too small");
+  CVX_CHECK(((uintptr_t)pred % 16) == 0 && ((uintptr_t)dpred_f16 % 8) == 0, "alignment");
+  const int no = pred_ld;
+  Levels L;
+  CVX_TRY(make_levels(level_hw, strides, n_levels, A, &L));
   const float img_h = level_hw[0] * strides[0], img_w = level_hw[1] * strides[0];
   char* base = (char*)(((uintptr_t)workspace + 255) & ~(uintptr_t)255);
   Ws w;
@@ -529,32 +630,85 @@
   const int n_lb = (int)((BA + 15) / 16);
   half_t* dpred = (half_t*)dpred_f16;
 
-  {
-    char *a = (char*)w.img_start, *b = (char*)w.img_end;
-    if (b > a && b - a <= 4096) {
-      CVX_HIP(hipMemsetAsync(a, 0, (size_t)(b - a) + (size_t)B * 4, st));
+  if (!prepared) {
+    char *a = (char*)w.img_start, *c = (char*)w.ticket + (size_t)(N > 0 ? N : 1) * 4;
+    if (c > a && c - a <= 65536) {
+      CVX_HIP(hipMemsetAsync(a, 0, (size_t)(c - a), st));
     } else {
       CVX_HIP(hipMemsetAsync(w.img_start, 0, B * 4, st));
       CVX_HIP(hipMemsetAsync(w.img_end, 0, B * 4, st));
-    }
+      CVX_HIP(hipMemsetAsync(w.ticket, 0, (size_t)(N > 0 ? N : 1) * 4, st));
+    }
+    if (N > 0)
+      hipLaunchKernelGGL(tgt_prep_kernel, dim3(cvx_cdiv(N, 128)), dim3(128), 0, st, targets, N, B, img_w, img_h, w.gtbox, w.gtlabel, w.gtb,
+                         w.gtvalid, w.img_start, w.img_end);
   }
   if (N > 0) {
-    hipLaunchKernelGGL(tgt_prep_kernel, dim3(cvx_cdiv(N, 128)), dim3(128), 0, st, targets, N, B, img_w, img_h, w.gtbox, w.gtlabel, w.gtb,
-                       w.gtvalid, w.img_start, w.img_end);
+    const int S = tal_split(N, A), chunk = cvx_cdiv(A, S);
     hipLaunchKernelGGL(pred_prep_kernel, dim3(cvx_cdiv(BA * 4, 256)), dim3(256), 0, st, pred, B, A, no, L, w.pbox);
-    hipLaunchKernelGGL(tal_metric_kernel, dim3(N), dim3(TAL_TPB), (size_t)A * 4, st, pred, A, no, nc, L, w.pbox, w.gtbox, w.gtlabel, w.gtb,
-                       w.gtvalid, w.ov, w.metric, w.mask);
-  }
-  hipLaunchKernelGGL(tal_resolve_kernel, dim3(cvx_cdiv(BA, 256)), dim3(256), 0, st, B, A, w.img_start, w.img_end, w.ov, w.mask, w.gt_idx);
+    hipLaunchKernelGGL(tal_metric_kernel, dim3(S, N), dim3(TALM_TPB), (size_t)chunk * 4, st, pred, A, no, nc, L, w.pbox, w.gtbox, w.gtlabel,
+                       w.gtb, w.gtvalid, w.ov, w.metric, w.sel, chunk, w.cand_v, w.cand_i, w.ticket);
+  }
+  hipLaunchKernelGGL(tal_resolve_kernel, dim3(cvx_cdiv(BA, 256)), dim3(256), 0, st, B, A, w.img_start, w.img_end, w.ov, w.sel, w.gt_idx);
   if (N > 0)
     hipLaunchKernelGGL(tal_posmax_kernel, dim3(N), dim3(TAL_TPB), 0, st, A, w.gtb, w.gt_idx, w.ov, w.metric, w.pos_align, w.pos_ov);
   hipLaunchKernelGGL(tal_norm_kernel, dim3(n_tss), dim3(256), 0, st, BA, A, w.gt_idx, w.metric, w.pos_align, w.pos_ov, w.norm, w.tss_part);
   hipLaunchKernelGGL(loss_grad_kernel, dim3(n_lb), dim3(256), 0, st, pred, B, A, no, nc, L, w.pbox, w.gtbox, w.gtlabel, w.gt_idx, w.norm,
                      w.tss_part, n_tss, gain_box, gain_cls, gain_dfl, loss_scale, dpred, w.loss_part);
-  hipLaunchKernelGGL(loss_finalize_kernel, dim3(1), dim3(1024), 0, st, w.loss_part, n_lb, w.tss_part, n_tss, gain_box, gain_cls, gain_dfl,
-                     loss_items, w.aux);
   CVX_HIP(hipGetLastError());
   return 0;
+}
+
+}
+
+extern "C" int cvx_loss_v8_finalize(void* workspace, int64_t workspace_bytes, int32_t B, int32_t A, int32_t nc, int32_t max_targets, float gain_box,
+                                    float gain_cls, float gain_dfl, float* loss_items, void* hip_stream) {
+  CVX_CHECK(workspace && loss_items && B > 0 && A > 0, "bad arguments");
+  CVX_CHECK(workspace_bytes >= cvx_loss_v8_workspace_bytes(B, A, nc, max_targets), "workspace too small");
+  char* base = (char*)(((uintptr_t)workspace + 255) & ~(uintptr_t)255);
+  Ws w;
+  carve(base, B, A, max_targets, &w);
+  const long long BA = (long long)B * A;
+  hipLaunchKernelGGL(loss_finalize_kernel, dim3(1), dim3(1024), 0, (hipStream_t)hip_stream, w.loss_part, (int)((BA + 15) / 16), w.tss_part,
+                     (int)((BA + 255) / 256), gain_box, gain_cls, gain_dfl, loss_items, w.aux);
+  CVX_HIP(hipGetLastError());
+  return 0;
+}
+
+extern "C" int cvx_loss_v8_strided(const float* pred, int32_t pred_ld, int32_t B, int32_t A, int32_t nc, const float* targets, int32_t N,
+                                   int32_t max_targets, const int32_t* level_hw, const float* strides, int32_t n_levels, float gain_box,
+                                   float gain_cls, float gain_dfl, float loss_scale, float* loss_items, void* dpred_f16, void* workspace,
+                                   int64_t workspace_bytes, void* hip_stream) {
+  CVX_CHECK(loss_items, "null arguments");
+  CVX_TRY(run_chain(pred, pred_ld, B, A, nc, targets, false, N, max_targets, level_hw, strides, n_levels, gain_box, gain_cls, gain_dfl, loss_scale,
+                    dpred_f16, workspace, workspace_bytes, (hipStream_t)hip_stream));
+  return cvx_loss_v8_finalize(workspace, workspace_bytes, B, A, nc, max_targets, gain_box, gain_cls, gain_dfl, loss_items, hip_stream);
+}
+
+extern "C" int cvx_loss_v8_prepare_targets(const float* batch_idx, const float* cls, const float* bboxes, int32_t N, int32_t B, int32_t A, int32_t nc,
+                                           int32_t max_targets, const int32_t* level_hw, const float* strides, int32_t n_levels, int64_t* counters,
+                                           int32_t n_counters, void* workspace, int64_t workspace_bytes, void* hip_stream) {
+  CVX_CHECK(workspace && B > 0 && A > 0, "bad arguments");
+  CVX_CHECK(N >= 0 && N <= max_targets && (N == 0 || (batch_idx && cls && bboxes)), "targets");
+  CVX_CHECK(n_counters >= 0 && (n_counters == 0 || counters), "counters");
+  CVX_CHECK(workspace_bytes >= cvx_loss_v8_workspace_bytes(B, A, nc, max_targets), "workspace too small");
+  Levels L;
+  CVX_TRY(make_levels(level_hw, strides, n_levels, A, &L));
+  const float img_h = level_hw[0] * strides[0], img_w = level_hw[1] * strides[0];
+  char* base = (char*)(((uintptr_t)workspace + 255) & ~(uintptr_t)255);
+  Ws w;
+  carve(base, B, A, max_targets, &w);
+  hipLaunchKernelGGL(tgt_early_kernel, dim3(1), dim3(TGT_EARLY_TPB), 0, (hipStream_t)hip_stream, batch_idx, cls, bboxes, N, B, img_w, img_h, w.rows,
+                     w.gtbox, w.gtlabel, w.gtb, w.gtvalid, w.img_start, w.img_end, w.ticket, (long long*)counters, n_counters);
+  CVX_HIP(hipGetLastError());
+  return 0;
+}
+
+extern "C" int cvx_loss_v8_prepared(const float* pred, int32_t pred_ld, int32_t B, int32_t A, int32_t nc, int32_t N, int32_t max_targets,
+                                    const int32_t* level_hw, const float* strides, int32_t n_levels, float gain_box, float gain_cls, float gain_dfl,
+                                    float loss_scale, void* dpred_f16, void* workspace, int64_t workspace_bytes, void* hip_stream) {
+  return run_chain(pred, pred_ld, B, A, nc, nullptr, true, N, max_targets, level_hw, strides, n_levels, gain_box, gain_cls, gain_dfl, loss_scale,
+                   dpred_f16, workspace, workspace_bytes, (hipStream_t)hip_stream);
 }
 
 extern "C" int cvx_loss_v8_assignment(const void* workspace, int32_t B, int32_t A, int32_t max_targets, int32_t* gt_index, float* norm_score,
@@ -573,19 +727,7 @@
 __global__ __launch_bounds__(256) void pack_targets_kernel(const float* bi, const float* cls, const float* box, int N, float* out) {
   const int i = blockIdx.x * 256 + threadIdx.x;
   if (i >= N) return;
-  const float b = bi[i];
-  int rank = 0;
-  for (int j = 0; j < N; ++j) {
-    const float bj = bi[j];
-    rank += (bj < b || (bj == b && j < i)) ? 1 : 0;
-  }
-  float* o = out + (long long)rank * 6;
-  o[0] = b;
-  o[1] = cls[i];
-  o[2] = box[i * 4 + 0];
-  o[3] = box[i * 4 + 1];
-  o[4] = box[i * 4 + 2];
-  o[5] = box[i * 4 + 3];
+  pack_row(bi, cls, box, N, i, out);
 }
 }
 
diff --git a/computervision.pytorch_amd/csrc/misc_ops.hip b/computervision.pytorch_amd/csrc/misc_ops.hip
--- a/computervision.pytorch_amd/csrc/misc_ops.hip
+++ b/computervision.pytorch_amd/csrc/misc_ops.hip
@@ -889,20 +889,26 @@
 __device__ __forceinline__ void pool5_row(const h8* src, int h, int w, int W, h8* rm, unsigned* ri) {
   float best[8];
   int bi[8];
-  bool first = true;
-#pragma unroll
-  for (int dx = 0; dx < 5; ++dx) {
-    const int ww = w + dx - 2;
-    const bool ok = ww >= 0 && ww < W;
-    const h8 v = src[h * W + min(max(ww, 0), W - 1)];
+  const h8* row = src + h * W;
+  {
+    const h8 v = row[max(w - 2, 0)];
+    const int dx0 = max(2 - w, 0);
+#pragma unroll
+    for (int k = 0; k < 8; ++k) {
+      best[k] = (float)v[k];
+      bi[k] = dx0;
+    }
+  }
+#pragma unroll
+  for (int dx = 1; dx < 5; ++dx) {
+    const h8 v = row[min(max(w + dx - 2, 0), W - 1)];
 #pragma unroll
     for (int k = 0; k < 8; ++k) {
       const float f = (float)v[k];
-      const bool take = ok && (first || f > best[k]);
-      best[k] = take ? f : (first ? -INFINITY : best[k]);
-      bi[k] = take ? dx : (first ? 0 : bi[k]);
-    }
-    first = first && !ok;
+      const bool take = f > best[k];
+      best[k] = take ? f : best[k];
+      bi[k] = take ? dx : bi[k];
+    }
   }
   h8 o;
   unsigned pk = 0;
@@ -917,22 +923,29 @@
 __device__ __forceinline__ h8 pool5_col(const h8* rm, const unsigned* ri, int h, int w, int H, int W, unsigned long long* pk_out) {
   float best[8];
   int bi[8];
-  bool first = true;
-#pragma unroll
-  for (int dy = 0; dy < 5; ++dy) {
-    const int hh = h + dy - 2;
-    const bool ok = hh >= 0 && hh < H;
-    const int q = min(max(hh, 0), H - 1) * W + w;
+  {
+    const int q = max(h - 2, 0) * W + w;
     const h8 v = rm[q];
     const unsigned di = ri[q];
+    const int dy0 = max(2 - h, 0);
+#pragma unroll
+    for (int k = 0; k < 8; ++k) {
+      best[k] = (float)v[k];
+      bi[k] = dy0 * 5 + (int)((di >> (4 * k)) & 7u);
+    }
+  }
+#pragma unroll
+  for (int dy = 1; dy < 5; ++dy) {
+    const int q = min(max(h + dy - 2, 0), H - 1) * W + w;
+    const h8 v = rm[q];
+    const unsigned di = ri[q];
 #pragma unroll
     for (int k = 0; k < 8; ++k) {
       const float f = (float)v[k];
-      const bool take = ok && (first || f > best[k]);
-      best[k] = take ? f : (first ? -INFINITY : best[k]);
-      bi[k] = take ? dy * 5 + (int)((di >> (4 * k)) & 7u) : (first ? 0 : bi[k]);
-    }
-    first = first && !ok;
+      const bool take = f > best[k];
+      best[k] = take ? f : best[k];
+      bi[k] = take ? dy * 5 + (int)((di >> (4 * k)) & 7u) : bi[k];
+    }
   }
   h8 o;
   unsigned long long pk = 0;
@@ -1000,19 +1013,25 @@
       float a[8];
 #pragma unroll
       for (int k = 0; k < 8; ++k) a[k] = 0.f;
+#pragma unroll
       for (int dy = 0; dy < 5; ++dy) {
         const int h = hq - dy + 2;
-        if (h < 0 || h >= H) continue;
+        const bool hok = h >= 0 && h < H;
+        const int hc = min(max(h, 0), H - 1) * W;
+#pragma unroll
         for (int dx = 0; dx < 5; ++dx) {
           const int w = wq - dx + 2;
-          if (w < 0 || w >= W) continue;
-          const int p = h * W + w;
+          const bool ok = hok && w >= 0 && w < W;
+          const int p = hc + min(max(w, 0), W - 1);
           const unsigned long long pk = pks[p];
           const h8 g = gcur[p];
-          const unsigned tap = (unsigned)(dy * 5 + dx);
-#pragma unroll
-          for (int k = 0; k < 8; ++k)
-            if (((pk >> (8 * k)) & 0xff) == tap) a[k] += (float)g[k];
+          const unsigned lo = (unsigned)pk, hi = (unsigned)(pk >> 32);
+          const unsigned tap = ok ? (unsigned)(dy * 5 + dx) : 0xffu;
+#pragma unroll
+          for (int k = 0; k < 4; ++k) {
+            a[k] += ((lo >> (8 * k)) & 0xffu) == tap ? (float)g[k] : 0.f;
+            a[4 + k] += ((hi >> (8 * k)) & 0xffu) == tap ? (float)g[4 + k] : 0.f;
+          }
         }
       }
       half_t* dst = gin.p + voff(gin, b, q) + cg * 8;
diff --git a/computervision.pytorch_amd/csrc/unit_ops.hip b/computervision.pytorch_amd/csrc/unit_ops.hip
--- a/computervision.pytorch_amd/csrc/unit_ops.hip
+++ b/computervision.pytorch_amd/csrc/unit_ops.hip
@@ -122,6 +122,28 @@
                                      void* gin_f16, int32_t accumulate, void* hip_stream) {
   CVX_CHECK(gout_f16 && argmax && gin_f16 && batch > 0 && c % 8 == 0, "bad arguments (channels in multiples of 8)");
   CVX_TRY(cvx_maxpool5_bwd(dense(gout_f16, h * w, c), dense(gin_f16, h * w, c), batch, h, w, c, argmax, accumulate, (hipStream_t)hip_stream));
+  CVX_HIP(hipStreamSynchronize((hipStream_t)hip_stream));
+  return 0;
+}
+extern "C" int cvx_sppf_pool3_nhwc(void* buf_f16, int32_t batch, int32_t h, int32_t w, int32_t c, int32_t ld, uint8_t* argmax, void* hip_stream) {
+  CVX_CHECK(buf_f16 && batch > 0 && h > 0 && w > 0 && c > 0 && c % 8 == 0 && ld >= 4 * c && ld % 8 == 0, "bad arguments (channels in multiples of 8, ld >= 4 c)");
+  half_t* p = (half_t*)buf_f16;
+  const long long bs = (long long)h * w * ld, n = (long long)batch * h * w * c;
+  auto slice = [&](int j) { return ViewDesc{p + (long long)j * c, bs, ld}; };
+  CVX_TRY(cvx_sppf_pool3_fwd(slice(0), slice(1), slice(2), slice(3), batch, h, w, c, argmax, argmax ? argmax + n : nullptr,
+                             argmax ? argmax + 2 * n : nullptr, (hipStream_t)hip_stream));
+  CVX_HIP(hipStreamSynchronize((hipStream_t)hip_stream));
+  return 0;
+}
+extern "C" int cvx_sppf_pool3_bwd_nhwc(void* gbuf_f16, const uint8_t* argmax, int32_t batch, int32_t h, int32_t w, int32_t c, int32_t ld,
+                                       int32_t acc_mask, void* hip_stream) {
+  CVX_CHECK(gbuf_f16 && argmax && batch > 0 && h > 0 && w > 0 && c > 0 && c % 8 == 0 && ld >= 4 * c && ld % 8 == 0,
+            "bad arguments (channels in multiples of 8, ld >= 4 c)");
+  half_t* p = (half_t*)gbuf_f16;
+  const long long bs = (long long)h * w * ld, n = (long long)batch * h * w * c;
+  auto slice = [&](int j) { return ViewDesc{p + (long long)j * c, bs, ld}; };
+  CVX_TRY(cvx_sppf_pool3_bwd(slice(3), slice(2), slice(1), slice(0), batch, h, w, c, argmax, argmax + n, argmax + 2 * n, acc_mask,
+                             (hipStream_t)hip_stream));
   CVX_HIP(hipStreamSynchronize((hipStream_t)hip_stream));
   return 0;
 }
diff --git a/computervision.pytorch_amd/engine.py b/computervision.pytorch_amd/engine.py
--- a/computervision.pytorch_amd/engine.py
+++ b/computervision.pytorch_amd/engine.py
@@ -176,6 +176,7 @@
         self.nc = nc
         self.gains = tuple(float(g) for g in gains)
         self._ws = None
+        self._prepared = None
 
     def __call__(self, pred: torch.Tensor, targets: torch.Tensor, level_hw, strides, loss_scale: float,
                  dpred: Optional[torch.Tensor] = None):
@@ -204,6 +205,53 @@
                                              self.gains[0], self.gains[1], self.gains[2], float(loss_scale), L.ptr(items), L.ptr(dpred),
                                              L.ptr(self._ws), self._ws.numel(), L.stream_ptr(pred.device)), "cvx_loss_v8")
         self._last_shape = (B, A, cap)
+        self._prepared = None
+        return items, dpred
+
+    def _workspace(self, B: int, A: int, cap: int, device):
+        need = int(self.lib.cvx_loss_v8_workspace_bytes(B, A, self.nc, cap))
+        if self._ws is None or self._ws.numel() < need or self._ws.device != device:
+            self._ws = torch.empty(need, dtype=torch.uint8, device=device)
+
+    def prepare_targets(self, batch_idx: torch.Tensor, cls: torch.Tensor, bboxes: torch.Tensor, B: int, A: int, level_hw, strides,
+                        counters: Optional[torch.Tensor] = None):
+        n = int(batch_idx.numel())
+        for name, t in (("batch_idx", batch_idx), ("cls", cls), ("bboxes", bboxes)):
+            _need_gpu(t, name)
+            assert t.dtype == torch.float32 and t.is_contiguous() and t.numel() == (4 * n if name == "bboxes" else n), name
+        dev = batch_idx.device
+        cap = max(n, 1)
+        self._workspace(B, A, cap, dev)
+        if counters is not None:
+            assert counters.dtype == torch.int64 and counters.is_contiguous() and counters.device == dev
+        lv, st, nl = _levels(level_hw, strides)
+        none = C.c_void_p(0)
+        L.check(self.lib.cvx_loss_v8_prepare_targets(L.ptr(batch_idx) if n else none, L.ptr(cls) if n else none, L.ptr(bboxes) if n else none, n, B, A,
+                                                     self.nc, cap, lv, st, nl, L.ptr(counters), 0 if counters is None else counters.numel(),
+                                                     L.ptr(self._ws), self._ws.numel(), L.stream_ptr(dev)), "cvx_loss_v8_prepare_targets")
+        self._prepared = (B, A, n, tuple(tuple(int(v) for v in hw) for hw in level_hw))
+        self._last_shape = (B, A, cap)
+
+    def run_prepared(self, pred: torch.Tensor, level_hw, strides, loss_scale: float, dpred: torch.Tensor, items_stream=None):
+        B, A, no = pred.shape
+        assert pred.dtype == torch.float32 and no == self.nc + 64
+        assert pred.stride(2) == 1 and pred.stride(0) == A * pred.stride(1) and pred.stride(1) % 4 == 0
+        ld = pred.stride(1)
+        assert self._prepared is not None, "prepare_targets first"
+        n = self._prepared[2]
+        assert self._prepared ==(B, A, n, tuple(tuple(int(v) for v in hw) for hw in level_hw)), "prepare_targets first (same shapes)"
+        assert dpred.is_contiguous() and dpred.shape[2] == ld and dpred.dtype == torch.float16
+        cap = max(n, 1)
+        items = torch.empty(3, dtype=torch.float32, device=pred.device)
+        lv, st, nl = _levels(level_hw, strides)
+        L.check(self.lib.cvx_loss_v8_prepared(L.ptr(pred), ld, B, A, self.nc, n, cap, lv, st, nl, self.gains[0], self.gains[1], self.gains[2],
+                                              float(loss_scale), L.ptr(dpred), L.ptr(self._ws), self._ws.numel(), L.stream_ptr(pred.device)),
+                "cvx_loss_v8_prepared")
+        cur = torch.cuda.current_stream(pred.device)
+        if items_stream is not None:
+            items_stream.wait_stream(cur)
+        L.check(self.lib.cvx_loss_v8_finalize(L.ptr(self._ws), self._ws.numel(), B, A, self.nc, cap, self.gains[0], self.gains[1], self.gains[2],
+                                              L.ptr(items), C.c_void_p((items_stream or cur).cuda_stream)), "cvx_loss_v8_finalize")
         return items, dpred
 
     def assignment(self, B: int, A: int, n_targets: int):
diff --git a/computervision.pytorch_amd/model.py b/computervision.pytorch_amd/model.py
--- a/computervision.pytorch_amd/model.py
+++ b/computervision.pytorch_amd/model.py
@@ -192,8 +192,8 @@
                 a[-1].bias.fill_(1.0)
                 b[-1].bias[:det.nc] = math.log(5 / det.nc / (640 / s) ** 2)
 
-    def _run_forward(self, images: torch.Tensor, training: bool, pred: Optional[torch.Tensor] = None) -> torch.Tensor:
-        out = super()._run_forward(images, training, pred)
+    def _run_forward(self, images: torch.Tensor, training: bool, pred: Optional[torch.Tensor] = None, count_batch: bool = True) -> torch.Tensor:
+        out = super()._run_forward(images, training, pred, count_batch)
         no = self.layout.no
         return out if out.shape[2] == no else out[..., :no]
 
diff --git a/computervision.pytorch_amd/train.py b/computervision.pytorch_amd/train.py
--- a/computervision.pytorch_amd/train.py
+++ b/computervision.pytorch_amd/train.py
@@ -288,10 +288,12 @@
         if self._pred is None or self._pred.shape[0] != B or self._pred.shape[1] != A:
             self._pred = torch.empty(B, A, no, device=dev)
             self._dpred = torch.zeros(B, A, no, device=dev, dtype=torch.float16)
-        targets = flatten_targets(batch, dev)
+        levels = m.level_shapes(H, W)
+        bi, cls, box = (batch[k].reshape(-1).to(dev, torch.float32, non_blocking=True).contiguous() for k in ("batch_idx", "cls", "bboxes"))
+        crit.op.prepare_targets(bi, cls, box, B, A, levels, STRIDES, counters=m._flat["nbt"])
         scale = self.scaler.begin_step() if self.scaler is not None else crit.loss_scale
-        pred = m._run_forward(images, training=True, pred=self._pred)
-        items, dpred = crit.op(pred, targets, m.level_shapes(H, W), STRIDES, scale, self._dpred)
+        pred = m._run_forward(images, training=True, pred=self._pred, count_batch=False)
+        items, dpred = crit.op.run_prepared(pred, levels, STRIDES, scale, self._dpred, items_stream=eng.exchange_stream() if dev.type == "cuda" else None)
         if self.distributed and dev.type == "cuda":
             self._backward_overlapped(eng, dpred, scale)
         else:
diff --git a/include/cvx_engine.h b/include/cvx_engine.h
--- a/include/cvx_engine.h
+++ b/include/cvx_engine.h
@@ -121,6 +121,15 @@
                         int32_t n_targets, int32_t max_targets_per_image, const int32_t* level_hw, const float* strides, int32_t n_levels,
                         float gain_box, float gain_cls, float gain_dfl, float loss_scale, float* loss_items, void* dpred_f16,
                         void* workspace, int64_t workspace_bytes, void* hip_stream);
+int cvx_loss_v8_prepare_targets(const float* batch_idx, const float* cls, const float* bboxes, int32_t n_targets, int32_t batch, int32_t anchors,
+                                int32_t nc, int32_t max_targets_per_image, const int32_t* level_hw, const float* strides, int32_t n_levels,
+                                int64_t* counters, int32_t n_counters, void* workspace, int64_t workspace_bytes, void* hip_stream);
+int cvx_loss_v8_prepared(const float* pred, int32_t pred_ld, int32_t batch, int32_t anchors, int32_t nc, int32_t n_targets,
+                         int32_t max_targets_per_image, const int32_t* level_hw, const float* strides, int32_t n_levels, float gain_box,
+                         float gain_cls, float gain_dfl, float loss_scale, void* dpred_f16, void* workspace, int64_t workspace_bytes,
+                         void* hip_stream);
+int cvx_loss_v8_finalize(void* workspace, int64_t workspace_bytes, int32_t batch, int32_t anchors, int32_t nc, int32_t max_targets_per_image,
+                         float gain_box, float gain_cls, float gain_dfl, float* loss_items, void* hip_stream);
 
 int cvx_loss_v8_assignment(const void* workspace, int32_t batch, int32_t anchors, int32_t max_targets_per_image, int32_t* gt_index,
                            float* norm_score, void* hip_stream);
@@ -219,6 +228,9 @@
 int cvx_maxpool5_nhwc(const void* x_f16, int32_t batch, int32_t h, int32_t w, int32_t c, void* out_f16, uint8_t* argmax, void* hip_stream);
 int cvx_maxpool5_bwd_nhwc(const void* gout_f16, const uint8_t* argmax, int32_t batch, int32_t h, int32_t w, int32_t c, void* gin_f16,
                           int32_t accumulate, void* hip_stream);
+int cvx_sppf_pool3_nhwc(void* buf_f16, int32_t batch, int32_t h, int32_t w, int32_t c, int32_t ld, uint8_t* argmax, void* hip_stream);
+int cvx_sppf_pool3_bwd_nhwc(void* gbuf_f16, const uint8_t* argmax, int32_t batch, int32_t h, int32_t w, int32_t c, int32_t ld,
+                            int32_t acc_mask, void* hip_stream);
 int cvx_maxpool_nhwc(const void* x_f16, int32_t batch, int32_t h, int32_t w, int32_t c, int32_t kernel, int32_t stride, int32_t ceil_mode,
                      void* out_f16, void* hip_stream);
 int cvx_avgpool_global_nhwc(const void* x_f16, int32_t batch, int32_t hw, int32_t c, void* out_f16, void* hip_stream);
```

Result: no change. 5835 images/sec (median of 6 runs) (+0.9%).
